# yeyupiaoling/VoiceprintRecognition-PaddlePaddle

Measured on NVIDIA H100. Metric: utterances/sec ECAPA-TDNN Fbank80 3s embed extract, higher is better.
Workload: dtype bf16x3 (split-bf16 operands, fp32 accumulate; fp32-grade)

## Files before the change

### include/ppv_b200.h

```cpp
#ifndef PPV_B200_H
#define PPV_B200_H

#include <stddef.h>
#include <stdint.h>

#ifdef __cplusplus
extern "C" {
#endif

#define PPV_OK 0
#define PPV_EINVAL (-1)
#define PPV_ECUDA (-2)
#define PPV_EUNSUPPORTED (-3)
#define PPV_ESTATE (-4)

#define PPV_PREC_BF16X3 0
#define PPV_PREC_BF16 1

#define PPV_POOL_ASP 0
#define PPV_POOL_SAP 1
#define PPV_POOL_TAP 2
#define PPV_POOL_TSP 3

typedef struct ppv_fbank ppv_fbank_t;
typedef struct ppv_model ppv_model_t;

int ppv_version(void);
int ppv_last_error(char* buf, size_t n);
int ppv_device_sm_count(void);

typedef struct {
    int sample_rate;
    int n_mels;
    float frame_length_ms;
    float frame_shift_ms;
    float preemph;
    float low_freq;
    float high_freq;
    float log_floor;
} ppv_fbank_cfg;

void ppv_fbank_default_cfg(ppv_fbank_cfg* cfg);
int ppv_fbank_create(const ppv_fbank_cfg* cfg, ppv_fbank_t** out);
int ppv_fbank_destroy(ppv_fbank_t* h);
int ppv_fbank_forward_ragged(ppv_fbank_t* h, const float* wav, const int32_t* valid_frames, int B, int L, float* out, void* stream);
int ppv_fbank_num_frames(const ppv_fbank_t* h, int L);
int ppv_fbank_feature_dim(const ppv_fbank_t* h);
int ppv_fbank_forward(ppv_fbank_t* h, const float* wav, const float* lens_ratio, int B, int L, float* out,
                      void* stream);

#define PPV_SPEC_SPECTROGRAM 1
#define PPV_SPEC_MEL 2
#define PPV_SPEC_LOGMEL 3
#define PPV_SPEC_MFCC 4
typedef struct {
    int method;
    int sample_rate;
    int n_fft;
    int hop_length;
    int win_length;
    float power;
    int center;
    int n_mels;
    float f_min;
    float f_max;
    int htk;
    int norm_slaney;
    float ref_value;
    float amin;
    int n_mfcc;
} ppv_spectral_cfg;
typedef struct ppv_spectral ppv_spectral_t;
void ppv_spectral_default_cfg(ppv_spectral_cfg* cfg, int method);
int ppv_spectral_create(const ppv_spectral_cfg* cfg, ppv_spectral_t** out);
int ppv_spectral_destroy(ppv_spectral_t* h);
int ppv_spectral_num_frames(const ppv_spectral_t* h, int L);
int ppv_spectral_feature_dim(const ppv_spectral_t* h);
int ppv_spectral_forward(ppv_spectral_t* h, const float* wav, const float* lens_ratio, int B, int L, float* out, void* stream);

#define PPV_SPECAUG_NPARAM 16
int ppv_spec_augment(float* feat, const int32_t* params, int B, int T, int F, int n_freq_masks, int n_time_masks, int fill_mode,
                     void* stream);

#define PPV_MODEL_ECAPA_TDNN 1

typedef struct {
    int input_size;
    int embd_dim;
    int channels[5];
    int kernel_sizes[5];
    int dilations[5];
    int attention_channels;
    int res2net_scale;
    int se_channels;
    int precision;
    int pooling;
    int global_context;
} ppv_ecapa_cfg;

void ppv_ecapa_default_cfg(ppv_ecapa_cfg* cfg);

#define PPV_MODEL_RESNET_SE 2
typedef struct {
    int input_size;
    int embd_dim;
    int layers[4];
    int num_filters[4];
    int attention_channels;
    int reduction;
    int precision;
} ppv_resnetse_cfg;
void ppv_resnetse_default_cfg(ppv_resnetse_cfg* cfg);

#define PPV_MODEL_ERES2NET 3
typedef struct {
    int input_size;
    int embd_dim;
    int num_blocks[4];
    int m_channels;
    int precision;
    int version;
    int base_width;
} ppv_eres2net_cfg;
void ppv_eres2net_default_cfg(ppv_eres2net_cfg* cfg);

#define PPV_MODEL_CAMPPLUS 4
typedef struct {
    int input_size;
    int embd_dim;
    int growth_rate;
    int bn_size;
    int init_channels;
    int precision;
} ppv_campplus_cfg;
void ppv_campplus_default_cfg(ppv_campplus_cfg* cfg);
int ppv_model_create(int kind, const void* cfg, ppv_model_t** out);
int ppv_model_destroy(ppv_model_t* h);
int ppv_model_load_weight(ppv_model_t* h, const char* name, const float* data, const int64_t* shape, int ndim);
int ppv_model_finalize(ppv_model_t* h);
int ppv_model_set_precision(ppv_model_t* h, int precision);
int ppv_model_embd_dim(const ppv_model_t* h);
size_t ppv_model_workspace_bytes(const ppv_model_t* h, int B, int T);
int ppv_model_forward(ppv_model_t* h, const float* feat, int B, int T, float* emb, void* ws, size_t ws_bytes,
                      void* stream);
int ppv_model_forward_lengths(ppv_model_t* h, const float* feat, const float* lengths, int B, int T, float* emb, void* ws,
                              size_t ws_bytes, void* stream);
int ppv_model_forward_wav(ppv_model_t* h, ppv_fbank_t* fb, const float* wav, const float* lens_ratio, int B, int L,
                          float* emb, void* ws, size_t ws_bytes, void* stream);
int ppv_model_read_tap(ppv_model_t* h, const char* name, float* out, size_t out_elems, void* stream);

int ppv_model_profile(ppv_model_t* h, int enable);
int ppv_model_profile_read(ppv_model_t* h, double* gemm_ms, double* other_ms, int64_t* gemm_launches,
                           int64_t* other_launches);

int ppv_set_pdl(int enabled);

typedef struct ppv_trainer ppv_trainer_t;
int ppv_trainer_create(const ppv_ecapa_cfg* cfg, int num_classes, ppv_trainer_t** out);
int ppv_trainer_destroy(ppv_trainer_t* h);
int64_t ppv_trainer_param_count(const ppv_trainer_t* h);
int64_t ppv_trainer_stat_count(const ppv_trainer_t* h);
int ppv_trainer_lookup(const ppv_trainer_t* h, const char* name, int64_t* offset, int64_t* numel, int* is_stat);
int ppv_trainer_bind(ppv_trainer_t* h, float* params, float* grads, float* stats);
int ppv_trainer_set_precision(ppv_trainer_t* h, int precision);
size_t ppv_trainer_workspace_bytes(ppv_trainer_t* h, int B, int T);
int ppv_trainer_forward_backward(ppv_trainer_t* h, const float* feat, const int64_t* labels, int B, int T, float margin, float scale,
                                 int easy_margin, float label_smoothing, float* loss, float* logits, void* ws, size_t ws_bytes, void* stream);
int ppv_trainer_read_tap(ppv_trainer_t* h, const char* name, float* out, size_t out_elems, void* stream);
int ppv_adam_step(float* params, const float* grads, float* m, float* v, int64_t n, float lr, float beta1, float beta2, float eps,
                  float weight_decay, int64_t step, float grad_scale, void* stream);

size_t ppv_cosine_workspace_bytes(int M, int N, int D);
int ppv_cosine_matrix(const float* A, const float* Bm, int M, int N, int D, float* out, void* ws, size_t ws_bytes,
                      void* stream);
int ppv_cosine_pairlist(const float* E, const int32_t* idx, int64_t P, int n, int D, float* out, void* stream);

#define PPV_PREP_NI 8
#define PPV_PREP_NF 4
size_t ppv_audio_prep_workspace_bytes(int B, int max_new_len);
int ppv_audio_prep(const float* wav, int64_t wav_ld, const int32_t* iparams, const float* fparams, const float* noise, int B,
                   int max_new_len, float target_db, int normalize, int Lout, float* out, void* ws, size_t ws_bytes, void* stream);

size_t ppv_eer_workspace_bytes(int64_t n);
int ppv_eer_mindcf(const float* scores, const int32_t* labels, int64_t n, double p_target, double c_miss, double c_fa, double* out4,
                   void* ws, size_t ws_bytes, void* stream);
int ppv_eer_mindcf_matrix(const float* scores, const int32_t* trial_labels, const int32_t* enroll_labels, int M, int N, double p_target,
                          double c_miss, double c_fa, double* out4, void* ws, size_t ws_bytes, void* stream);
int ppv_row_argmax(const float* sim, int rows, int cols, int32_t* idx, float* best, void* stream);

#define PPV_HEAD_AAM 0
#define PPV_HEAD_AAM_EASY 1
#define PPV_HEAD_AM 2
#define PPV_HEAD_ARM 3
#define PPV_HEAD_CE 4
#define PPV_HEAD_SUBCENTER 16
#define PPV_HEAD_SPHEREFACE2 8
int ppv_aam_forward(const float* emb, const float* W, const int64_t* labels, int B, int D, int S, float margin,
                    float scale, int easy_margin, float label_smoothing, float* logits, float* loss,
                    void* ws, size_t ws_bytes, void* stream);
size_t ppv_aam_workspace_bytes(int B, int D, int S);
int ppv_aam_backward(const float* emb, const float* W, const int64_t* labels, const float* logits, int B, int D,
                     int S, float margin, float scale, int easy_margin, float label_smoothing, float* d_emb,
                     float* d_W, void* ws, size_t ws_bytes, void* stream);

size_t ppv_gemm_test_workspace_bytes(int M, int N, int K);
int ppv_gemm_test(const float* A, const float* W, const float* bias, const float* bn_scale, const float* bn_shift,
                  int relu, int M, int N, int K, int block_n, int block_k, int precision, float* out, void* ws,
                  size_t ws_bytes, void* stream);

int ppv_gemm_test_planes(const float* A, const float* W, const float* bias, const float* rowgrp_bias, const float* bn_scale,
                         const float* bn_shift, int relu, int tanh_, int Tp, int P, int M, int N, int K, int block_n,
                         int precision, void* out, void* ws, size_t ws_bytes, void* stream);

size_t ppv_conv2d_test_workspace_bytes(int B, int H, int W, int Cin, int Cout, int k, int x_ld);
int ppv_conv2d_test(const float* x, const float* w, const float* bias, int relu, int B, int H, int W, int Cin, int Cout, int k,
                    int stride_h, int stride_w, int x_col0, int x_ld, int path, int precision, void* out, void* ws,
                    size_t ws_bytes, void* stream);

int ppv_gemm_bench(int M, int N, int K, int block_n, int block_k, int precision, int planes_out, int iters, void* ws,
                   size_t ws_bytes, float* ms_per_launch, void* stream);

#ifdef __cplusplus
}
#endif
#endif
```

### voiceprintrecognition-paddlepaddle_b200/csrc/capi.cu

```cuda
#include <string.h>

#include <new>

#include "common.h"
#include "image_plan.h"
#include "model_common.h"

namespace ppv {

static thread_local std::string g_last_error;

void set_error(const std::string& msg) { g_last_error = msg; }
int fail(int code, const std::string& msg) {
    g_last_error = msg;
    return code;
}

int device_sm_count() {
    int dev = 0, n = 0;
    if (cudaGetDevice(&dev) != cudaSuccess || cudaDeviceGetAttribute(&n, cudaDevAttrMultiProcessorCount, dev) != cudaSuccess || n <= 0) {
        cudaGetLastError();
        return 132;
    }
    return n;
}

static int check_device() {
    int dev = 0;
    if (cudaGetDevice(&dev) != cudaSuccess) return fail(PPV_ECUDA, "no CUDA device: libppv_b200 has no CPU fallback");
    int major = 0, minor = 0;
    cudaDeviceGetAttribute(&major, cudaDevAttrComputeCapabilityMajor, dev);
    cudaDeviceGetAttribute(&minor, cudaDevAttrComputeCapabilityMinor, dev);
    if (major != 9 || minor != 0) return fail(PPV_EUNSUPPORTED, "libppv_b200 is built for sm_90a only (found sm_" + std::to_string(major * 10 + minor) + ")");
    return PPV_OK;
}

}

using namespace ppv;

struct ppv_fbank {
    Fbank* impl;
};
struct ppv_spectral {
    Spectral* impl;
};

struct ppv_trainer {
    Trainer* impl;
};

struct ppv_model {
    int kind;
    Model* m;
};

static Model* ecapa_of(const ppv_model* h) { return h && h->kind == PPV_MODEL_ECAPA_TDNN ? h->m : nullptr; }

#define PPV_GUARD_BEGIN try {
#define PPV_GUARD_END                                                        \
    }                                                                        \
    catch (const std::bad_alloc&) { return fail(PPV_ECUDA, "host out of memory"); } \
    catch (const std::exception& e) { return fail(PPV_EINVAL, std::string("exception: ") + e.what()); } \
    catch (...) { return fail(PPV_EINVAL, "unknown exception"); }

extern "C" {

int ppv_version(void) { return 100; }

int ppv_last_error(char* buf, size_t n) {
    const std::string& e = g_last_error;
    if (buf && n > 0) {
        const size_t k = std::min(n - 1, e.size());
        memcpy(buf, e.data(), k);
        buf[k] = 0;
    }
    return int(e.size());
}

int ppv_device_sm_count(void) { return device_sm_count(); }

void ppv_fbank_default_cfg(ppv_fbank_cfg* c) {
    if (!c) return;
    c->sample_rate = 16000;
    c->n_mels = 80;
    c->frame_length_ms = 25.f;
    c->frame_shift_ms = 10.f;
    c->preemph = 0.97f;
    c->low_freq = 20.f;
    c->high_freq = 0.f;
    c->log_floor = 1.1920928955078125e-07f;
}

int ppv_fbank_create(const ppv_fbank_cfg* cfg, ppv_fbank_t** out) {
    PPV_GUARD_BEGIN
    PPV_REQUIRE(cfg && out, "ppv_fbank_create: null argument");
    int rc = check_device();
    if (rc) return rc;
    Fbank* impl = nullptr;
    rc = fbank_create(cfg, &impl);
    if (rc) return rc;
    *out = new ppv_fbank{impl};
    return PPV_OK;
    PPV_GUARD_END
}
int ppv_fbank_destroy(ppv_fbank_t* h) {
    if (!h) return PPV_OK;
    fbank_destroy(h->impl);
    delete h;
    return PPV_OK;
}
int ppv_fbank_num_frames(const ppv_fbank_t* h, int L) { return h ? fbank_num_frames(h->impl, L) : 0; }
int ppv_fbank_feature_dim(const ppv_fbank_t* h) { return h ? fbank_n_mels(h->impl) : 0; }

int ppv_fbank_forward(ppv_fbank_t* h, const float* wav, const float* lens_ratio, int B, int L, float* out, void* stream) {
    PPV_GUARD_BEGIN
    PPV_REQUIRE(h && wav && out, "ppv_fbank_forward: null argument");
    PPV_REQUIRE(B > 0 && L > 0, "ppv_fbank_forward: empty input");
    return fbank_run(h->impl, wav, lens_ratio, B, L, out, out, Planes(), 0, 0, static_cast<cudaStream_t>(stream));
    PPV_GUARD_END
}

int ppv_fbank_forward_ragged(ppv_fbank_t* h, const float* wav, const int32_t* valid_frames, int B, int L, float* out, void* stream) {
    PPV_GUARD_BEGIN
    PPV_REQUIRE(h && wav && out && valid_frames, "ppv_fbank_forward_ragged: null argument");
    PPV_REQUIRE(B > 0 && L > 0, "ppv_fbank_forward_ragged: empty input");
    return fbank_run(h->impl, wav, nullptr, B, L, out, out, Planes(), 0, 0, static_cast<cudaStream_t>(stream), valid_frames);
    PPV_GUARD_END
}

size_t ppv_audio_prep_workspace_bytes(int B, int max_new_len) { return audio_prep_workspace_bytes(B, max_new_len); }
int ppv_audio_prep(const float* wav, int64_t wav_ld, const int32_t* iparams, const float* fparams, const float* noise, int B, int max_new_len,
                   float target_db, int normalize, int Lout, float* out, void* ws, size_t ws_bytes, void* stream) {
    PPV_GUARD_BEGIN
    return audio_prep(wav, wav_ld, iparams, fparams, noise, B, max_new_len, target_db, normalize, Lout, out, ws, ws_bytes,
                      static_cast<cudaStream_t>(stream));
    PPV_GUARD_END
}

void ppv_ecapa_default_cfg(ppv_ecapa_cfg* c) {
    if (c) ppv_ecapa_default_cfg_impl(c);
}
void ppv_eres2net_default_cfg(ppv_eres2net_cfg* c) {
    if (c) ppv_eres2net_default_cfg_impl(c);
}
void ppv_campplus_default_cfg(ppv_campplus_cfg* c) {
    if (c) ppv_campplus_default_cfg_impl(c);
}
void ppv_resnetse_default_cfg(ppv_resnetse_cfg* c) {
    if (c) ppv_resnetse_default_cfg_impl(c);
}

int ppv_model_create(int kind, const void* cfg, ppv_model_t** out) {
    PPV_GUARD_BEGIN
    PPV_REQUIRE(cfg && out, "ppv_model_create: null argument");
    if (kind != PPV_MODEL_ECAPA_TDNN && kind != PPV_MODEL_RESNET_SE && kind != PPV_MODEL_ERES2NET && kind != PPV_MODEL_CAMPPLUS)
        return fail(PPV_EUNSUPPORTED,
                    "ppv_model_create: implemented kinds are PPV_MODEL_ECAPA_TDNN, PPV_MODEL_RESNET_SE, PPV_MODEL_ERES2NET, PPV_MODEL_CAMPPLUS");
    int rc = check_device();
    if (rc) return rc;
    Model* m = nullptr;
    switch (kind) {
        case PPV_MODEL_ECAPA_TDNN: rc = ecapa_create(static_cast<const ppv_ecapa_cfg*>(cfg), &m); break;
        case PPV_MODEL_RESNET_SE: rc = resnetse_create(static_cast<const ppv_resnetse_cfg*>(cfg), &m); break;
        case PPV_MODEL_ERES2NET: rc = eres2net_create(static_cast<const ppv_eres2net_cfg*>(cfg), &m); break;
        default: rc = campplus_create(static_cast<const ppv_campplus_cfg*>(cfg), &m); break;
    }
    if (rc) return rc;
    *out = new ppv_model{kind, m};
    return PPV_OK;
    PPV_GUARD_END
}
int ppv_model_destroy(ppv_model_t* h) {
    if (!h) return PPV_OK;
    delete h->m;
    delete h;
    return PPV_OK;
}
int ppv_model_load_weight(ppv_model_t* h, const char* name, const float* data, const int64_t* shape, int ndim) {
    PPV_GUARD_BEGIN
    PPV_REQUIRE(h, "ppv_model_load_weight: null model");
    return h->m->load_weight(name, data, shape, ndim);
    PPV_GUARD_END
}
int ppv_model_finalize(ppv_model_t* h) {
    PPV_GUARD_BEGIN
    PPV_REQUIRE(h, "ppv_model_finalize: null model");
    return h->m->finalize();
    PPV_GUARD_END
}
int ppv_model_set_precision(ppv_model_t* h, int precision) {
    PPV_REQUIRE(h, "ppv_model_set_precision: null model");
    return h->m->set_precision(precision);
}
int ppv_model_embd_dim(const ppv_model_t* h) { return h ? h->m->embd_dim() : 0; }
size_t ppv_model_workspace_bytes(const ppv_model_t* h, int B, int T) { return h ? h->m->workspace_bytes(B, T) : 0; }

int ppv_model_forward(ppv_model_t* h, const float* feat, int B, int T, float* emb, void* ws, size_t ws_bytes, void* stream) {
    PPV_GUARD_BEGIN
    PPV_REQUIRE(h && feat && emb, "ppv_model_forward: null argument");
    return h->m->forward(feat, B, T, emb, ws, ws_bytes, static_cast<cudaStream_t>(stream));
    PPV_GUARD_END
}
int ppv_model_forward_lengths(ppv_model_t* h, const float* feat, const float* lengths, int B, int T, float* emb, void* ws, size_t ws_bytes,
                              void* stream) {
    PPV_GUARD_BEGIN
    PPV_REQUIRE(h && feat && emb, "ppv_model_forward_lengths: null argument");
    if (!ecapa_of(h)) return fail(PPV_EUNSUPPORTED, "ppv_model_forward_lengths: only EcapaTdnn.forward takes lengths in the reference");
    return ecapa_forward(h->m, feat, nullptr, nullptr, nullptr, B, T, 0, emb, ws, ws_bytes, static_cast<cudaStream_t>(stream), lengths);
    PPV_GUARD_END
}
int ppv_model_forward_wav(ppv_model_t* h, ppv_fbank_t* fb, const float* wav, const float* lens_ratio, int B, int L, float* emb,
                          void* ws, size_t ws_bytes, void* stream) {
    PPV_GUARD_BEGIN
    PPV_REQUIRE(h && fb && wav && emb, "ppv_model_forward_wav: null argument");
    if (!ecapa_of(h)) return fail(PPV_EUNSUPPORTED, "ppv_model_forward_wav: the fused waveform path exists for ECAPA-TDNN only; call ppv_fbank_forward + ppv_model_forward");
    const int T = fbank_num_frames(fb->impl, L);
    PPV_REQUIRE(T > 0, "ppv_model_forward_wav: waveform shorter than one frame");
    return ecapa_forward(h->m, nullptr, fb->impl, wav, lens_ratio, B, T, L, emb, ws, ws_bytes, static_cast<cudaStream_t>(stream));
    PPV_GUARD_END
}
int ppv_model_read_tap(ppv_model_t* h, const char* name, float* out, size_t out_elems, void* stream) {
    PPV_GUARD_BEGIN
    PPV_REQUIRE(h, "ppv_model_read_tap: null model");
    return h->m->read_tap(name, out, out_elems, static_cast<cudaStream_t>(stream));
    PPV_GUARD_END
}

size_t ppv_eer_workspace_bytes(int64_t n) { return eer_workspace_bytes(n); }
int ppv_eer_mindcf(const float* scores, const int32_t* labels, int64_t n, double p_target, double c_miss, double c_fa, double* out4, void* ws,
                   size_t ws_bytes, void* stream) {
    PPV_GUARD_BEGIN
    PPV_REQUIRE(labels, "ppv_eer_mindcf: null labels");
    return eer_mindcf(scores, labels, nullptr, nullptr, 0, n, p_target, c_miss, c_fa, out4, ws, ws_bytes, static_cast<cudaStream_t>(stream));
    PPV_GUARD_END
}
int ppv_eer_mindcf_matrix(const float* scores, const int32_t* trial_labels, const int32_t* enroll_labels, int M, int N, double p_target,
                          double c_miss, double c_fa, double* out4, void* ws, size_t ws_bytes, void* stream) {
    PPV_GUARD_BEGIN
    PPV_REQUIRE(trial_labels && enroll_labels && M > 0 && N > 0, "ppv_eer_mindcf_matrix: bad argument");
    return eer_mindcf(scores, nullptr, trial_labels, enroll_labels, N, int64_t(M) * N, p_target, c_miss, c_fa, out4, ws, ws_bytes,
                      static_cast<cudaStream_t>(stream));
    PPV_GUARD_END
}
int ppv_row_argmax(const float* sim, int rows, int cols, int32_t* idx, float* best, void* stream) {
    PPV_GUARD_BEGIN
    return row_argmax(sim, rows, cols, idx, best, static_cast<cudaStream_t>(stream));
    PPV_GUARD_END
}

int ppv_model_profile(ppv_model_t* h, int enable) {
    PPV_REQUIRE(ecapa_of(h), "ppv_model_profile: ECAPA-TDNN model required");
    return ecapa_profile(h->m, enable);
}
int ppv_model_profile_read(ppv_model_t* h, double* gemm_ms, double* other_ms, int64_t* gemm_launches, int64_t* other_launches) {
    PPV_GUARD_BEGIN
    PPV_REQUIRE(ecapa_of(h), "ppv_model_profile_read: ECAPA-TDNN model required");
    return ecapa_profile_read(h->m, gemm_ms, other_ms, gemm_launches, other_launches);
    PPV_GUARD_END
}

void ppv_spectral_default_cfg(ppv_spectral_cfg* c, int method) {
    if (c) spectral_default_cfg(c, method);
}
int ppv_spectral_create(const ppv_spectral_cfg* cfg, ppv_spectral_t** out) {
    PPV_GUARD_BEGIN
    PPV_REQUIRE(cfg && out, "ppv_spectral_create: null argument");
    int rc = check_device();
    if (rc) return rc;
    Spectral* impl = nullptr;
    rc = spectral_create(cfg, &impl);
    if (rc) return rc;
    *out = new ppv_spectral{impl};
    return PPV_OK;
    PPV_GUARD_END
}
int ppv_spectral_destroy(ppv_spectral_t* h) {
    if (!h) return PPV_OK;
    spectral_destroy(h->impl);
    delete h;
    return PPV_OK;
}
int ppv_spectral_num_frames(const ppv_spectral_t* h, int L) { return h ? spectral_num_frames(h->impl, L) : 0; }
int ppv_spectral_feature_dim(const ppv_spectral_t* h) { return h ? spectral_feature_dim(h->impl) : 0; }
int ppv_spectral_forward(ppv_spectral_t* h, const float* wav, const float* lens_ratio, int B, int L, float* out, void* stream) {
    PPV_GUARD_BEGIN
    PPV_REQUIRE(h && wav && out, "ppv_spectral_forward: null argument");
    PPV_REQUIRE(B > 0 && L > 0, "ppv_spectral_forward: empty input");
    return spectral_run(h->impl, wav, lens_ratio, B, L, out, static_cast<cudaStream_t>(stream));
    PPV_GUARD_END
}
int ppv_spec_augment(float* feat, const int32_t* params, int B, int T, int F, int n_freq_masks, int n_time_masks, int fill_mode, void* stream) {
    PPV_GUARD_BEGIN
    return spec_augment_run(feat, params, B, T, F, n_freq_masks, n_time_masks, fill_mode, static_cast<cudaStream_t>(stream));
    PPV_GUARD_END
}

int ppv_trainer_create(const ppv_ecapa_cfg* cfg, int num_classes, ppv_trainer_t** out) {
    PPV_GUARD_BEGIN
    PPV_REQUIRE(cfg && out, "ppv_trainer_create: null argument");
    int rc = check_device();
    if (rc) return rc;
    Trainer* impl = nullptr;
    rc = trainer_create(cfg, num_classes, &impl);
    if (rc) return rc;
    *out = new ppv_trainer{impl};
    return PPV_OK;
    PPV_GUARD_END
}
int ppv_trainer_destroy(ppv_trainer_t* h) {
    if (!h) return PPV_OK;
    trainer_destroy(h->impl);
    delete h;
    return PPV_OK;
}
int64_t ppv_trainer_param_count(const ppv_trainer_t* h) { return h ? trainer_param_count(h->impl) : 0; }
int64_t ppv_trainer_stat_count(const ppv_trainer_t* h) { return h ? trainer_stat_count(h->impl) : 0; }
int ppv_trainer_lookup(const ppv_trainer_t* h, const char* name, int64_t* offset, int64_t* numel, int* is_stat) {
    PPV_GUARD_BEGIN
    PPV_REQUIRE(h, "ppv_trainer_lookup: null handle");
    return trainer_lookup(h->impl, name, offset, numel, is_stat);
    PPV_GUARD_END
}
int ppv_set_pdl(int enabled) {
    const int prev = ppv::pdl_enabled();
    ppv::pdl_enabled() = enabled ? 1 : 0;
    return prev;
}
int ppv_trainer_set_precision(ppv_trainer_t* h, int precision) {
    PPV_GUARD_BEGIN
    PPV_REQUIRE(h, "ppv_trainer_set_precision: null handle");
    return trainer_set_precision(h->impl, precision);
    PPV_GUARD_END
}
int ppv_trainer_bind(ppv_trainer_t* h, float* params, float* grads, float* stats) {
    PPV_GUARD_BEGIN
    PPV_REQUIRE(h, "ppv_trainer_bind: null handle");
    return trainer_bind(h->impl, params, grads, stats);
    PPV_GUARD_END
}
size_t ppv_trainer_workspace_bytes(ppv_trainer_t* h, int B, int T) {
    try {
        return h ? trainer_workspace_bytes(h->impl, B, T) : 0;
    } catch (...) {
        return 0;
    }
}
int ppv_trainer_forward_backward(ppv_trainer_t* h, const float* feat, const int64_t* labels, int B, int T, float margin, float scale,
                                 int easy_margin, float label_smoothing, float* loss, float* logits, void* ws, size_t ws_bytes, void* stream) {
    PPV_GUARD_BEGIN
    PPV_REQUIRE(h, "ppv_trainer_forward_backward: null handle");
    return trainer_forward_backward(h->impl, feat, labels, B, T, margin, scale, easy_margin, label_smoothing, loss, logits, ws, ws_bytes,
                                    static_cast<cudaStream_t>(stream));
    PPV_GUARD_END
}
int ppv_trainer_read_tap(ppv_trainer_t* h, const char* name, float* out, size_t out_elems, void* stream) {
    PPV_GUARD_BEGIN
    PPV_REQUIRE(h, "ppv_trainer_read_tap: null handle");
    return trainer_read_tap(h->impl, name, out, out_elems, static_cast<cudaStream_t>(stream));
    PPV_GUARD_END
}
int ppv_adam_step(float* params, const float* grads, float* m, float* v, int64_t n, float lr, float beta1, float beta2, float eps,
                  float weight_decay, int64_t step, float grad_scale, void* stream) {
    PPV_GUARD_BEGIN
    return adam_step(params, grads, m, v, n, lr, beta1, beta2, eps, weight_decay, step, grad_scale, static_cast<cudaStream_t>(stream));
    PPV_GUARD_END
}

size_t ppv_cosine_workspace_bytes(int M, int N, int D) { return cosine_workspace_bytes(M, N, D); }
int ppv_cosine_matrix(const float* A, const float* Bm, int M, int N, int D, float* out, void* ws, size_t ws_bytes, void* stream) {
    PPV_GUARD_BEGIN
    int rc = check_device();
    if (rc) return rc;
    return cosine_matrix(A, Bm, M, N, D, out, ws, ws_bytes, PPV_PREC_BF16X3, static_cast<cudaStream_t>(stream));
    PPV_GUARD_END
}
int ppv_cosine_pairlist(const float* E, const int32_t* idx, int64_t P, int n, int D, float* out, void* stream) {
    PPV_GUARD_BEGIN
    return cosine_pairlist(E, idx, P, n, D, out, static_cast<cudaStream_t>(stream));
    PPV_GUARD_END
}

size_t ppv_aam_workspace_bytes(int B, int D, int S) { return aam_workspace_bytes(B, D, S); }
int ppv_aam_forward(const float* emb, const float* W, const int64_t* labels, int B, int D, int S, float margin, float scale,
                    int easy_margin, float label_smoothing, float* logits, float* loss, void* ws, size_t ws_bytes, void* stream) {
    PPV_GUARD_BEGIN
    return aam_forward(emb, W, labels, B, D, S, margin, scale, easy_margin, label_smoothing, logits, loss, ws, ws_bytes,
                       static_cast<cudaStream_t>(stream));
    PPV_GUARD_END
}
int ppv_aam_backward(const float* emb, const float* W, const int64_t* labels, const float* logits, int B, int D, int S, float margin,
                     float scale, int easy_margin, float label_smoothing, float* d_emb, float* d_W, void* ws, size_t ws_bytes,
                     void* stream) {
    PPV_GUARD_BEGIN
    return aam_backward(emb, W, labels, logits, B, D, S, margin, scale, easy_margin, label_smoothing, d_emb, d_W, ws, ws_bytes,
                        static_cast<cudaStream_t>(stream));
    PPV_GUARD_END
}

static inline size_t au(size_t x, size_t a) { return (x + a - 1) / a * a; }
size_t ppv_gemm_test_workspace_bytes(int M, int N, int K) {
    const size_t Kp = au(size_t(K), 64);
    return au(au(size_t(M), 128) * Kp * 4, 256) + au(au(size_t(N), 256) * Kp * 4, 256) + 256;
}
int ppv_gemm_test(const float* A, const float* W, const float* bias, const float* bn_scale, const float* bn_shift, int relu, int M,
                  int N, int K, int block_n, int block_k, int precision, float* out, void* ws, size_t ws_bytes, void* stream) {
    PPV_GUARD_BEGIN
    PPV_REQUIRE(A && W && out && ws, "ppv_gemm_test: null argument");
    PPV_REQUIRE(ws_bytes >= ppv_gemm_test_workspace_bytes(M, N, K), "ppv_gemm_test: workspace too small");
    int rc = check_device();
    if (rc) return rc;
    cudaStream_t st = static_cast<cudaStream_t>(stream);
    const int Kp = int(au(size_t(K), 64));
    Planes pa, pw;
    pa.rows = int64_t(au(size_t(M), 128));
    pa.ld = Kp;
    pa.plane_stride = pa.rows * Kp;
    pa.base = static_cast<__nv_bfloat16*>(ws);
    pw.rows = int64_t(au(size_t(N), 256));
    pw.ld = Kp;
    pw.plane_stride = pw.rows * Kp;
    pw.base = reinterpret_cast<__nv_bfloat16*>(static_cast<uint8_t*>(ws) + au(size_t(pa.plane_stride) * 4, 256));
    PPV_CUDA_OK(cudaMemsetAsync(ws, 0, ppv_gemm_test_workspace_bytes(M, N, K), st));
    rc = launch_f32_to_planes(A, M, K, pa, st);
    if (rc) return rc;
    rc = launch_f32_to_planes(W, N, K, pw, st);
    if (rc) return rc;
    GemmSource src{pa, 0, Kp, 0};
    Epilogue ep;
    ep.bias = bias;
    ep.relu = relu;
    ep.bn_scale = bn_scale;
    ep.bn_shift = bn_shift;
    ep.out_mode = OUT_F32;
    ep.out = out;
    ep.out_ld = N;
    GemmParams gp;
    rc = gemm_build(&gp, &src, 1, pw, M, N, ep, block_n, block_k);
    if (rc) return rc;
    return gemm_launch(gp, precision, device_sm_count(), st);
    PPV_GUARD_END
}

int ppv_gemm_test_planes(const float* A, const float* W, const float* bias, const float* rowgrp_bias, const float* bn_scale,
                         const float* bn_shift, int relu, int tanh_, int Tp, int P, int M, int N, int K, int block_n, int precision,
                         void* out, void* ws, size_t ws_bytes, void* stream) {
    PPV_GUARD_BEGIN
    PPV_REQUIRE(A && W && out && ws, "ppv_gemm_test_planes: null argument");
    PPV_REQUIRE(ws_bytes >= ppv_gemm_test_workspace_bytes(M, N, K), "ppv_gemm_test_planes: workspace too small");
    PPV_REQUIRE(N % 32 == 0 && (Tp == 0 || (M % Tp == 0 && Tp > 2 * P)), "ppv_gemm_test_planes: bad shape");
    int rc = check_device();
    if (rc) return rc;
    cudaStream_t st = static_cast<cudaStream_t>(stream);
    const int Kp = int(au(size_t(K), 64));
    Planes pa, pw;
    pa.rows = int64_t(au(size_t(M), 128));
    pa.ld = Kp;
    pa.plane_stride = pa.rows * Kp;
    pa.base = static_cast<__nv_bfloat16*>(ws);
    pw.rows = int64_t(au(size_t(N), 256));
    pw.ld = Kp;
    pw.plane_stride = pw.rows * Kp;
    pw.base = reinterpret_cast<__nv_bfloat16*>(static_cast<uint8_t*>(ws) + au(size_t(pa.plane_stride) * 4, 256));
    PPV_CUDA_OK(cudaMemsetAsync(ws, 0, ppv_gemm_test_workspace_bytes(M, N, K), st));
    rc = launch_f32_to_planes(A, M, K, pa, st);
    if (rc) return rc;
    rc = launch_f32_to_planes(W, N, K, pw, st);
    if (rc) return rc;
    GemmSource src{pa, 0, Kp, 0};
    Epilogue ep;
    ep.bias = bias;
    ep.rowgrp_bias = rowgrp_bias;
    ep.relu = relu;
    ep.tanh_ = tanh_;
    ep.bn_scale = bn_scale;
    ep.bn_shift = bn_shift;
    ep.out_mode = OUT_PLANES;
    ep.out = out;
    ep.out_ld = N;
    ep.out_plane_stride = int64_t(M) * N;
    if (Tp > 0) {
        ep.Tp = Tp;
        ep.P = P;
        ep.T = Tp - 2 * P;
    }
    GemmParams gp;
    rc = gemm_build(&gp, &src, 1, pw, M, N, ep, block_n, 64);
    if (rc) return rc;
    return gemm_launch(gp, precision, device_sm_count(), st);
    PPV_GUARD_END
}

static size_t conv2d_test_x_bytes(int B, int H, int W, int x_ld) {
    return au(au(size_t(B) * (H + 2) * (W + 2), 128) * size_t(x_ld) * 4, 256);
}
size_t ppv_conv2d_test_workspace_bytes(int B, int H, int W, int Cin, int Cout, int k, int x_ld) {
    if (x_ld <= 0) x_ld = Cin;
    return conv2d_test_x_bytes(B, H, W, x_ld) + au(au(size_t(Cout), 256) * k * k * Cin * 4, 256) + 256;
}
int ppv_conv2d_test(const float* x, const float* w, const float* bias, int relu, int B, int H, int W, int Cin, int Cout, int k,
                    int stride_h, int stride_w, int x_col0, int x_ld, int path, int precision, void* out, void* ws, size_t ws_bytes,
                    void* stream) {
    PPV_GUARD_BEGIN
    PPV_REQUIRE(x && w && out && ws, "ppv_conv2d_test: null argument");
    if (x_ld <= 0) x_ld = Cin;
    PPV_REQUIRE(B > 0 && H > 0 && W > 0 && Cin > 0 && Cout > 0 && (k == 1 || k == 3) && stride_h >= 1 && stride_w >= 1,
                "ppv_conv2d_test: bad shape");
    PPV_REQUIRE(x_col0 >= 0 && x_col0 + Cin <= x_ld, "ppv_conv2d_test: the input columns exceed x_ld");
    PPV_REQUIRE(path >= 0 && path <= 2, "ppv_conv2d_test: path must be 0 (3x3 patch kernel), 1 (pointwise kernel) or 2 (gather-GEMM)");
    PPV_REQUIRE(precision == PPV_PREC_BF16X3 || precision == PPV_PREC_BF16, "ppv_conv2d_test: bad precision");
    PPV_REQUIRE(ws_bytes >= ppv_conv2d_test_workspace_bytes(B, H, W, Cin, Cout, k, x_ld), "ppv_conv2d_test: workspace too small");
    const int Hp = H + 2, Wp = W + 2, Ho = (H - 1) / stride_h + 1, Wo = (W - 1) / stride_w + 1;
    const int64_t M = int64_t(B) * Hp * Wp;
    PPV_REQUIRE(M < (int64_t(1) << 31) && Wp + 1 < 32768, "ppv_conv2d_test: grid too large for 32-bit rows / 16-bit tap offsets");
    int rc = check_device();
    if (rc) return rc;
    cudaStream_t st = static_cast<cudaStream_t>(stream);
    Planes xp;
    xp.rows = int64_t(au(size_t(M), 128));
    xp.ld = x_ld;
    xp.plane_stride = xp.rows * x_ld;
    xp.base = static_cast<__nv_bfloat16*>(ws);
    const size_t x_bytes = conv2d_test_x_bytes(B, H, W, x_ld);
    PPV_CUDA_OK(cudaMemsetAsync(ws, 0, x_bytes, st));
    const size_t pitch = size_t(x_ld) * sizeof(__nv_bfloat16), rows2 = size_t(2 * xp.rows);
    if (x_col0 > 0) PPV_CUDA_OK(cudaMemset2DAsync(xp.base, pitch, 0x3f, size_t(x_col0) * sizeof(__nv_bfloat16), rows2, st));
    if (x_col0 + Cin < x_ld)
        PPV_CUDA_OK(cudaMemset2DAsync(xp.base + x_col0 + Cin, pitch, 0x3f, size_t(x_ld - x_col0 - Cin) * sizeof(__nv_bfloat16), rows2, st));
    for (int b = 0; b < B; ++b)
        for (int h = 0; h < H; ++h) {
            Planes row = xp;
            row.base = xp.base + ((int64_t(b) * Hp + h + 1) * Wp + 1) * x_ld + x_col0;
            rc = launch_f32_to_planes(x + (int64_t(b) * H + h) * W * Cin, W, Cin, row, st);
            if (rc) return rc;
        }
    const int K = k * k * Cin;
    std::vector<float> wh(size_t(Cout) * K);
    PPV_CUDA_OK(cudaMemcpyAsync(wh.data(), w, wh.size() * sizeof(float), cudaMemcpyDeviceToHost, st));
    PPV_CUDA_OK(cudaStreamSynchronize(st));
    ArenaBuilder ab;
    GemmWeights gw;
    ab.put_matrix(&gw, conv_weight_matrix(wh.data(), Cout, Cin, k * k, Cout, {{k * k, Cin, 0, Cin, 0}}), Cout, K);
    uint8_t* wdev = static_cast<uint8_t*>(ws) + x_bytes;
    PPV_CUDA_OK(cudaMemcpyAsync(wdev, ab.host.data(), ab.host.size(), cudaMemcpyHostToDevice, st));
    PPV_CUDA_OK(cudaStreamSynchronize(st));
    gw.W.base = reinterpret_cast<__nv_bfloat16*>(wdev + ab.patches[0].off);
    const int64_t out_plane = int64_t(B) * (Ho + 2) * (Wo + 2) * Cout;
    PPV_CUDA_OK(cudaMemsetAsync(out, 0, size_t(2 * out_plane) * sizeof(__nv_bfloat16), st));
    Planes outp;
    outp.base = static_cast<__nv_bfloat16*>(out);
    outp.ld = Cout;
    outp.plane_stride = out_plane;
    const ImageGeo gin{H, W, Hp, Wp}, gout{Ho, Wo, Ho + 2, Wo + 2};
    Epilogue ep = image_epilogue(outp, gin, gout, stride_h, stride_w);
    ep.bias = bias;
    ep.relu = relu ? 1 : 0;
    const int sms = device_sm_count();
    if (path == 0) {
        PPV_REQUIRE(k == 3 && conv3x3_c32_supported(Cin, Cout, H, W), "ppv_conv2d_test: the patch kernel takes 3x3 convs with 32 -> 32 channels only");
        Conv3x3Params cp;
        rc = conv3x3_build(&cp, xp, x_col0, gw.W, B, H, W, Hp, Wp, ep);
        if (rc) return rc;
        return conv3x3_launch(cp, precision, sms, st);
    }
    if (path == 1) {
        PPV_REQUIRE(k == 1, "ppv_conv2d_test: the pointwise kernel takes 1x1 convs only");
        const GemmSource src{xp, x_col0, Cin, 0};
        PwStep s;
        if (!pointwise_step_build(&s, &src, 1, gw.W, Cout, M, ep))
            return fail(PPV_EINVAL, "ppv_conv2d_test: the pointwise kernel does not take this conv (or PPV_POINTWISE=0)");
        return pointwise_launch(s, sms, st);
    }
    std::vector<GemmSource> srcs;
    if (k == 3)
        image_taps(&srcs, xp, x_col0, Cin, gin);
    else
        srcs.push_back(GemmSource{xp, x_col0, Cin, 0});
    GemmParams gp;
    rc = gemm_build(&gp, srcs.data(), int(srcs.size()), gw.W, int(M), Cout, ep, gemm_pick_bn(Cout));
    if (rc) return rc;
    return gemm_launch(gp, precision, sms, st);
    PPV_GUARD_END
}

int ppv_gemm_bench(int M, int N, int K, int block_n, int block_k, int precision, int planes_out, int iters, void* ws, size_t ws_bytes,
                   float* ms_per_launch, void* stream) {
    PPV_GUARD_BEGIN
    PPV_REQUIRE(ws && ms_per_launch && iters > 0, "ppv_gemm_bench: bad argument");
    PPV_REQUIRE(planes_out >= 0 && planes_out <= 3, "ppv_gemm_bench: planes_out must be 0-3");
    constexpr int kTp = 306, kP = 4;
    PPV_REQUIRE(planes_out < 2 || M % kTp == 0, "ppv_gemm_bench: model epilogues need M % 306 == 0");
    cudaStream_t st = static_cast<cudaStream_t>(stream);
    const size_t Kp = au(size_t(K), 64);
    const size_t a_bytes = au(au(size_t(M), 128) * Kp * 4, 256), w_bytes = au(au(size_t(N), 256) * Kp * 4, 256);
    const size_t o_bytes = au(au(size_t(M), 128) * size_t(N) * 4, 256);
    const size_t v_bytes = au((3 + size_t(M / kTp)) * size_t(N) * 4, 256);
    PPV_REQUIRE(ws_bytes >= a_bytes + w_bytes + o_bytes + v_bytes, "ppv_gemm_bench: workspace too small");
    Planes pa, pw, po;
    pa.rows = int64_t(au(size_t(M), 128)); pa.ld = int(Kp); pa.plane_stride = pa.rows * pa.ld; pa.base = static_cast<__nv_bfloat16*>(ws);
    pw.rows = int64_t(au(size_t(N), 256)); pw.ld = int(Kp); pw.plane_stride = pw.rows * pw.ld;
    pw.base = reinterpret_cast<__nv_bfloat16*>(static_cast<uint8_t*>(ws) + a_bytes);
    po.rows = pa.rows; po.ld = N; po.plane_stride = po.rows * po.ld;
    po.base = reinterpret_cast<__nv_bfloat16*>(static_cast<uint8_t*>(ws) + a_bytes + w_bytes);
    PPV_CUDA_OK(cudaMemsetAsync(ws, 0x11, a_bytes + w_bytes, st));
    float* vec = reinterpret_cast<float*>(static_cast<uint8_t*>(ws) + a_bytes + w_bytes + o_bytes);
    PPV_CUDA_OK(cudaMemsetAsync(vec, 0x3c, v_bytes, st));
    GemmSource src{pa, 0, int(Kp), 0};
    Epilogue ep;
    ep.relu = 1;
    if (planes_out) {
        ep.out_mode = OUT_PLANES; ep.out = po.base; ep.out_ld = po.ld; ep.out_plane_stride = po.plane_stride;
        if (planes_out >= 2) {
            ep.Tp = kTp; ep.P = kP; ep.T = kTp - 2 * kP;
            ep.bias = vec; ep.bn_scale = vec + N; ep.bn_shift = vec + 2 * N;
            if (planes_out == 3) { ep.rowgrp_bias = vec + 3 * N; ep.tanh_ = 1; }
        }
    } else {
        ep.out_mode = OUT_F32; ep.out = po.base; ep.out_ld = N;
    }
    GemmParams gp;
    int rc = gemm_build(&gp, &src, 1, pw, M, N, ep, block_n, block_k);
    if (rc) return rc;
    const int sms = device_sm_count();
    for (int i = 0; i < 3; ++i) { rc = gemm_launch(gp, precision, sms, st); if (rc) return rc; }
    cudaEvent_t e0, e1;
    PPV_CUDA_OK(cudaEventCreate(&e0));
    PPV_CUDA_OK(cudaEventCreate(&e1));
    PPV_CUDA_OK(cudaEventRecord(e0, st));
    for (int i = 0; i < iters; ++i) { rc = gemm_launch(gp, precision, sms, st); if (rc) return rc; }
    PPV_CUDA_OK(cudaEventRecord(e1, st));
    PPV_CUDA_OK(cudaEventSynchronize(e1));
    float ms = 0.f;
    PPV_CUDA_OK(cudaEventElapsedTime(&ms, e0, e1));
    cudaEventDestroy(e0);
    cudaEventDestroy(e1);
    gemm_trace_dump(gp);
    *ms_per_launch = ms / float(iters);
    return PPV_OK;
    PPV_GUARD_END
}

}
```

### voiceprintrecognition-paddlepaddle_b200/csrc/common.h

```cpp
#pragma once
#include <cuda.h>
#include <cuda_bf16.h>
#include <cuda_runtime.h>
#include <stdint.h>
#include <stdlib.h>

#include <algorithm>
#include <string>
#include <utility>

#include "../../include/ppv_b200.h"

namespace ppv {

void set_error(const std::string& msg);
int fail(int code, const std::string& msg);

#define PPV_CUDA_OK(expr)                                                                             \
    do {                                                                                              \
        cudaError_t _e = (expr);                                                                      \
        if (_e != cudaSuccess)                                                                        \
            return ::ppv::fail(PPV_ECUDA, std::string(#expr) + ": " + cudaGetErrorString(_e));        \
    } while (0)
#define PPV_LAUNCH_OK(what)                                                                           \
    do {                                                                                              \
        cudaError_t _e = cudaGetLastError();                                                          \
        if (_e != cudaSuccess) return ::ppv::fail(PPV_ECUDA, std::string(what) + ": " + cudaGetErrorString(_e)); \
    } while (0)
#define PPV_REQUIRE(cond, msg)                                     \
    do {                                                           \
        if (!(cond)) return ::ppv::fail(PPV_EINVAL, std::string(msg)); \
    } while (0)

#define PPV_ONCE_PER_DEVICE(stmt)                                    \
    do {                                                             \
        static unsigned long long _ppv_done = 0ull;                  \
        int _ppv_dev = 0;                                            \
        cudaGetDevice(&_ppv_dev);                                    \
        if (!((_ppv_done >> (_ppv_dev & 63)) & 1ull)) {              \
            stmt;                                                    \
            _ppv_done |= 1ull << (_ppv_dev & 63);                    \
        }                                                            \
    } while (0)

inline int& pdl_enabled() {
    static int v = 1;
    return v;
}

template <typename... KArgs, typename... Args>
inline cudaError_t launch_pdl(void (*kernel)(KArgs...), dim3 grid, dim3 block, size_t smem, cudaStream_t st, Args&&... args) {
    cudaLaunchConfig_t cfg = {};
    cfg.gridDim = grid;
    cfg.blockDim = block;
    cfg.dynamicSmemBytes = smem;
    cfg.stream = st;
    cudaLaunchAttribute attr[1];
    attr[0].id = cudaLaunchAttributeProgrammaticStreamSerialization;
    attr[0].val.programmaticStreamSerializationAllowed = pdl_enabled() ? 1 : 0;
    cfg.attrs = attr;
    cfg.numAttrs = 1;
    return cudaLaunchKernelEx(&cfg, kernel, std::forward<Args>(args)...);
}
#define PPV_PDL_OK(call, what)                                                                                     \
    do {                                                                                                           \
        cudaError_t _e = (call);                                                                                   \
        if (_e != cudaSuccess) return ::ppv::fail(PPV_ECUDA, std::string(what) + ": " + cudaGetErrorString(_e));   \
    } while (0)

struct Planes {
    __nv_bfloat16* base = nullptr;
    int64_t rows = 0;
    int ld = 0;
    int64_t plane_stride = 0;
    __host__ __device__ __nv_bfloat16* hi() const { return base; }
    __host__ __device__ __nv_bfloat16* lo() const { return base + plane_stride; }
};

struct TimeLayout {
    int B = 0, T = 0, P = 0, Tp = 0;
    int64_t rows() const { return int64_t(B) * Tp; }
};

constexpr int GEMM_BM = 128;
constexpr int GEMM_BK = 64;
constexpr int GEMM_MAX_KSTEPS = 192;
constexpr int GEMM_MAX_MAPS = 4;
constexpr int GEMM_WS_STAGES = 4;

struct KStep {
    int16_t map;
    int16_t row_off;
    int32_t a_col;
};

enum OutMode : int { OUT_PLANES = 0, OUT_F32 = 1 };

struct Epilogue {
    const float* bias = nullptr;
    const float* rowgrp_bias = nullptr;
    const float* bn_scale = nullptr;
    const float* bn_shift = nullptr;
    int relu = 0;
    int tanh_ = 0;
    int sigmoid_ = 0;
    int silu_ = 0;
    float relu_max = 0.f;
    int out_mode = OUT_PLANES;
    void* out = nullptr;
    int64_t out_ld = 0;
    int64_t out_plane_stride = 0;
    int out_col0 = 0;
    int Tp = 0, P = 0, T = 0;
    int halo = 0;
    int img_Hp = 0, img_Wp = 0, img_H = 0, img_W = 0, img_stride = 1, out_Hp = 0, out_Wp = 0;
    int img_stride_w = 0;
    const float* seg_scale = nullptr;
    int seg_len = 0, nseg = 0;
    int zero_invalid = 0;
    int f32_vec_ok = 0;
    int debug_nostore = 0;
    int lean = 0;
};

constexpr int GEMM_TRACE_TILES = 16;

struct GemmParams {
    CUtensorMap mapA[GEMM_MAX_MAPS];
    CUtensorMap mapB;
    KStep ksteps[GEMM_MAX_KSTEPS];
    int num_ksteps;
    int bk;
    int l2_prefetch;
    int ws;
    int lin_splits;
    int lin_b_row0, lin_b_col0;
    int64_t lin_split_rows;
    int M, N;
    int m_tiles, n_tiles;
    Epilogue epi;
    unsigned long long* trace;
    int bn;
};
void gemm_trace_dump(const GemmParams& gp);

struct GemmSource {
    Planes t;
    int col0;
    int ncols;
    int row_off;
};

int gemm_build(GemmParams* gp, const GemmSource* srcs, int nsrc, const Planes& W, int M, int N, const Epilogue& epi,
               int BN, int BK = 0);
int gemm_build_wgrad(GemmParams* gp, const Planes& At, const Planes& Bt, int M, int N, int b_row0, int b_col0, int splits, float* out,
                     int64_t out_ld, int out_col0, int64_t split_rows, int BN);
int gemm_launch(const GemmParams& gp, int precision, int num_sms, cudaStream_t stream);
inline int gemm_pick_bn(int N, int max_bn = 256) {
    for (int bn = max_bn; bn > 64; bn /= 2)
        if (N % bn == 0) return bn;
    return 64;
}

int encode_planes_map(CUtensorMap* m, const Planes& t, int box_rows);
int encode_planes_map_ex(CUtensorMap* m, const Planes& t, int box_cols, int box_rows, int swizzle_bytes);

struct Res2Params {
    CUtensorMap mapA[2];
    CUtensorMap mapW;
    int a_col[2];
    int nsrc, dil;
    int l2_prefetch;
    int M, m_tiles;
    Epilogue epi;
};
int res2conv_build(Res2Params* rp, const GemmSource* srcs, int nsrc, const Planes& W, int M, int dil, const Epilogue& epi);
int res2conv_launch(const Res2Params& rp, int precision, int num_sms, cudaStream_t st);

struct Conv3x3Params {
    CUtensorMap mapX;
    CUtensorMap mapW;
    int x_col0;
    int B, H, W, Hp, Wp;
    int nph, npw, patches;
    Epilogue epi;
};
bool conv3x3_c32_supported(int Cin, int Cout, int H, int W);
int conv3x3_build(Conv3x3Params* cp, const Planes& x, int x_col0, const Planes& Wt, int B, int H, int W, int Hp, int Wp, const Epilogue& epi);
int conv3x3_launch(const Conv3x3Params& cp, int precision, int num_sms, cudaStream_t st);

constexpr int RES2CHAIN_MAX = 7;
struct Res2ChainParams {
    CUtensorMap mapX;
    CUtensorMap mapXt, mapY, mapYtail;
    CUtensorMap mapW[RES2CHAIN_MAX];
    const float* bias[RES2CHAIN_MAX];
    const float* bn_scale[RES2CHAIN_MAX];
    const float* bn_shift[RES2CHAIN_MAX];
    Planes x;
    Planes y;
    int nconv, width, B, T, P, Tp, dil, ntiles;
    int paired;
    unsigned long long* trace;
};
int res2chain_build(Res2ChainParams* cp, const Planes& x, const Planes& y, const Planes* W, const float* const* bias, const float* const* bn_scale,
                    const float* const* bn_shift, int nconv, int B, int T, int P, int Tp, int dil, bool paired);
int res2chain_launch(const Res2ChainParams& cp, int precision, int num_sms, cudaStream_t st);
bool res2chain_fits(int T, int P);
bool res2chain_pair_fits(int T, int P);
void res2chain_trace_dump(const Res2ChainParams& cp);

int pointwise_launch(const GemmSource* srcs, int nsrc, const Planes& W, int64_t M, int N, const Epilogue& ep, int num_sms, cudaStream_t st);
struct PwStep {
    GemmSource srcs[2];
    int nsrc = 0, N = 0;
    int64_t M = 0;
    Planes W;
    Epilogue ep;
};
inline int pointwise_launch(const PwStep& s, int num_sms, cudaStream_t st) { return pointwise_launch(s.srcs, s.nsrc, s.W, s.M, s.N, s.ep, num_sms, st); }
bool pointwise_step_build(PwStep* s, const GemmSource* srcs, int nsrc, const Planes& W, int N, int64_t M, const Epilogue& ep);

bool skinny_linear_supported(int M, int N, int K, const Epilogue& ep);
int skinny_linear_launch(const Planes& x, int x_col0, const Planes& W, int M, int N, int K, const Epilogue& ep, cudaStream_t st);

struct AspFusedParams {
    CUtensorMap mapW;
    CUtensorMap mapAtt;
    CUtensorMap mapX;
    Planes x;
    Planes gstat;
    const float* bn_scale;
    const float* bn_shift;
    Planes out;
    float* out_raw;
    int B, T, P, Tp, C, K;
    float eps;
    const int* nvalid;
};

int asp_fused_build(AspFusedParams* p, const Planes& W, const Planes& att, const Planes& x, const Planes& gstat, const float* bn_scale,
                    const float* bn_shift, const Planes& out, float* out_raw, int B, int T, int P, int Tp, int C, int K, float eps);
int asp_fused_launch(const AspFusedParams& p, int precision, int num_sms, cudaStream_t st);

int launch_pack_features(const float* feat, int B, int T, int F, const Planes& out, int P, int Tp, cudaStream_t st);
int launch_colstats(const Planes& x, int col0, int C, int B, int T, int P, int Tp, int mode, float eps, float* out_f32,
                    const Planes& out_pl, cudaStream_t st, float inv_count = 0.f, const int* nvalid = nullptr);
int launch_lengths_to_counts(const float* lengths, int B, int T, int* nvalid, cudaStream_t st);
int launch_se_scale_res(const Planes& z, const float* scale, const Planes& res, int rc0, const Planes& out, int oc0, int C,
                        int Tp, int64_t rows, int num_sms, cudaStream_t st, int relu = 0, float relu_max = 0.f);
int launch_asp_pool(const float* logits, int64_t lg_ld, const Planes& x, int C, int B, int T, int P, int Tp, float eps,
                    const float* bn_scale, const float* bn_shift, const Planes& out_pl, float* out_raw, cudaStream_t st);
int launch_planes_to_f32(const Planes& x, int col0, int C, int B, int T, int P, int Tp, float* out, cudaStream_t st);
int launch_f32_to_planes(const float* src, int64_t rows, int cols, const Planes& out, cudaStream_t st);

struct Fbank;
int fbank_create(const ppv_fbank_cfg* cfg, Fbank** out);
void fbank_destroy(Fbank* h);
int fbank_num_frames(const Fbank* h, int L);
int fbank_n_mels(const Fbank* h);
int fbank_run(Fbank* h, const float* wav, const float* lens_ratio, int B, int L, float* raw, float* out_f32,
              const Planes& out_pl, int P, int Tp, cudaStream_t st, const int* valid_frames = nullptr);

size_t audio_prep_workspace_bytes(int B, int max_new_len);
int audio_prep(const float* wav, int64_t wav_ld, const int32_t* iparams, const float* fparams, const float* noise, int B, int max_new_len,
               float target_db, int normalize, int Lout, float* out, void* ws, size_t ws_bytes, cudaStream_t st);

struct Spectral;
void spectral_default_cfg(ppv_spectral_cfg* c, int method);
int spectral_create(const ppv_spectral_cfg* cfg, Spectral** out);
void spectral_destroy(Spectral* h);
int spectral_num_frames(const Spectral* h, int L);
int spectral_feature_dim(const Spectral* h);
int spectral_run(Spectral* h, const float* wav, const float* lens_ratio, int B, int L, float* out, cudaStream_t st);
int spec_augment_run(float* feat, const int32_t* params, int B, int T, int F, int n_freq_masks, int n_time_masks, int fill_mode, cudaStream_t st);

struct Model;
void ppv_ecapa_default_cfg_impl(ppv_ecapa_cfg* c);
int ecapa_create(const ppv_ecapa_cfg* cfg, Model** out);
int ecapa_forward(Model* m, const float* feat, Fbank* fb, const float* wav, const float* lens_ratio, int B, int T, int L, float* emb,
                  void* ws, size_t ws_bytes, cudaStream_t st, const float* lengths = nullptr);
int ecapa_profile(Model* m, int enable);
int ecapa_profile_read(Model* m, double* gemm_ms, double* other_ms, int64_t* gemm_launches, int64_t* other_launches);
void ppv_resnetse_default_cfg_impl(ppv_resnetse_cfg* c);
int resnetse_create(const ppv_resnetse_cfg* cfg, Model** out);
void ppv_eres2net_default_cfg_impl(ppv_eres2net_cfg* c);
int eres2net_create(const ppv_eres2net_cfg* cfg, Model** out);
void ppv_campplus_default_cfg_impl(ppv_campplus_cfg* c);
int campplus_create(const ppv_campplus_cfg* cfg, Model** out);

struct ImageGeo {
    int H = 0, W = 0, Hp = 0, Wp = 0;
    int64_t rows(int B) const { return int64_t(B) * Hp * Wp; }
};
int launch_stem_conv(const float* feat, int B, int T, int F, const float* w9, const float* bias, int C0, const Planes& out, int Hp, int Wp,
                     cudaStream_t st);
int launch_flatten_image(const Planes& in, int B, int H, int W, int Hp, int Wp, int C, const Planes& out, int num_sms, cudaStream_t st);
int launch_image_to_f32(const Planes& in, int B, int H, int W, int Hp, int Wp, int C, float* out, cudaStream_t st);
int launch_aff_combine(const Planes& x, int xc0, const Planes& y, int yc0, const Planes& t, const Planes& out, int C, int64_t rows, int num_sms,
                       cudaStream_t st);

struct Trainer;
int trainer_create(const ppv_ecapa_cfg* cfg, int num_classes, Trainer** out);
void trainer_destroy(Trainer* t);
int64_t trainer_param_count(const Trainer* t);
int64_t trainer_stat_count(const Trainer* t);
int trainer_lookup(const Trainer* t, const char* name, int64_t* off, int64_t* numel, int* is_stat);
int trainer_bind(Trainer* t, float* params, float* grads, float* stats);
int trainer_set_precision(Trainer* t, int precision);
size_t trainer_workspace_bytes(Trainer* t, int B, int T);
int trainer_forward_backward(Trainer* t, const float* feat, const int64_t* labels, int B, int T, float margin, float scale, int easy_margin,
                             float label_smoothing, float* loss_out, float* logits_out, void* ws, size_t ws_bytes, cudaStream_t st);
int trainer_read_tap(Trainer* t, const char* name, float* out, size_t out_elems, cudaStream_t st);
int adam_step(float* params, const float* grads, float* m, float* v, int64_t n, float lr, float beta1, float beta2, float eps, float weight_decay,
              int64_t step, float grad_scale, cudaStream_t st);

size_t cosine_workspace_bytes(int M, int N, int D);
int cosine_matrix(const float* A, const float* Bm, int M, int N, int D, float* out, void* ws, size_t ws_bytes, int precision,
                  cudaStream_t st);
int cosine_pairlist(const float* E, const int32_t* idx, int64_t P, int n, int D, float* out, cudaStream_t st);
size_t aam_workspace_bytes(int B, int D, int S);
int aam_forward(const float* emb, const float* W, const int64_t* labels, int B, int D, int S, float margin, float scale,
                int easy_margin, float label_smoothing, float* logits, float* loss, void* ws, size_t ws_bytes, cudaStream_t st);
int aam_backward(const float* emb, const float* W, const int64_t* labels, const float* logits, int B, int D, int S, float margin,
                 float scale, int easy_margin, float label_smoothing, float* d_emb, float* d_W, void* ws, size_t ws_bytes,
                 cudaStream_t st);

size_t eer_workspace_bytes(int64_t n);
int eer_mindcf(const float* scores, const int32_t* labels, const int32_t* row_labels, const int32_t* col_labels, int ncols, int64_t n,
               double p_target, double c_miss, double c_fa, double* out, void* ws, size_t ws_bytes, cudaStream_t st);
int row_argmax(const float* sim, int rows, int cols, int32_t* idx, float* best, cudaStream_t st);

int device_sm_count();

}
```

### voiceprintrecognition-paddlepaddle_b200/csrc/ecapa.cu

```cuda
#include <stdlib.h>
#include <string.h>

#include "common.h"
#include "model_common.h"

namespace ppv {

namespace {

struct ConvW : GemmWeights {
    float* bn_scale = nullptr;
    float* bn_shift = nullptr;
};

struct KSpec {
    int src;
    int col0, ncols, row_off;
    int w_cin0, w_cnt, w_tap;
};

enum Buf { B_FEAT, B_X0, B_H, B_Y, B_Z, B_CAT, B_MFA, B_ATT, B_GSTAT, B_POOL, B_SEM, B_SEH, B_COUNT };

struct Step {
    enum Kind { GEMM, SKINNY, RES2, RES2CHAIN, SE_SQUEEZE, SE_SCALE, ASP_GLOBAL, ASP_FUSED, POOL_STATS } kind;
    Planes sk_x, sk_w;
    int sk_col0 = 0, sk_M = 0, sk_N = 0, sk_K = 0;
    Epilogue sk_ep;
    GemmParams gp;
    AspFusedParams ap;
    Res2Params rp;
    Res2ChainParams cp;
    int blk = 0;
};

struct EcBuffers {
    Planes bufs[B_COUNT];
    float *se_mean = nullptr, *se_scale = nullptr, *fold_out = nullptr, *pooled_raw = nullptr, *raw_logmel = nullptr;
    int* nvalid = nullptr;
};

}

struct EcapaModel : Model {
    ppv_ecapa_cfg cfg;
    int C = 0, C3 = 0, width = 0, scale = 0, Fp = 0, P = 0, att = 0, se = 0;
    ConvW conv0, tdnn1[3], res2[3][8], tdnn2[3], se1[3], se2[3], mfa, fold, att1, att2, fc;
    float *aspbn_scale = nullptr, *aspbn_shift = nullptr;
    std::vector<Step> steps;
    EcBuffers buf;
    int Tp = 0;
    bool prof_on = false;
    std::vector<cudaEvent_t> prof_ev;
    std::vector<int> prof_kind;
    size_t prof_used = 0;
    int64_t launches_gemm = 0, launches_other = 0;

    explicit EcapaModel(const ppv_ecapa_cfg& c) : Model("ecapa", c.precision), cfg(c) {}
    ~EcapaModel() override {
        for (cudaEvent_t e : prof_ev) cudaEventDestroy(e);
    }
    int embd_dim() const override { return cfg.embd_dim; }
    size_t workspace_bytes(int B, int T) const override;
    int forward_ex(const float* feat, Fbank* fb, const float* wav, const float* lens_ratio, int B, int T, int L, float* emb, void* ws,
                   size_t ws_bytes, cudaStream_t st, const float* lengths);

  protected:
    bool prepare_weights(ArenaBuilder& ab) override;
    int build_plan(int B, int T, void* ws, size_t ws_bytes, cudaStream_t st) override;
    int run_steps(const float* feat, cudaStream_t st) override { return run(feat, nullptr, nullptr, nullptr, 0, nullptr, st); }
    int tap(const std::string& n, float* out, size_t out_elems, cudaStream_t st) override;
    int run(const float* feat, Fbank* fb, const float* wav, const float* lens_ratio, int L, const float* lengths, cudaStream_t st);
};

void ppv_ecapa_default_cfg_impl(ppv_ecapa_cfg* c) {
    c->input_size = 80;
    c->embd_dim = 192;
    const int ch[5] = {512, 512, 512, 512, 1536}, ks[5] = {5, 3, 3, 3, 1}, dl[5] = {1, 2, 3, 4, 1};
    for (int i = 0; i < 5; ++i) {
        c->channels[i] = ch[i];
        c->kernel_sizes[i] = ks[i];
        c->dilations[i] = dl[i];
    }
    c->attention_channels = 128;
    c->res2net_scale = 8;
    c->se_channels = 128;
    c->precision = PPV_PREC_BF16X3;
    c->pooling = PPV_POOL_ASP;
    c->global_context = 1;
}

int ecapa_create(const ppv_ecapa_cfg* cfg, Model** out) {
    PPV_REQUIRE(cfg && out, "ecapa_create: null argument");
    const int C = cfg->channels[0];
    if (cfg->channels[1] != C || cfg->channels[2] != C || cfg->channels[3] != C)
        return fail(PPV_EUNSUPPORTED, "ecapa: channels[0..3] must be equal (no shortcut conv path)");
    if (cfg->channels[4] != 3 * C) return fail(PPV_EUNSUPPORTED, "ecapa: channels[4] must equal 3 * channels[0] (MFA concat)");
    if (cfg->res2net_scale < 2 || cfg->res2net_scale > 8 || C % cfg->res2net_scale)
        return fail(PPV_EUNSUPPORTED, "ecapa: res2net_scale must divide channels and be in [2,8]");
    const int width = C / cfg->res2net_scale;
    if (width % 64) return fail(PPV_EUNSUPPORTED, "ecapa: channels / res2net_scale must be a multiple of 64");
    if (cfg->kernel_sizes[1] != 3 || cfg->kernel_sizes[2] != 3 || cfg->kernel_sizes[3] != 3 || cfg->kernel_sizes[4] != 1 ||
        (cfg->kernel_sizes[0] % 2) == 0 || cfg->dilations[4] != 1)
        return fail(PPV_EUNSUPPORTED, "ecapa: kernel sizes must be [odd,3,3,3,1]");
    if (cfg->attention_channels % 64 || cfg->embd_dim % 32 || cfg->se_channels <= 0 || cfg->se_channels % 64)
        return fail(PPV_EUNSUPPORTED, "ecapa: attention_channels % 64, se_channels % 64, embd_dim % 32 required");
    if (cfg->pooling < PPV_POOL_ASP || cfg->pooling > PPV_POOL_TSP) return fail(PPV_EUNSUPPORTED, "ecapa: pooling must be PPV_POOL_ASP / SAP / TAP / TSP");
    EcapaModel* m = new EcapaModel(*cfg);
    m->C = C;
    m->C3 = 3 * C;
    m->width = width;
    m->scale = cfg->res2net_scale;
    m->Fp = int(mc_align_up(cfg->input_size, 64));
    m->att = cfg->attention_channels;
    m->se = cfg->se_channels;
    int P = (cfg->kernel_sizes[0] - 1) / 2 * cfg->dilations[0];
    for (int i = 1; i <= 3; ++i) P = std::max(P, cfg->dilations[i]);
    m->P = P;
    *out = m;
    return PPV_OK;
}

namespace {

void put_conv(ArenaBuilder& ab, ConvW* cw, const std::vector<float>& w, int N, int Cin, int k, const std::vector<KSpec>& ks) {
    int Ktot = 0;
    for (const KSpec& s : ks) Ktot += s.ncols;
    std::vector<double> mtx(size_t(N) * Ktot, 0.0);
    for (int n = 0; n < N; ++n) {
        int kpos = 0;
        for (const KSpec& s : ks) {
            for (int c = 0; c < s.w_cnt; ++c) mtx[size_t(n) * Ktot + kpos + c] = w[(size_t(n) * Cin + s.w_cin0 + c) * k + s.w_tap];
            kpos += s.ncols;
        }
    }
    ab.put_matrix(cw, mtx, N, Ktot, 128);
}

bool bn_affine_f32(ArenaBuilder& ab, const std::string& prefix, int C, std::vector<float>* scale, std::vector<float>* shift) {
    std::vector<double> sc, sh;
    if (!ab.bn_affine(prefix, C, &sc, &sh)) return false;
    scale->assign(sc.begin(), sc.end());
    shift->assign(sh.begin(), sh.end());
    return true;
}

std::vector<KSpec> spec_conv0(const EcapaModel* m) {
    std::vector<KSpec> ks;
    const int k = m->cfg.kernel_sizes[0], d = m->cfg.dilations[0];
    for (int j = 0; j < k; ++j) ks.push_back({B_FEAT, 0, m->Fp, (j - (k - 1) / 2) * d, 0, m->cfg.input_size, j});
    return ks;
}
std::vector<KSpec> spec_res2(const EcapaModel* m, int blk, int j) {
    std::vector<KSpec> ks;
    const int d = m->cfg.dilations[blk], w = m->width;
    for (int tap = 0; tap < 3; ++tap) ks.push_back({B_H, j * w, w, (tap - 1) * d, 0, w, tap});
    if (j >= 2)
        for (int tap = 0; tap < 3; ++tap) ks.push_back({B_Y, (j - 1) * w, w, (tap - 1) * d, 0, w, tap});
    return ks;
}

}

bool EcapaModel::prepare_weights(ArenaBuilder& ab) {
    EcapaModel* const m = this;
    const int C = m->C, C3 = m->C3, w = m->width, F = m->cfg.input_size, A = m->att, S = m->se, E = m->cfg.embd_dim;
    const int k0 = m->cfg.kernel_sizes[0];
    auto conv_layer = [&](ConvW* cw, const std::string& wname, int N, int Cin, int k, const std::vector<KSpec>& ks,
                          const std::string& bn_prefix, bool has_bias) -> bool {
        const HostWeight* hw = ab.get(wname + ".weight", {N, Cin, k});
        if (!hw) return false;
        put_conv(ab, cw, hw->v, N, Cin, k, ks);
        if (has_bias) {
            const HostWeight* hb = ab.get(wname + ".bias", {N});
            if (!hb) return false;
            ab.put_f32(&cw->bias, hb->v);
        }
        if (!bn_prefix.empty()) {
            std::vector<float> sc, sh;
            if (!bn_affine_f32(ab, bn_prefix, N, &sc, &sh)) return false;
            ab.put_f32(&cw->bn_scale, sc);
            ab.put_f32(&cw->bn_shift, sh);
        }
        return true;
    };
    bool ok = conv_layer(&m->conv0, "blocks.0.conv.conv", C, F, k0, spec_conv0(m), "blocks.0.norm.norm", true);
    for (int b = 1; b <= 3 && ok; ++b) {
        const std::string p = "blocks." + std::to_string(b);
        ok = ok && conv_layer(&m->tdnn1[b - 1], p + ".tdnn1.conv.conv", C, C, 1, {{-1, 0, C, 0, 0, C, 0}}, p + ".tdnn1.norm.norm", true);
        for (int j = 1; j < m->scale && ok; ++j) {
            const std::string q = p + ".res2net_block.blocks." + std::to_string(j - 1);
            ok = ok && conv_layer(&m->res2[b - 1][j], q + ".conv.conv", w, w, 3, spec_res2(m, b, j), q + ".norm.norm", true);
        }
        ok = ok && conv_layer(&m->tdnn2[b - 1], p + ".tdnn2.conv.conv", C, C, 1, {{B_H, 0, w, 0, 0, w, 0}, {B_Y, w, C - w, 0, w, C - w, 0}},
                              p + ".tdnn2.norm.norm", true);
        ok = ok && conv_layer(&m->se1[b - 1], p + ".se_block.conv1.conv", S, C, 1, {{B_SEM, 0, C, 0, 0, C, 0}}, "", true);
        ok = ok && conv_layer(&m->se2[b - 1], p + ".se_block.conv2.conv", C, S, 1, {{B_SEH, 0, S, 0, 0, S, 0}}, "", true);
    }
    ok = ok && conv_layer(&m->mfa, "mfa.conv.conv", C3, C3, 1, {{B_CAT, 0, C3, 0, 0, C3, 0}}, "mfa.norm.norm", true);
    const int pooling = m->cfg.pooling;
    auto folded_fc = [&](int Kp) -> bool {
        const HostWeight* w = ab.get("fc.conv.weight", {E, Kp, 1});
        const HostWeight* b = ab.get("fc.conv.bias", {E});
        std::vector<float> sc, sh;
        if (!w || !b || !bn_affine_f32(ab, "asp_bn", Kp, &sc, &sh)) return false;
        std::vector<float> wf(size_t(E) * Kp), bf(E);
        for (int n = 0; n < E; ++n) {
            double acc = b->v[n];
            for (int k = 0; k < Kp; ++k) {
                wf[size_t(n) * Kp + k] = w->v[size_t(n) * Kp + k] * sc[k];
                acc += double(w->v[size_t(n) * Kp + k]) * sh[k];
            }
            bf[n] = float(acc);
        }
        put_conv(ab, &m->fc, wf, E, Kp, 1, {{B_POOL, 0, Kp, 0, 0, Kp, 0}});
        ab.put_f32(&m->fc.bias, bf);
        return true;
    };
    if (pooling == PPV_POOL_ASP) {
    const int ctx = m->cfg.global_context ? 3 : 1;
    ok = ok && conv_layer(&m->att1, "asp.tdnn.conv.conv", A, ctx * C3, 1, {{B_MFA, 0, C3, 0, 0, C3, 0}}, "asp.tdnn.norm.norm", true);
    if (ok && m->cfg.global_context) {
        const HostWeight* hw = ab.get("asp.tdnn.conv.conv.weight", {A, 3 * C3, 1});
        put_conv(ab, &m->fold, hw->v, A, 3 * C3, 1, {{B_GSTAT, 0, 2 * C3, 0, C3, 2 * C3, 0}});
    }
    ok = ok && conv_layer(&m->att2, "asp.conv.conv", C3, A, 1, {{B_ATT, 0, A, 0, 0, A, 0}}, "", true);
    ok = ok && conv_layer(&m->fc, "fc.conv", E, 2 * C3, 1, {{B_POOL, 0, 2 * C3, 0, 0, 2 * C3, 0}}, "", true);
    if (ok) {
        std::vector<float> sc, sh;
        ok = bn_affine_f32(ab, "asp_bn.norm", 2 * C3, &sc, &sh);
        if (ok) {
            ab.put_f32(&m->aspbn_scale, sc);
            ab.put_f32(&m->aspbn_shift, sh);
        }
    }
    } else if (pooling == PPV_POOL_SAP) {
        if (A != 128) {
            ab.err = "SAP pooling uses a 128-channel bottleneck (ecapa_tdnn.py:222): attention_channels must be 128";
            ok = false;
        }
        ok = ok && conv_layer(&m->att1, "asp.linear1", A, C3, 1, {{B_MFA, 0, C3, 0, 0, C3, 0}}, "", true);
        ok = ok && conv_layer(&m->att2, "asp.linear2", C3, A, 1, {{B_ATT, 0, A, 0, 0, A, 0}}, "", true);
        ok = ok && folded_fc(C3);
        if (ok) {
            ab.put_f32(&m->aspbn_scale, std::vector<float>(2 * C3, 1.f));
            ab.put_f32(&m->aspbn_shift, std::vector<float>(2 * C3, 0.f));
        }
    } else {
        ok = ok && folded_fc(pooling == PPV_POOL_TAP ? C3 : 2 * C3);
    }
    return ok;
}

namespace {

void carve(const EcapaModel* m, WsCarver& cv, int B, int T, EcBuffers* eb, float** emb_out) {
    const int64_t R = int64_t(B) * (T + 2 * m->P);
    const int C = m->C, C3 = m->C3;
    eb->bufs[B_FEAT] = cv.planes(R, m->Fp);
    eb->bufs[B_X0] = cv.planes(R, C);
    eb->bufs[B_H] = cv.planes(R, C);
    eb->bufs[B_Y] = cv.planes(R, C);
    eb->bufs[B_Z] = cv.planes(R, C);
    eb->bufs[B_CAT] = cv.planes(R, C3);
    eb->bufs[B_MFA] = cv.planes(R, C3);
    eb->bufs[B_ATT] = cv.planes(R, m->att);
    eb->bufs[B_GSTAT] = cv.planes(B, 2 * C3);
    eb->bufs[B_POOL] = cv.planes(B, 2 * C3);
    eb->bufs[B_SEM] = cv.planes(B, C);
    eb->bufs[B_SEH] = cv.planes(B, m->se);
    eb->se_mean = static_cast<float*>(cv.take(size_t(B) * C * 4));
    eb->se_scale = static_cast<float*>(cv.take(size_t(B) * C * 4));
    eb->fold_out = static_cast<float*>(cv.take(mc_align_up(B, 128) * m->att * 4));
    eb->pooled_raw = static_cast<float*>(cv.take(size_t(B) * 2 * C3 * 4));
    eb->raw_logmel = static_cast<float*>(cv.take(size_t(B) * T * m->cfg.input_size * 4));
    *emb_out = static_cast<float*>(cv.take(mc_align_up(B, 128) * m->cfg.embd_dim * 4));
    eb->nvalid = static_cast<int*>(cv.take(size_t(B) * sizeof(int)));
}

constexpr int ECAPA_MAX_BN = 128;

}

size_t EcapaModel::workspace_bytes(int B, int T) const {
    if (B <= 0 || T <= 0) return 0;
    WsCarver cv;
    EcBuffers eb;
    float* emb;
    carve(this, cv, B, T, &eb, &emb);
    return mc_align_up(cv.off, 256);
}

int EcapaModel::build_plan(int B, int T, void* ws, size_t ws_bytes, cudaStream_t st) {
    EcapaModel* const m = this;
    PPV_REQUIRE(T > m->P, "ecapa: too few frames for the reflect padding");
    const size_t need = workspace_bytes(B, T);
    PPV_REQUIRE(ws && ws_bytes >= need, "ecapa: workspace too small (see ppv_model_workspace_bytes)");
    PPV_REQUIRE((reinterpret_cast<uintptr_t>(ws) & 255) == 0, "ecapa: workspace must be 256-byte aligned");
    WsCarver cv;
    cv.base = static_cast<uint8_t*>(ws);
    carve(m, cv, B, T, &m->buf, &m->emb_out);
    m->Tp = T + 2 * m->P;
    PPV_CUDA_OK(cudaMemsetAsync(ws, 0, need, st));
    m->steps.clear();
    const int Tp = m->Tp, P = m->P, C = m->C, C3 = m->C3, w = m->width;
    const int64_t R = int64_t(B) * Tp;
    const char* r2env = getenv("PPV_RES2_GEMM");
    const bool use_res2_kernel = (w == 64) && !(r2env && r2env[0] == '1');
    const char* rcenv = getenv("PPV_RES2_CHAIN");
    const bool use_res2_chain = use_res2_kernel && m->scale == 8 && res2chain_fits(T, P) && !(rcenv && rcenv[0] == '0');
    const bool res2_paired = use_res2_chain && res2chain_pair_fits(T, P) && !(rcenv && strcmp(rcenv, "single") == 0);
    const char* skenv = getenv("PPV_SKINNY");
    const bool use_skinny = !(skenv && skenv[0] == '0');

    auto add_gemm = [&](const ConvW& cw, const std::vector<KSpec>& ks, const Planes* src_override, int override_col0, int M,
                        Epilogue ep) -> int {
        std::vector<GemmSource> srcs;
        for (const KSpec& s : ks) {
            GemmSource g;
            if (s.src < 0) {
                g.t = *src_override;
                g.col0 = override_col0 + s.col0;
            } else {
                g.t = m->buf.bufs[s.src];
                g.col0 = s.col0;
            }
            g.ncols = s.ncols;
            g.row_off = s.row_off;
            srcs.push_back(g);
        }
        ep.bias = cw.bias;
        if (ep.relu) {
            ep.bn_scale = cw.bn_scale;
            ep.bn_shift = cw.bn_shift;
        }
        if (use_skinny && M == B && srcs.size() == 1 && srcs[0].row_off == 0 && skinny_linear_supported(M, cw.N, srcs[0].ncols, ep) &&
            cw.Ktot == srcs[0].ncols) {
            Step sk;
            sk.kind = Step::SKINNY;
            sk.sk_x = srcs[0].t;
            sk.sk_col0 = srcs[0].col0;
            sk.sk_w = cw.W;
            sk.sk_M = M;
            sk.sk_N = cw.N;
            sk.sk_K = srcs[0].ncols;
            sk.sk_ep = ep;
            m->steps.push_back(sk);
            return PPV_OK;
        }
        Step stp;
        stp.kind = Step::GEMM;
        int rc = gemm_build(&stp.gp, srcs.data(), int(srcs.size()), cw.W, M, cw.N, ep, gemm_pick_bn(cw.N, ECAPA_MAX_BN));
        if (rc) return rc;
        m->steps.push_back(stp);
        return PPV_OK;
    };
    auto planes_out = [&](const Planes& p, int col0, bool halo) {
        Epilogue ep;
        ep.out_mode = OUT_PLANES;
        ep.out = p.base;
        ep.out_ld = p.ld;
        ep.out_plane_stride = p.plane_stride;
        ep.out_col0 = col0;
        ep.Tp = Tp;
        ep.P = P;
        ep.T = T;
        ep.halo = halo ? 1 : 0;
        ep.relu = 1;
        return ep;
    };
    int rc = add_gemm(m->conv0, spec_conv0(m), nullptr, 0, int(R), planes_out(m->buf.bufs[B_X0], 0, false));
    if (rc) return rc;
    for (int b = 1; b <= 3; ++b) {
        const Planes& X = (b == 1) ? m->buf.bufs[B_X0] : m->buf.bufs[B_CAT];
        const int xcol = (b == 1) ? 0 : (b - 2) * C;
        rc = add_gemm(m->tdnn1[b - 1], {{-1, 0, C, 0, 0, C, 0}}, &X, xcol, int(R), planes_out(m->buf.bufs[B_H], 0, !use_res2_chain));
        if (rc) return rc;
        if (use_res2_chain) {
            Planes Wj[RES2CHAIN_MAX];
            const float *bj[RES2CHAIN_MAX], *sj[RES2CHAIN_MAX], *hj[RES2CHAIN_MAX];
            for (int j = 1; j < m->scale; ++j) {
                const ConvW& cw = m->res2[b - 1][j];
                Wj[j - 1] = cw.W;
                bj[j - 1] = cw.bias;
                sj[j - 1] = cw.bn_scale;
                hj[j - 1] = cw.bn_shift;
            }
            Step stp;
            stp.kind = Step::RES2CHAIN;
            rc = res2chain_build(&stp.cp, m->buf.bufs[B_H], m->buf.bufs[B_Y], Wj, bj, sj, hj, m->scale - 1, B, T, P, Tp, m->cfg.dilations[b],
                                 res2_paired);
            if (rc) return rc;
            m->steps.push_back(stp);
        }
        for (int j = 1; j < m->scale && !use_res2_chain; ++j) {
            if (use_res2_kernel) {
                GemmSource srcs[2];
                srcs[0] = GemmSource{m->buf.bufs[B_H], j * w, w, 0};
                srcs[1] = GemmSource{m->buf.bufs[B_Y], (j - 1) * w, w, 0};
                Epilogue ep = planes_out(m->buf.bufs[B_Y], j * w, true);
                const ConvW& cw = m->res2[b - 1][j];
                ep.bias = cw.bias;
                ep.bn_scale = cw.bn_scale;
                ep.bn_shift = cw.bn_shift;
                Step stp;
                stp.kind = Step::RES2;
                rc = res2conv_build(&stp.rp, srcs, j >= 2 ? 2 : 1, cw.W, int(R), m->cfg.dilations[b], ep);
                if (rc) return rc;
                m->steps.push_back(stp);
            } else {
                rc = add_gemm(m->res2[b - 1][j], spec_res2(m, b, j), nullptr, 0, int(R), planes_out(m->buf.bufs[B_Y], j * w, true));
                if (rc) return rc;
            }
        }
        rc = add_gemm(m->tdnn2[b - 1], {{B_H, 0, w, 0, 0, w, 0}, {B_Y, w, C - w, 0, w, C - w, 0}}, nullptr, 0, int(R),
                      planes_out(m->buf.bufs[B_Z], 0, false));
        if (rc) return rc;
        Step s;
        s.blk = b;
        s.kind = Step::SE_SQUEEZE;
        m->steps.push_back(s);
        {
            Epilogue e1;
            e1.out_mode = OUT_PLANES;
            e1.out = m->buf.bufs[B_SEH].base;
            e1.out_ld = m->buf.bufs[B_SEH].ld;
            e1.out_plane_stride = m->buf.bufs[B_SEH].plane_stride;
            e1.relu = 1;
            rc = add_gemm(m->se1[b - 1], {{B_SEM, 0, C, 0, 0, 0, 0}}, nullptr, 0, B, e1);
            if (rc) return rc;
            Epilogue e2;
            e2.out_mode = OUT_F32;
            e2.out = m->buf.se_scale;
            e2.out_ld = C;
            e2.sigmoid_ = 1;
            rc = add_gemm(m->se2[b - 1], {{B_SEH, 0, m->se, 0, 0, 0, 0}}, nullptr, 0, B, e2);
            if (rc) return rc;
        }
        s.kind = Step::SE_SCALE;
        m->steps.push_back(s);
    }
    rc = add_gemm(m->mfa, {{B_CAT, 0, C3, 0, 0, C3, 0}}, nullptr, 0, int(R), planes_out(m->buf.bufs[B_MFA], 0, false));
    if (rc) return rc;
    const int pooling = m->cfg.pooling;
    if (pooling == PPV_POOL_TAP || pooling == PPV_POOL_TSP) {
        Step s;
        s.kind = Step::POOL_STATS;
        m->steps.push_back(s);
    } else {
        Step s;
        s.kind = Step::ASP_GLOBAL;
        m->steps.push_back(s);
    }
    if (pooling == PPV_POOL_ASP && m->cfg.global_context) {
        Epilogue ep;
        ep.out_mode = OUT_F32;
        ep.out = m->buf.fold_out;
        ep.out_ld = m->att;
        ConvW cw = m->fold;
        cw.bias = nullptr;
        rc = add_gemm(cw, {{B_GSTAT, 0, 2 * C3, 0, 0, 0, 0}}, nullptr, 0, B, ep);
        if (rc) return rc;
    }
    if (pooling == PPV_POOL_ASP || pooling == PPV_POOL_SAP) {
        {
            Epilogue ep = planes_out(m->buf.bufs[B_ATT], 0, false);
            if (pooling == PPV_POOL_ASP) {
                if (m->cfg.global_context) ep.rowgrp_bias = m->buf.fold_out;
            } else {
                ep.relu = 0;
            }
            ep.tanh_ = 1;
            rc = add_gemm(m->att1, {{B_MFA, 0, C3, 0, 0, 0, 0}}, nullptr, 0, int(R), ep);
            if (rc) return rc;
        }
        {
            Step s;
            s.kind = Step::ASP_FUSED;
            rc = asp_fused_build(&s.ap, m->att2.W, m->buf.bufs[B_ATT], m->buf.bufs[B_MFA], m->buf.bufs[B_GSTAT], m->aspbn_scale, m->aspbn_shift,
                                 m->buf.bufs[B_POOL], m->buf.pooled_raw, B, T, P, Tp, C3, m->att, 1e-12f);
            if (rc) return rc;
            m->steps.push_back(s);
        }
    }
    {
        Epilogue ep;
        ep.out_mode = OUT_F32;
        ep.out = m->emb_out;
        ep.out_ld = m->cfg.embd_dim;
        const int Kp = (pooling == PPV_POOL_ASP || pooling == PPV_POOL_TSP) ? 2 * C3 : C3;
        rc = add_gemm(m->fc, {{B_POOL, 0, Kp, 0, 0, 0, 0}}, nullptr, 0, B, ep);
        if (rc) return rc;
    }
    return PPV_OK;
}

int EcapaModel::forward_ex(const float* feat, Fbank* fb, const float* wav, const float* lens_ratio, int B, int T, int L, float* emb, void* ws,
                           size_t ws_bytes, cudaStream_t st, const float* lengths) {
    int rc = forward_begin(emb, B, T);
    if (rc) return rc;
    PPV_REQUIRE((feat != nullptr) != (wav != nullptr), "ecapa_forward: exactly one of feat / wav");
    if (wav) {
        PPV_REQUIRE(fb, "ecapa_forward: wav input needs a fbank handle");
        PPV_REQUIRE(fbank_n_mels(fb) == cfg.input_size, "ecapa_forward: fbank n_mels != model input_size");
        PPV_REQUIRE(fbank_num_frames(fb, L) == T, "ecapa_forward: frame count mismatch");
    }
    rc = update_plan(B, T, ws, ws_bytes, st);
    if (!rc) rc = run(feat, fb, wav, lens_ratio, L, lengths, st);
    return rc ? rc : copy_embeddings(emb, st);
}

int ecapa_forward(Model* m, const float* feat, Fbank* fb, const float* wav, const float* lens_ratio, int B, int T, int L, float* emb, void* ws,
                  size_t ws_bytes, cudaStream_t st, const float* lengths) {
    return static_cast<EcapaModel*>(m)->forward_ex(feat, fb, wav, lens_ratio, B, T, L, emb, ws, ws_bytes, st, lengths);
}

int EcapaModel::run(const float* feat, Fbank* fb, const float* wav, const float* lens_ratio, int L, const float* lengths, cudaStream_t st) {
    EcapaModel* const m = this;
    const int B = m->plan_B, T = m->plan_T;
    const int Tp = m->Tp, P = m->P, C = m->C, C3 = m->C3;
    const int64_t R = int64_t(B) * Tp;
    int rc;
    auto prof_mark = [&](int kind, bool begin) {
        if (!m->prof_on) return;
        if (begin) {
            if (m->prof_used + 2 > m->prof_ev.size()) {
                cudaEvent_t a, b;
                cudaEventCreate(&a);
                cudaEventCreate(&b);
                m->prof_ev.push_back(a);
                m->prof_ev.push_back(b);
                m->prof_kind.push_back(kind);
            }
            m->prof_kind[m->prof_used / 2] = kind;
            cudaEventRecord(m->prof_ev[m->prof_used], st);
        } else {
            cudaEventRecord(m->prof_ev[m->prof_used + 1], st);
            m->prof_used += 2;
        }
    };
    const int* nv = nullptr;
    if (lengths) {
        PPV_REQUIRE(m->cfg.pooling == PPV_POOL_ASP, "ecapa_forward: lengths is implemented for ASP pooling (the other heads ignore it in the reference)");
        rc = launch_lengths_to_counts(lengths, B, T, m->buf.nvalid, st);
        if (rc) return rc;
        nv = m->buf.nvalid;
    }
    prof_mark(1, true);
    if (wav) {
        rc = fbank_run(fb, wav, lens_ratio, B, L, m->buf.raw_logmel, nullptr, m->buf.bufs[B_FEAT], P, Tp, st);
        m->launches_other += 3;
    } else {
        rc = launch_pack_features(feat, B, T, m->cfg.input_size, m->buf.bufs[B_FEAT], P, Tp, st);
        m->launches_other += 1;
    }
    prof_mark(1, false);
    if (rc) return rc;
    for (const Step& s : m->steps) {
        const bool tensor_step = (s.kind == Step::GEMM || s.kind == Step::ASP_FUSED || s.kind == Step::RES2 || s.kind == Step::RES2CHAIN);
        prof_mark(tensor_step ? 0 : 1, true);
        if (tensor_step) m->launches_gemm += 1; else m->launches_other += 1;
        switch (s.kind) {
            case Step::GEMM: rc = gemm_launch(s.gp, m->precision, m->num_sms, st); break;
            case Step::SKINNY: rc = skinny_linear_launch(s.sk_x, s.sk_col0, s.sk_w, s.sk_M, s.sk_N, s.sk_K, s.sk_ep, st); break;
            case Step::RES2: rc = res2conv_launch(s.rp, m->precision, m->num_sms, st); break;
            case Step::RES2CHAIN:
                rc = res2chain_launch(s.cp, m->precision, m->num_sms, st);
                if (s.cp.trace) {
                    static int dumps = 0;
                    if (++dumps == 10) res2chain_trace_dump(s.cp);
                }
                break;
            case Step::SE_SQUEEZE:
                rc = launch_colstats(m->buf.bufs[B_Z], 0, C, B, T, P, Tp, 0, 0.f, nullptr, m->buf.bufs[B_SEM], st, 0.f, nv);
                break;
            case Step::SE_SCALE: {
                const Planes& X = (s.blk == 1) ? m->buf.bufs[B_X0] : m->buf.bufs[B_CAT];
                const int xcol = (s.blk == 1) ? 0 : (s.blk - 2) * C;
                rc = launch_se_scale_res(m->buf.bufs[B_Z], m->buf.se_scale, X, xcol, m->buf.bufs[B_CAT], (s.blk - 1) * C, C, Tp, R, m->num_sms, st);
                break;
            }
            case Step::ASP_GLOBAL:
                rc = launch_colstats(m->buf.bufs[B_MFA], 0, C3, B, T, P, Tp, 1, 1e-12f, nullptr, m->buf.bufs[B_GSTAT], st, 0.f, nv);
                break;
            case Step::ASP_FUSED: {
                AspFusedParams ap = s.ap;
                ap.nvalid = nv;
                rc = asp_fused_launch(ap, m->precision, m->num_sms, st);
                break;
            }
            case Step::POOL_STATS:
                rc = launch_colstats(m->buf.bufs[B_MFA], 0, C3, B, T, P, Tp, m->cfg.pooling == PPV_POOL_TAP ? 0 : 3, 0.f, nullptr, m->buf.bufs[B_POOL], st);
                break;
        }
        prof_mark(0, false);
        if (rc) return rc;
    }
    return PPV_OK;
}

int ecapa_profile(Model* model, int enable) {
    EcapaModel* m = static_cast<EcapaModel*>(model);
    m->prof_on = enable != 0;
    m->prof_used = 0;
    m->launches_gemm = m->launches_other = 0;
    return PPV_OK;
}

int ecapa_profile_read(Model* model, double* gemm_ms, double* other_ms, int64_t* gemm_launches, int64_t* other_launches) {
    EcapaModel* m = static_cast<EcapaModel*>(model);
    PPV_REQUIRE(gemm_ms && other_ms && gemm_launches && other_launches, "ecapa_profile_read: null argument");
    double g = 0, o = 0;
    if (m->prof_used >= 2) PPV_CUDA_OK(cudaEventSynchronize(m->prof_ev[m->prof_used - 1]));
    for (size_t i = 0; i + 1 < m->prof_used; i += 2) {
        float ms = 0.f;
        PPV_CUDA_OK(cudaEventElapsedTime(&ms, m->prof_ev[i], m->prof_ev[i + 1]));
        (m->prof_kind[i / 2] == 0 ? g : o) += ms;
    }
    *gemm_ms = g;
    *other_ms = o;
    *gemm_launches = m->launches_gemm;
    *other_launches = m->launches_other;
    m->prof_used = 0;
    m->launches_gemm = m->launches_other = 0;
    return PPV_OK;
}

int EcapaModel::tap(const std::string& n, float* out, size_t out_elems, cudaStream_t st) {
    EcapaModel* const m = this;
    const int B = m->plan_B, T = m->plan_T, P = m->P, Tp = m->Tp, C = m->C, C3 = m->C3;
    const Planes* src = nullptr;
    int col0 = 0, cols = 0;
    if (n == "feat") {
        src = &m->buf.bufs[B_FEAT];
        cols = m->cfg.input_size;
    } else if (n == "blocks.0") {
        src = &m->buf.bufs[B_X0];
        cols = C;
    } else if (n == "blocks.1" || n == "blocks.2" || n == "blocks.3") {
        src = &m->buf.bufs[B_CAT];
        col0 = (n.back() - '1') * C;
        cols = C;
    } else if (n == "mfa") {
        src = &m->buf.bufs[B_MFA];
        cols = C3;
    } else if (n == "asp") {
        PPV_REQUIRE(out_elems >= size_t(B) * 2 * C3, "ecapa_read_tap: output too small");
        PPV_CUDA_OK(cudaMemcpyAsync(out, m->buf.pooled_raw, size_t(B) * 2 * C3 * 4, cudaMemcpyDeviceToDevice, st));
        return PPV_OK;
    } else {
        return fail(PPV_EINVAL, "ecapa_read_tap: unknown tap " + n);
    }
    PPV_REQUIRE(out_elems >= size_t(B) * T * cols, "ecapa_read_tap: output too small");
    return launch_planes_to_f32(*src, col0, cols, B, T, P, Tp, out, st);
}

}
```

### voiceprintrecognition-paddlepaddle_b200/csrc/elementwise.cu

```cuda
#include "common.h"
#include "ptx.cuh"

namespace ppv {

__device__ __forceinline__ float2 ld_split2(const __nv_bfloat16* hi, const __nv_bfloat16* lo, int64_t off) {
    const __nv_bfloat162 h = *reinterpret_cast<const __nv_bfloat162*>(hi + off);
    const __nv_bfloat162 l = *reinterpret_cast<const __nv_bfloat162*>(lo + off);
    const float2 hf = __bfloat1622float2(h);
    const float2 lf = __bfloat1622float2(l);
    return make_float2(hf.x + lf.x, hf.y + lf.y);
}
__device__ __forceinline__ void st_split2(__nv_bfloat16* hi, __nv_bfloat16* lo, int64_t off, float a, float b) {
    __nv_bfloat16 h0, l0, h1, l1;
    split_bf16(a, h0, l0);
    split_bf16(b, h1, l1);
    *reinterpret_cast<uint32_t*>(hi + off) = pack_bf16x2(h0, h1);
    *reinterpret_cast<uint32_t*>(lo + off) = pack_bf16x2(l0, l1);
}

__global__ void pack_features_kernel(const float* __restrict__ feat, int B, int T, int F, Planes out, int P, int Tp) {
    griddep_launch_dependents();
    griddep_wait();
    const int warps_per_block = blockDim.x >> 5;
    const int64_t frame = int64_t(blockIdx.x) * warps_per_block + (threadIdx.x >> 5);
    const int lane = threadIdx.x & 31;
    if (frame >= int64_t(B) * T) return;
    const int b = int(frame / T);
    const int t = int(frame - int64_t(b) * T);
    const float* src = feat + frame * F;
    const int64_t row = int64_t(b) * Tp + P + t;
    int64_t rows[3] = {row, -1, -1};
    if (t >= 1 && t <= P) rows[1] = row - 2 * t;
    const int u = T - 1 - t;
    if (u >= 1 && u <= P) rows[2] = row + 2 * u;
    for (int c = 2 * lane; c < out.ld; c += 64) {
        const float a = (c < F) ? src[c] : 0.f;
        const float bb = (c + 1 < F) ? src[c + 1] : 0.f;
#pragma unroll
        for (int k = 0; k < 3; ++k)
            if (rows[k] >= 0) st_split2(out.hi(), out.lo(), rows[k] * out.ld + c, a, bb);
    }
}

int launch_pack_features(const float* feat, int B, int T, int F, const Planes& out, int P, int Tp, cudaStream_t st) {
    const int64_t frames = int64_t(B) * T;
    const int wpb = 8;
    PPV_PDL_OK(launch_pdl(pack_features_kernel, dim3(unsigned((frames + wpb - 1) / wpb)), dim3(wpb * 32), 0, st, feat, B, T, F, out, P, Tp),
               "pack_features_kernel");
    return PPV_OK;
}

constexpr int STAT_WARPS = 8;

__device__ __forceinline__ float2 block_colsum(float2 v, float2 (*s_part)[32], int warp, int lane) {
    s_part[warp][lane] = v;
    __syncthreads();
    float2 r = make_float2(0.f, 0.f);
#pragma unroll
    for (int w = 0; w < STAT_WARPS; ++w) {
        r.x += s_part[w][lane].x;
        r.y += s_part[w][lane].y;
    }
    __syncthreads();
    return r;
}

__global__ void __launch_bounds__(STAT_WARPS * 32)
    colstats_kernel(Planes x, int col0, int C, int T_all, int P, int Tp, int mode, float eps, float inv_count, float* __restrict__ out_f32,
                    Planes out_pl, const int* __restrict__ nvalid) {
    __shared__ float s_s[STAT_WARPS][64];
    __shared__ float s_q[STAT_WARPS][64];
    griddep_launch_dependents();
    griddep_wait();
    const int b = blockIdx.y;
    const int T = nvalid ? max(1, min(T_all, nvalid[b])) : T_all;
    const int warp = threadIdx.x >> 5, lane = threadIdx.x & 31;
    const int cg = lane & 7, rsub = lane >> 3;
    const int c = col0 + blockIdx.x * 64 + cg * 8;
    const int64_t row0 = int64_t(b) * Tp + P;
    auto load8 = [&](int64_t row, float (&v)[8]) {
        const uint4 h = *reinterpret_cast<const uint4*>(x.hi() + row * x.ld + c);
        const uint4 l = *reinterpret_cast<const uint4*>(x.lo() + row * x.ld + c);
        const uint32_t hw[4] = {h.x, h.y, h.z, h.w}, lw[4] = {l.x, l.y, l.z, l.w};
#pragma unroll
        for (int i = 0; i < 4; ++i) {
            const float2 hf = __bfloat1622float2(*reinterpret_cast<const __nv_bfloat162*>(&hw[i]));
            const float2 lf = __bfloat1622float2(*reinterpret_cast<const __nv_bfloat162*>(&lw[i]));
            v[2 * i] = hf.x + lf.x;
            v[2 * i + 1] = hf.y + lf.y;
        }
    };
    float k[8], s[8], q[8];
    load8(row0, k);
#pragma unroll
    for (int i = 0; i < 8; ++i) s[i] = q[i] = 0.f;
#pragma unroll 4
    for (int t = warp * 4 + rsub; t < T; t += STAT_WARPS * 4) {
        float v[8];
        load8(row0 + t, v);
#pragma unroll
        for (int i = 0; i < 8; ++i) {
            const float d = v[i] - k[i];
            s[i] += d;
            q[i] = fmaf(d, d, q[i]);
        }
    }
#pragma unroll
    for (int i = 0; i < 8; ++i) {
        s[i] += __shfl_xor_sync(0xffffffffu, s[i], 8);
        s[i] += __shfl_xor_sync(0xffffffffu, s[i], 16);
        q[i] += __shfl_xor_sync(0xffffffffu, q[i], 8);
        q[i] += __shfl_xor_sync(0xffffffffu, q[i], 16);
    }
    if (rsub == 0) {
#pragma unroll
        for (int i = 0; i < 8; ++i) {
            s_s[warp][cg * 8 + i] = s[i];
            s_q[warp][cg * 8 + i] = q[i];
        }
    }
    __syncthreads();
    if (threadIdx.x < 64) {
        const int ch = threadIdx.x;
        float S = 0.f, Q = 0.f;
#pragma unroll
        for (int w = 0; w < STAT_WARPS; ++w) {
            S += s_s[w][ch];
            Q += s_q[w][ch];
        }
        const int64_t off0 = row0 * x.ld + col0 + blockIdx.x * 64 + ch;
        const float K = __bfloat162float(x.hi()[off0]) + __bfloat162float(x.lo()[off0]);
        const float inv = inv_count > 0.f ? inv_count : 1.f / float(T);
        const float mean = (inv_count > 0.f ? K * float(T) * inv : K) + S * inv;
        const int cc = blockIdx.x * 64 + ch;
        if (mode == 0) {
            if (out_f32) out_f32[int64_t(b) * C + cc] = mean;
            if (out_pl.base) {
                __nv_bfloat16 h, l;
                split_bf16(mean, h, l);
                out_pl.hi()[int64_t(b) * out_pl.ld + cc] = h;
                out_pl.lo()[int64_t(b) * out_pl.ld + cc] = l;
            }
        } else {
            const float ssq = Q - S * S * inv;
            const float sd = (mode == 2)   ? sqrtf(fmaxf(ssq, 0.f) / float(T > 1 ? T - 1 : 1) + eps)
                             : (mode == 3) ? fmaxf(ssq, 0.f) / float(T > 1 ? T - 1 : 1)
                                           : sqrtf(fmaxf(ssq * inv, eps));
            __nv_bfloat16 h, l;
            split_bf16(mean, h, l);
            out_pl.hi()[int64_t(b) * out_pl.ld + cc] = h;
            out_pl.lo()[int64_t(b) * out_pl.ld + cc] = l;
            split_bf16(sd, h, l);
            out_pl.hi()[int64_t(b) * out_pl.ld + C + cc] = h;
            out_pl.lo()[int64_t(b) * out_pl.ld + C + cc] = l;
        }
    }
}

__global__ void lengths_to_counts_kernel(const float* __restrict__ lengths, int B, int T, int* __restrict__ nvalid) {
    griddep_launch_dependents();
    griddep_wait();
    const int b = blockIdx.x * blockDim.x + threadIdx.x;
    if (b >= B) return;
    const float lim = lengths[b] * float(T);
    int n = 0;
    for (int t = 0; t < T; ++t) n += (float(t) < lim) ? 1 : 0;
    nvalid[b] = n;
}
int launch_lengths_to_counts(const float* lengths, int B, int T, int* nvalid, cudaStream_t st) {
    PPV_PDL_OK(launch_pdl(lengths_to_counts_kernel, dim3((B + 127) / 128), dim3(128), 0, st, lengths, B, T, nvalid), "lengths_to_counts_kernel");
    return PPV_OK;
}

int launch_colstats(const Planes& x, int col0, int C, int B, int T, int P, int Tp, int mode, float eps, float* out_f32,
                    const Planes& out_pl, cudaStream_t st, float inv_count, const int* nvalid) {
    PPV_REQUIRE(C % 64 == 0 && col0 % 8 == 0 && x.ld % 8 == 0, "colstats: C % 64, col0 % 8, ld % 8 required");
    dim3 grid(C / 64, B);
    PPV_PDL_OK(launch_pdl(colstats_kernel, grid, dim3(STAT_WARPS * 32), 0, st, x, col0, C, T, P, Tp, mode, eps, inv_count, out_f32, out_pl, nvalid),
               "colstats_kernel");
    return PPV_OK;
}

__device__ __forceinline__ void unpack8(const uint4& h, const uint4& l, float (&v)[8]) {
    const uint32_t hw[4] = {h.x, h.y, h.z, h.w}, lw[4] = {l.x, l.y, l.z, l.w};
#pragma unroll
    for (int i = 0; i < 4; ++i) {
        const float2 hf = __bfloat1622float2(*reinterpret_cast<const __nv_bfloat162*>(&hw[i]));
        const float2 lf = __bfloat1622float2(*reinterpret_cast<const __nv_bfloat162*>(&lw[i]));
        v[2 * i] = hf.x + lf.x;
        v[2 * i + 1] = hf.y + lf.y;
    }
}
__global__ void __launch_bounds__(256)
    se_scale_res_kernel(Planes z, const float* __restrict__ scale, Planes res, int rc0, Planes out, int oc0, int C, int Tp,
                        int64_t rows, int relu, float relu_max) {
    griddep_launch_dependents();
    griddep_wait();
    const int groups = C >> 3;
    const int64_t total = rows * groups;
    for (int64_t i = int64_t(blockIdx.x) * blockDim.x + threadIdx.x; i < total; i += int64_t(gridDim.x) * blockDim.x) {
        const int64_t r = i / groups;
        const int c = int(i - r * groups) * 8;
        const int b = int(r / Tp);
        float zv[8], rv[8];
        unpack8(*reinterpret_cast<const uint4*>(z.hi() + r * z.ld + c), *reinterpret_cast<const uint4*>(z.lo() + r * z.ld + c), zv);
        unpack8(*reinterpret_cast<const uint4*>(res.hi() + r * res.ld + rc0 + c),
                *reinterpret_cast<const uint4*>(res.lo() + r * res.ld + rc0 + c), rv);
        float4 s0 = make_float4(1.f, 1.f, 1.f, 1.f), s1 = s0;
        if (scale) {
            s0 = *reinterpret_cast<const float4*>(scale + int64_t(b) * C + c);
            s1 = *reinterpret_cast<const float4*>(scale + int64_t(b) * C + c + 4);
        }
        const float sv[8] = {s0.x, s0.y, s0.z, s0.w, s1.x, s1.y, s1.z, s1.w};
        uint32_t h[4], l[4];
#pragma unroll
        for (int k = 0; k < 4; ++k) {
            __nv_bfloat16 h0, l0, h1, l1;
            float y0 = fmaf(sv[2 * k], zv[2 * k], rv[2 * k]), y1 = fmaf(sv[2 * k + 1], zv[2 * k + 1], rv[2 * k + 1]);
            if (relu) {
                y0 = fmaxf(y0, 0.f);
                y1 = fmaxf(y1, 0.f);
                if (relu_max > 0.f) {
                    y0 = fminf(y0, relu_max);
                    y1 = fminf(y1, relu_max);
                }
            }
            split_bf16(y0, h0, l0);
            split_bf16(y1, h1, l1);
            h[k] = pack_bf16x2(h0, h1);
            l[k] = pack_bf16x2(l0, l1);
        }
        *reinterpret_cast<uint4*>(out.hi() + r * out.ld + oc0 + c) = make_uint4(h[0], h[1], h[2], h[3]);
        *reinterpret_cast<uint4*>(out.lo() + r * out.ld + oc0 + c) = make_uint4(l[0], l[1], l[2], l[3]);
    }
}

int launch_se_scale_res(const Planes& z, const float* scale, const Planes& res, int rc0, const Planes& out, int oc0, int C,
                        int Tp, int64_t rows, int num_sms, cudaStream_t st, int relu, float relu_max) {
    PPV_REQUIRE(C % 8 == 0 && rc0 % 8 == 0 && oc0 % 8 == 0, "se_scale_res: 8-channel alignment required");
    const int64_t total = rows * (C / 8);
    const int64_t want = (total + 255) / 256;
    const int grid = int(std::min<int64_t>(want, int64_t(num_sms) * 16));
    PPV_PDL_OK(launch_pdl(se_scale_res_kernel, dim3(grid), dim3(256), 0, st, z, scale, res, rc0, out, oc0, C, Tp, rows, relu, relu_max), "se_scale_res_kernel");
    return PPV_OK;
}

__global__ void __launch_bounds__(STAT_WARPS * 32)
    asp_pool_kernel(const float* __restrict__ logits, int64_t lg_ld, Planes x, int C, int T, int P, int Tp, float eps,
                    const float* __restrict__ bn_scale, const float* __restrict__ bn_shift, Planes out_pl,
                    float* __restrict__ out_raw) {
    __shared__ float2 s_part[STAT_WARPS][32];
    const int b = blockIdx.y;
    const int warp = threadIdx.x >> 5, lane = threadIdx.x & 31;
    const int c = blockIdx.x * 64 + 2 * lane;
    const int64_t row0 = int64_t(b) * Tp + P;
    float2 mx = make_float2(-INFINITY, -INFINITY);
    for (int t = warp; t < T; t += STAT_WARPS) {
        const float2 l = *reinterpret_cast<const float2*>(logits + (row0 + t) * lg_ld + c);
        mx.x = fmaxf(mx.x, l.x);
        mx.y = fmaxf(mx.y, l.y);
    }
    s_part[warp][lane] = mx;
    __syncthreads();
#pragma unroll
    for (int w = 0; w < STAT_WARPS; ++w) {
        mx.x = fmaxf(mx.x, s_part[w][lane].x);
        mx.y = fmaxf(mx.y, s_part[w][lane].y);
    }
    __syncthreads();
    float2 se = make_float2(0.f, 0.f), sx = make_float2(0.f, 0.f);
    for (int t = warp; t < T; t += STAT_WARPS) {
        const float2 l = *reinterpret_cast<const float2*>(logits + (row0 + t) * lg_ld + c);
        const float2 v = ld_split2(x.hi(), x.lo(), (row0 + t) * x.ld + c);
        const float ex = expf(l.x - mx.x), ey = expf(l.y - mx.y);
        se.x += ex;
        se.y += ey;
        sx.x = fmaf(ex, v.x, sx.x);
        sx.y = fmaf(ey, v.y, sx.y);
    }
    se = block_colsum(se, s_part, warp, lane);
    sx = block_colsum(sx, s_part, warp, lane);
    const float2 inv = make_float2(1.f / se.x, 1.f / se.y);
    const float2 mean = make_float2(sx.x * inv.x, sx.y * inv.y);
    float2 sv = make_float2(0.f, 0.f);
    for (int t = warp; t < T; t += STAT_WARPS) {
        const float2 l = *reinterpret_cast<const float2*>(logits + (row0 + t) * lg_ld + c);
        const float2 v = ld_split2(x.hi(), x.lo(), (row0 + t) * x.ld + c);
        const float ax = expf(l.x - mx.x) * inv.x, ay = expf(l.y - mx.y) * inv.y;
        const float dx = v.x - mean.x, dy = v.y - mean.y;
        sv.x = fmaf(ax, dx * dx, sv.x);
        sv.y = fmaf(ay, dy * dy, sv.y);
    }
    sv = block_colsum(sv, s_part, warp, lane);
    if (warp == 0) {
        const float stdx = sqrtf(fmaxf(sv.x, eps)), stdy = sqrtf(fmaxf(sv.y, eps));
        if (out_raw) {
            *reinterpret_cast<float2*>(out_raw + int64_t(b) * 2 * C + c) = mean;
            *reinterpret_cast<float2*>(out_raw + int64_t(b) * 2 * C + C + c) = make_float2(stdx, stdy);
        }
        if (!bn_scale || !out_pl.base) return;
        const float2 s0 = *reinterpret_cast<const float2*>(bn_scale + c), h0 = *reinterpret_cast<const float2*>(bn_shift + c);
        const float2 s1 = *reinterpret_cast<const float2*>(bn_scale + C + c),
                     h1 = *reinterpret_cast<const float2*>(bn_shift + C + c);
        st_split2(out_pl.hi(), out_pl.lo(), int64_t(b) * out_pl.ld + c, fmaf(mean.x, s0.x, h0.x), fmaf(mean.y, s0.y, h0.y));
        st_split2(out_pl.hi(), out_pl.lo(), int64_t(b) * out_pl.ld + C + c, fmaf(stdx, s1.x, h1.x), fmaf(stdy, s1.y, h1.y));
    }
}

int launch_asp_pool(const float* logits, int64_t lg_ld, const Planes& x, int C, int B, int T, int P, int Tp, float eps,
                    const float* bn_scale, const float* bn_shift, const Planes& out_pl, float* out_raw, cudaStream_t st) {
    PPV_REQUIRE(C % 64 == 0, "asp_pool: C must be a multiple of 64");
    dim3 grid(C / 64, B);
    asp_pool_kernel<<<grid, STAT_WARPS * 32, 0, st>>>(logits, lg_ld, x, C, T, P, Tp, eps, bn_scale, bn_shift, out_pl, out_raw);
    PPV_LAUNCH_OK("asp_pool_kernel");
    return PPV_OK;
}

__global__ void __launch_bounds__(256)
    aff_combine_kernel(Planes x, int xc0, Planes y, int yc0, Planes t, Planes out, int C, int64_t rows) {
    griddep_launch_dependents();
    griddep_wait();
    const int groups = C >> 3;
    const int64_t total = rows * groups;
    for (int64_t i = int64_t(blockIdx.x) * blockDim.x + threadIdx.x; i < total; i += int64_t(gridDim.x) * blockDim.x) {
        const int64_t r = i / groups;
        const int c = int(i - r * groups) * 8;
        float xv[8], yv[8], tv[8];
        unpack8(*reinterpret_cast<const uint4*>(x.hi() + r * x.ld + xc0 + c), *reinterpret_cast<const uint4*>(x.lo() + r * x.ld + xc0 + c), xv);
        unpack8(*reinterpret_cast<const uint4*>(y.hi() + r * y.ld + yc0 + c), *reinterpret_cast<const uint4*>(y.lo() + r * y.ld + yc0 + c), yv);
        unpack8(*reinterpret_cast<const uint4*>(t.hi() + r * t.ld + c), *reinterpret_cast<const uint4*>(t.lo() + r * t.ld + c), tv);
        uint32_t h[4], l[4];
#pragma unroll
        for (int k = 0; k < 4; ++k) {
            __nv_bfloat16 h0, l0, h1, l1;
            split_bf16(fmaf(xv[2 * k], 1.f + tv[2 * k], yv[2 * k] * (1.f - tv[2 * k])), h0, l0);
            split_bf16(fmaf(xv[2 * k + 1], 1.f + tv[2 * k + 1], yv[2 * k + 1] * (1.f - tv[2 * k + 1])), h1, l1);
            h[k] = pack_bf16x2(h0, h1);
            l[k] = pack_bf16x2(l0, l1);
        }
        *reinterpret_cast<uint4*>(out.hi() + r * out.ld + c) = make_uint4(h[0], h[1], h[2], h[3]);
        *reinterpret_cast<uint4*>(out.lo() + r * out.ld + c) = make_uint4(l[0], l[1], l[2], l[3]);
    }
}

int launch_aff_combine(const Planes& x, int xc0, const Planes& y, int yc0, const Planes& t, const Planes& out, int C, int64_t rows, int num_sms,
                       cudaStream_t st) {
    PPV_REQUIRE(C % 8 == 0 && xc0 % 8 == 0 && yc0 % 8 == 0, "aff_combine: 8-channel alignment required");
    const int64_t total = rows * (C / 8);
    const int grid = int(std::min<int64_t>((total + 255) / 256, int64_t(num_sms) * 16));
    PPV_PDL_OK(launch_pdl(aff_combine_kernel, dim3(grid), dim3(256), 0, st, x, xc0, y, yc0, t, out, C, rows), "aff_combine_kernel");
    return PPV_OK;
}

__global__ void planes_to_f32_kernel(Planes x, int col0, int C, int B, int T, int P, int Tp, float* __restrict__ out) {
    const int64_t total = int64_t(B) * T * C;
    for (int64_t i = int64_t(blockIdx.x) * blockDim.x + threadIdx.x; i < total; i += int64_t(gridDim.x) * blockDim.x) {
        const int c = int(i % C);
        const int64_t f = i / C;
        const int b = int(f / T), t = int(f % T);
        const int64_t off = (int64_t(b) * Tp + P + t) * x.ld + col0 + c;
        out[i] = __bfloat162float(x.hi()[off]) + __bfloat162float(x.lo()[off]);
    }
}

int launch_planes_to_f32(const Planes& x, int col0, int C, int B, int T, int P, int Tp, float* out, cudaStream_t st) {
    const int64_t total = int64_t(B) * T * C;
    const int grid = int(std::min<int64_t>((total + 255) / 256, 132 * 32));
    planes_to_f32_kernel<<<grid, 256, 0, st>>>(x, col0, C, B, T, P, Tp, out);
    PPV_LAUNCH_OK("planes_to_f32_kernel");
    return PPV_OK;
}

__global__ void f32_to_planes_kernel(const float* __restrict__ src, int64_t rows, int cols, Planes out) {
    const int64_t total = rows * cols;
    for (int64_t i = int64_t(blockIdx.x) * blockDim.x + threadIdx.x; i < total; i += int64_t(gridDim.x) * blockDim.x) {
        const int64_t r = i / cols;
        const int c = int(i - r * cols);
        __nv_bfloat16 h, l;
        split_bf16(src[i], h, l);
        out.hi()[r * out.ld + c] = h;
        out.lo()[r * out.ld + c] = l;
    }
}

int launch_f32_to_planes(const float* src, int64_t rows, int cols, const Planes& out, cudaStream_t st) {
    const int64_t total = rows * cols;
    const int grid = int(std::min<int64_t>((total + 255) / 256, 132 * 32));
    f32_to_planes_kernel<<<grid, 256, 0, st>>>(src, rows, cols, out);
    PPV_LAUNCH_OK("f32_to_planes_kernel");
    return PPV_OK;
}

}
```

### voiceprintrecognition-paddlepaddle_b200/csrc/gemm_epilogue.cuh

```cuda
#pragma once
#include "common.h"
#include "ptx.cuh"

namespace ppv {

constexpr int GEMM_MMA_THREADS = 256;
constexpr int GEMM_THREADS = 128 + GEMM_MMA_THREADS;

__device__ __forceinline__ float epilogue_math1(const Epilogue& ep, int N, int col, int64_t grp, int64_t sgrp, float x) {
    if (ep.bias) x += __ldg(ep.bias + col);
    if (ep.rowgrp_bias) x += __ldg(ep.rowgrp_bias + grp * N + col);
    if (ep.seg_scale) x *= __ldg(ep.seg_scale + sgrp * N + col);
    if (ep.relu) {
        x = fmaxf(x, 0.f);
        if (ep.relu_max > 0.f) x = fminf(x, ep.relu_max);
    }
    if (ep.silu_) x = x / (1.f + expf(-x));
    if (ep.bn_scale) x = fmaf(x, __ldg(ep.bn_scale + col), __ldg(ep.bn_shift + col));
    if (ep.tanh_) x = tanhf(x);
    if (ep.sigmoid_) x = 1.f / (1.f + expf(-x));
    return x;
}

struct EpiRow {
    bool valid = false;
    int64_t out_row = 0, mirror_a = -1, mirror_b = -1, grp = 0, sgrp = 0;
    int64_t zero_row = -1;
};
__device__ __forceinline__ EpiRow epilogue_row(const Epilogue& ep, int64_t row, int64_t out_row_shift) {
    EpiRow r;
    r.valid = row >= 0;
    const int64_t row_in = row;
    if (row < 0) row = 0;
    r.out_row = row + out_row_shift;
    if (ep.img_Wp > 0) {
        const int64_t img = int64_t(ep.img_Hp) * ep.img_Wp;
        r.grp = row / img;
        const int rem = int(row - r.grp * img);
        const int h = rem / ep.img_Wp - 1, w = rem % ep.img_Wp - 1;
        r.valid = r.valid && h >= 0 && h < ep.img_H && w >= 0 && w < ep.img_W;
        const int sw = ep.img_stride_w ? ep.img_stride_w : ep.img_stride;
        r.valid = r.valid && (h % ep.img_stride) == 0 && (w % sw) == 0;
        r.out_row = (r.grp * ep.out_Hp + h / ep.img_stride + 1) * ep.out_Wp + w / sw + 1;
    } else if (ep.Tp > 0) {
        r.grp = row / ep.Tp;
        const int t = int(row - r.grp * ep.Tp) - ep.P;
        r.valid = r.valid && t >= 0 && t < ep.T;
        if (ep.seg_scale && r.valid) r.sgrp = r.grp * ep.nseg + t / ep.seg_len;
        if (ep.halo && r.valid) {
            if (t >= 1 && t <= ep.P) r.mirror_a = row - 2 * t;
            const int u = ep.T - 1 - t;
            if (u >= 1 && u <= ep.P) r.mirror_b = row + 2 * u;
        }
    }
    const bool same_grid = ep.img_Wp == 0 || (ep.img_stride == 1 && ep.img_stride_w <= 1 && ep.out_Hp == ep.img_Hp && ep.out_Wp == ep.img_Wp);
    if (!r.valid && row_in >= 0 && ep.zero_invalid && ep.out_mode == OUT_PLANES && !ep.halo && same_grid) r.zero_row = row_in + out_row_shift;
    return r;
}

__device__ __forceinline__ void epilogue_pair(const Epilogue& ep, int N, int col, const EpiRow& r, float a, float b) {
    if (col >= N) return;
    if (!r.valid) {
        if (r.zero_row >= 0) {
            __nv_bfloat16* ph = static_cast<__nv_bfloat16*>(ep.out) + r.zero_row * ep.out_ld + ep.out_col0 + col;
            *reinterpret_cast<uint32_t*>(ph) = 0u;
            *reinterpret_cast<uint32_t*>(ph + ep.out_plane_stride) = 0u;
        }
        return;
    }
    const bool two = col + 1 < N;
    a = epilogue_math1(ep, N, col, r.grp, r.sgrp, a);
    if (two) b = epilogue_math1(ep, N, col + 1, r.grp, r.sgrp, b);
    if (ep.out_mode == OUT_F32) {
        float* dst = static_cast<float*>(ep.out) + r.out_row * ep.out_ld + ep.out_col0 + col;
        if (two && ep.f32_vec_ok) {
            *reinterpret_cast<float2*>(dst) = make_float2(a, b);
        } else {
            dst[0] = a;
            if (two) dst[1] = b;
        }
        return;
    }
    uint32_t h, l;
    split_pack_bf16x2(a, b, h, l);
    __nv_bfloat16* obase = static_cast<__nv_bfloat16*>(ep.out) + ep.out_col0 + col;
    auto store_row = [&](int64_t row) {
        uint32_t* ph = reinterpret_cast<uint32_t*>(obase + row * ep.out_ld);
        ph[0] = h;
        *reinterpret_cast<uint32_t*>(reinterpret_cast<__nv_bfloat16*>(ph) + ep.out_plane_stride) = l;
    };
    store_row(r.out_row);
    if (r.mirror_a >= 0) store_row(r.mirror_a);
    if (r.mirror_b >= 0) store_row(r.mirror_b);
}

template <int BN, typename RowOf>
__device__ __forceinline__ void epilogue_frag(const Epilogue& ep, int N, int n0, float (&acc)[BN / 2], RowOf&& row_of, int t,
                                              int64_t out_row_shift = 0) {
    if (ep.debug_nostore) return;
    const int w = t >> 5, l = t & 31;
    const int r0 = 16 * w + (l >> 2);
    const EpiRow ra = epilogue_row(ep, row_of(r0), out_row_shift);
    const EpiRow rb = epilogue_row(ep, row_of(r0 + 8), out_row_shift);
    constexpr int EPI_GROUPS = BN / 8 < 4 ? BN / 8 : 4;
#pragma unroll 1
    for (int c = 0; c < BN / 8; c += EPI_GROUPS) {
#pragma unroll
        for (int i = 0; i < EPI_GROUPS; ++i) {
            const int col = n0 + 8 * (c + i) + 2 * (l & 3);
            epilogue_pair(ep, N, col, ra, acc[4 * i + 0], acc[4 * i + 1]);
            epilogue_pair(ep, N, col, rb, acc[4 * i + 2], acc[4 * i + 3]);
        }
#pragma unroll
        for (int j = 0; j + 4 * EPI_GROUPS < BN / 2; ++j) acc[j] = acc[j + 4 * EPI_GROUPS];
    }
}

__device__ __forceinline__ void quad_transpose_pairs(float (&a)[8], float (&b)[8], int q) {
    const bool q2 = (q & 2) != 0, q1 = (q & 1) != 0;
#pragma unroll
    for (int e = 0; e < 4; ++e) {
        const float sa = q2 ? a[e] : a[e + 4], sb = q2 ? b[e] : b[e + 4];
        const float ra_ = __shfl_xor_sync(0xffffffffu, sa, 2), rb_ = __shfl_xor_sync(0xffffffffu, sb, 2);
        if (q2) a[e] = ra_, b[e] = rb_;
        else a[e + 4] = ra_, b[e + 4] = rb_;
    }
#pragma unroll
    for (int e = 0; e < 8; e += 4) {
#pragma unroll
        for (int f = 0; f < 2; ++f) {
            const float sa = q1 ? a[e + f] : a[e + 2 + f], sb = q1 ? b[e + f] : b[e + 2 + f];
            const float ra_ = __shfl_xor_sync(0xffffffffu, sa, 1), rb_ = __shfl_xor_sync(0xffffffffu, sb, 1);
            if (q1) a[e + f] = ra_, b[e + f] = rb_;
            else a[e + 2 + f] = ra_, b[e + 2 + f] = rb_;
        }
    }
}

template <int BN, typename RowOf>
__device__ __forceinline__ void epilogue_frag_lean(const Epilogue& ep, int N, int n0, float (&acc)[BN / 2], RowOf&& row_of, int t) {
    static_assert(BN % 32 == 0, "lean epilogue: whole 32-column trips");
    const int w = t >> 5, l = t & 31, q = l & 3;
    const int r0 = 16 * w + (l >> 2);
    const EpiRow ra = epilogue_row(ep, row_of(r0), 0);
    const EpiRow rb = epilogue_row(ep, row_of(r0 + 8), 0);
    const int cq = n0 + 8 * q;
    __nv_bfloat16* const obase = static_cast<__nv_bfloat16*>(ep.out) + ep.out_col0 + cq;
    __nv_bfloat16* const pa = obase + ra.out_row * ep.out_ld;
    __nv_bfloat16* const pb = obase + rb.out_row * ep.out_ld;
    const int64_t lo_off = ep.out_plane_stride;
    const float* const ga = ep.rowgrp_bias ? ep.rowgrp_bias + ra.grp * N + cq : nullptr;
    const float* const gb = ep.rowgrp_bias ? ep.rowgrp_bias + rb.grp * N + cq : nullptr;
#pragma unroll 1
    for (int c = 0; c < BN / 8; c += 4) {
        float a[8], b[8];
#pragma unroll
        for (int i = 0; i < 4; ++i) a[2 * i] = acc[4 * i], a[2 * i + 1] = acc[4 * i + 1], b[2 * i] = acc[4 * i + 2], b[2 * i + 1] = acc[4 * i + 3];
#pragma unroll
        for (int j = 0; j + 16 < BN / 2; ++j) acc[j] = acc[j + 16];
        quad_transpose_pairs(a, b, q);
        const int j0 = 8 * c;
        if (n0 + j0 >= N) continue;
#pragma unroll
        for (int k = 0; k < 8; ++k) {
            const int col = cq + j0 + k;
            if (ep.bias) {
                const float bb = __ldg(ep.bias + col);
                a[k] += bb, b[k] += bb;
            }
            if (ga) a[k] += __ldg(ga + j0 + k), b[k] += __ldg(gb + j0 + k);
            if (ep.relu) a[k] = fmaxf(a[k], 0.f), b[k] = fmaxf(b[k], 0.f);
            if (ep.bn_scale) {
                const float sc = __ldg(ep.bn_scale + col), sh = __ldg(ep.bn_shift + col);
                a[k] = fmaf(a[k], sc, sh), b[k] = fmaf(b[k], sc, sh);
            }
            if (ep.tanh_) a[k] = tanhf(a[k]), b[k] = tanhf(b[k]);
        }
        uint4 ha, la, hb, lb;
        split_pack_bf16x2(a[0], a[1], ha.x, la.x), split_pack_bf16x2(a[2], a[3], ha.y, la.y);
        split_pack_bf16x2(a[4], a[5], ha.z, la.z), split_pack_bf16x2(a[6], a[7], ha.w, la.w);
        split_pack_bf16x2(b[0], b[1], hb.x, lb.x), split_pack_bf16x2(b[2], b[3], hb.y, lb.y);
        split_pack_bf16x2(b[4], b[5], hb.z, lb.z), split_pack_bf16x2(b[6], b[7], hb.w, lb.w);
        if (ra.valid) {
            *reinterpret_cast<uint4*>(pa + j0) = ha;
            *reinterpret_cast<uint4*>(pa + j0 + lo_off) = la;
        }
        if (rb.valid) {
            *reinterpret_cast<uint4*>(pb + j0) = hb;
            *reinterpret_cast<uint4*>(pb + j0 + lo_off) = lb;
        }
    }
}

template <int BN, typename RowOf>
__device__ __forceinline__ void gemm_epilogue(const Epilogue& ep, int N, int n0, float (&acc)[BN / 2], RowOf&& row_of, int t,
                                              int64_t out_row_shift) {
    if (ep.lean) epilogue_frag_lean<BN>(ep, N, n0, acc, row_of, t);
    else epilogue_frag<BN>(ep, N, n0, acc, row_of, t, out_row_shift);
}

}
```

### voiceprintrecognition-paddlepaddle_b200/csrc/gemm_wgmma.cu

```cuda
#include <stdio.h>
#include <stdlib.h>
#include <string.h>

#include <algorithm>
#include <mutex>

#include "common.h"
#include "gemm_epilogue.cuh"
#include "ptx.cuh"

namespace ppv {

template <int BN, int NSPLIT, int BK>
struct GemmCfg {
    static constexpr int NA = (NSPLIT == 3) ? 2 : 1;
    static constexpr int NB = NA;
    static constexpr int A_BYTES = GEMM_BM * BK * 2;
    static constexpr int B_BYTES = BN * BK * 2;
    static constexpr int STAGE_BYTES = NA * A_BYTES + NB * B_BYTES;
    static constexpr int BAR_BYTES = 256;
    static constexpr int MAX_SMEM = 232448;
    static constexpr int STAGES_RAW = (MAX_SMEM - 1024 - BAR_BYTES) / STAGE_BYTES;
    static constexpr int MAX_STAGES = 8;
    static constexpr int STAGES = STAGES_RAW > MAX_STAGES ? MAX_STAGES : STAGES_RAW;
    static constexpr int SMEM_BYTES = 1024 + STAGES * STAGE_BYTES + BAR_BYTES;
    static constexpr bool PINGPONG = BN <= 128;
    static constexpr int EMPTY_ARRIVALS = PINGPONG ? 1 : GEMM_MMA_THREADS / 128;
    static_assert(STAGES >= 2, "need at least a double buffer");
    static_assert(BN == 64 || BN == 128 || BN == 256, "BN");
    static_assert(BK == 64 || BK == 32, "BK");
};

template <int BK>
__device__ __forceinline__ uint64_t make_kmajor_desc(uint32_t smem_addr) {
    return BK == 64 ? make_sw128_kmajor_desc(smem_addr) : make_sw64_kmajor_desc(smem_addr);
}

template <int BN, int NSPLIT, int BK>
__global__ void __launch_bounds__(GEMM_THREADS, 1) gemm_wgmma_kernel(const __grid_constant__ GemmParams gp) {
    using Cfg = GemmCfg<BN, NSPLIT, BK>;
    constexpr int STAGES = Cfg::STAGES;
    extern __shared__ uint8_t smem_raw[];
    const uint32_t smem_base = (smem_u32(smem_raw) + 1023u) & ~1023u;
    const uint32_t tiles_base = smem_base;
    const uint32_t bar_base = smem_base + STAGES * Cfg::STAGE_BYTES;
    constexpr int MAXST = Cfg::MAX_STAGES;
    auto full_bar = [&](int s) { return bar_base + 8u * s; };
    auto empty_bar = [&](int s) { return bar_base + 8u * (MAXST + s); };
    const uint32_t w_full = bar_base + 8u * (2 * MAXST);

    const int warp = threadIdx.x >> 5;
    const int lane = threadIdx.x & 31;
    const int nst = gp.ws ? GEMM_WS_STAGES : STAGES;
    const uint32_t w_res = tiles_base + GEMM_WS_STAGES * Cfg::STAGE_BYTES;

    if (warp == 0 && lane == 0) {
        for (int i = 0; i < GEMM_MAX_MAPS; ++i) prefetch_tmap(&gp.mapA[i]);
        prefetch_tmap(&gp.mapB);
    }
    if (warp == 1 && lane == 0) {
        for (int s = 0; s < MAXST; ++s) {
            mbar_init(full_bar(s), 1);
            mbar_init(empty_bar(s), Cfg::EMPTY_ARRIVALS);
        }
        mbar_init(w_full, 1);
        fence_mbar_init();
    }
    __syncthreads();
    griddep_launch_dependents();
    griddep_wait();

    const int mn_tiles = gp.m_tiles * gp.n_tiles;
    const int num_tiles = mn_tiles * (gp.lin_splits > 0 ? gp.lin_splits : 1);
    const int nk = gp.num_ksteps;
    auto tile_m = [&](int t) { return (t % mn_tiles) / gp.n_tiles; };
    auto tile_n = [&](int t) { return (t % mn_tiles) % gp.n_tiles; };
    const bool trace_cta = gp.trace != nullptr && blockIdx.x == 0;
    auto stamp = [&](bool on, int role, int local, int ev) {
        if (on) gp.trace[(role * GEMM_TRACE_TILES + local) * 8 + ev] = clock64();
    };
    stamp(trace_cta && threadIdx.x == 0, 0, 0, 7);

    if (warp < 4) {
        setmaxnreg_dec<40>();
        if (warp == 0) {
            int stage = 0;
            uint32_t phase = 0;
            if (gp.ws && lane == 0) {
                mbar_arrive_expect_tx(w_full, nk * Cfg::NB * Cfg::B_BYTES);
                for (int s = 0; s < nk; ++s)
                    for (int p = 0; p < Cfg::NB; ++p) tma_load_3d(w_res + (s * Cfg::NB + p) * Cfg::B_BYTES, &gp.mapB, w_full, s * BK, 0, p);
            }
            __syncwarp();
            int local = 0;
            for (int tile = blockIdx.x; tile < num_tiles; tile += gridDim.x, ++local) {
                const bool tr = trace_cta && lane == 0 && local < GEMM_TRACE_TILES;
                const int zsplit = tile / mn_tiles;
                const int m0 = tile_m(tile) * GEMM_BM;
                const int n0 = tile_n(tile) * BN;
                const int ntile = tile + gridDim.x;
                if (gp.l2_prefetch && ntile < num_tiles && tile_n(ntile) == 0 && lane < nk && gp.lin_splits == 0) {
                    const int nm0 = tile_m(ntile) * GEMM_BM;
                    for (int s = lane; s < nk; s += 32) {
                        const KStep ks = gp.ksteps[s];
#pragma unroll
                        for (int p = 0; p < Cfg::NA; ++p) tma_prefetch_l2_3d(&gp.mapA[ks.map], ks.a_col, nm0 + ks.row_off, p);
                    }
                }
                __syncwarp();
                for (int s = 0; s < nk; ++s) {
                    mbar_wait(empty_bar(stage), phase ^ 1u);
                    stamp(tr && s == 0, 0, local, 0);
                    stamp(tr && s == nk - 1, 0, local, 1);
                    if (lane == 0) {
                        const uint32_t sa = tiles_base + stage * Cfg::STAGE_BYTES;
                        const uint32_t sb = sa + Cfg::NA * Cfg::A_BYTES;
                        const uint32_t fb = full_bar(stage);
                        mbar_arrive_expect_tx(fb, gp.ws ? Cfg::NA * Cfg::A_BYTES : Cfg::STAGE_BYTES);
                        if (gp.ws) {
                            const KStep ks = gp.ksteps[s];
#pragma unroll
                            for (int p = 0; p < Cfg::NA; ++p) tma_load_3d(sa + p * Cfg::A_BYTES, &gp.mapA[ks.map], fb, ks.a_col, m0 + ks.row_off, p);
                        } else if (gp.lin_splits > 0) {
                            const int kcol = (zsplit * nk + s) * BK;
#pragma unroll
                            for (int p = 0; p < Cfg::NA; ++p) tma_load_3d(sa + p * Cfg::A_BYTES, &gp.mapA[0], fb, kcol, m0, p);
#pragma unroll
                            for (int p = 0; p < Cfg::NB; ++p)
                                tma_load_3d(sb + p * Cfg::B_BYTES, &gp.mapB, fb, kcol + gp.lin_b_col0, gp.lin_b_row0 + n0, p);
                        } else {
                            const KStep ks = gp.ksteps[s];
                            const CUtensorMap* ma = &gp.mapA[ks.map];
#pragma unroll
                            for (int p = 0; p < Cfg::NA; ++p) tma_load_3d(sa + p * Cfg::A_BYTES, ma, fb, ks.a_col, m0 + ks.row_off, p);
#pragma unroll
                            for (int p = 0; p < Cfg::NB; ++p) tma_load_3d(sb + p * Cfg::B_BYTES, &gp.mapB, fb, s * BK, n0, p);
                        }
                    }
                    __syncwarp();
                    if (++stage == nst) {
                        stage = 0;
                        phase ^= 1u;
                    }
                }
            }
        }
    } else if constexpr (Cfg::PINGPONG) {
        setmaxnreg_inc<232>();
        const int g = (warp - 4) >> 2;
        const int t = threadIdx.x & 127;
        constexpr uint32_t A_HALF = 64 * BK * 2;
        const int my_tiles = blockIdx.x < num_tiles ? (num_tiles - 1 - int(blockIdx.x)) / int(gridDim.x) + 1 : 0;
        int stage = 0;
        uint32_t phase = 0;
        float acc0[BN / 2], acc1[BN / 2];
#pragma unroll
        for (int i = 0; i < BN / 2; ++i) acc0[i] = acc1[i] = 0.f;
        if (gp.ws) mbar_wait(w_full, 0);
        int local = 0;
        for (int tile = blockIdx.x; tile < num_tiles; tile += gridDim.x, ++local) {
            if ((local & 1) != g) {
                const int adv = stage + nk;
                phase ^= uint32_t((adv / nst) & 1);
                stage = adv % nst;
                continue;
            }
            const int m0 = tile_m(tile) * GEMM_BM;
            const int n0 = tile_n(tile) * BN;
            const bool tr = trace_cta && t == 0 && local < GEMM_TRACE_TILES;
            named_bar_sync_if(local > 0, 1 + g, 2 * 128);
            stamp(tr, 1 + g, local, 0);
            int prev = -1;
            wgmma_fence_acc(acc0);
            wgmma_fence_acc(acc1);
            for (int s = 0; s < nk; ++s) {
                mbar_wait(full_bar(stage), phase);
                stamp(tr && s == 0, 1 + g, local, 1);
                const uint32_t sa = tiles_base + stage * Cfg::STAGE_BYTES;
                const uint32_t sb = gp.ws ? w_res + s * Cfg::NB * Cfg::B_BYTES : sa + Cfg::NA * Cfg::A_BYTES;
                const uint64_t a0_hi = make_kmajor_desc<BK>(sa), a1_hi = make_kmajor_desc<BK>(sa + A_HALF);
                const uint64_t b_hi = make_kmajor_desc<BK>(sb);
                wgmma_fence();
#pragma unroll
                for (int k = 0; k < BK / 16; ++k) {
                    wgmma_bf16<BN>(acc0, a0_hi + 2 * k, b_hi + 2 * k, (s > 0 || k > 0) ? 1u : 0u);
                    wgmma_bf16<BN>(acc1, a1_hi + 2 * k, b_hi + 2 * k, (s > 0 || k > 0) ? 1u : 0u);
                }
                if (NSPLIT == 3) {
                    const uint64_t a0_lo = make_kmajor_desc<BK>(sa + Cfg::A_BYTES), a1_lo = make_kmajor_desc<BK>(sa + Cfg::A_BYTES + A_HALF);
                    const uint64_t b_lo = make_kmajor_desc<BK>(sb + Cfg::B_BYTES);
#pragma unroll
                    for (int k = 0; k < BK / 16; ++k) {
                        wgmma_bf16<BN>(acc0, a0_lo + 2 * k, b_hi + 2 * k, 1u);
                        wgmma_bf16<BN>(acc1, a1_lo + 2 * k, b_hi + 2 * k, 1u);
                    }
#pragma unroll
                    for (int k = 0; k < BK / 16; ++k) {
                        wgmma_bf16<BN>(acc0, a0_hi + 2 * k, b_lo + 2 * k, 1u);
                        wgmma_bf16<BN>(acc1, a1_hi + 2 * k, b_lo + 2 * k, 1u);
                    }
                }
                wgmma_commit();
                stamp(tr && s == nk - 1, 1 + g, local, 2);
                wgmma_wait<1>();
                if (prev >= 0 && t == 0) mbar_arrive(empty_bar(prev));
                prev = stage;
                if (++stage == nst) {
                    stage = 0;
                    phase ^= 1u;
                }
            }
            wgmma_wait<0>();
            stamp(tr, 1 + g, local, 3);
            named_bar_arrive_if(local + 1 < my_tiles, 1 + (g ^ 1), 2 * 128);
            wgmma_fence_acc(acc0);
            wgmma_fence_acc(acc1);
            if (t == 0) mbar_arrive(empty_bar(prev));
            stamp(tr, 1 + g, local, 4);
            const int64_t shift = int64_t(tile / mn_tiles) * gp.lin_split_rows;
#pragma unroll 1
            for (int h = 0; h < 2; ++h) {
                const int rbase = m0 + 64 * h;
                gemm_epilogue<BN>(gp.epi, gp.N, n0, acc0, [&](int r) -> int64_t { return rbase + r < gp.M ? int64_t(rbase + r) : -1; }, t, shift);
#pragma unroll
                for (int i = 0; i < BN / 2; ++i) acc0[i] = acc1[i];
            }
            stamp(tr, 1 + g, local, 5);
        }
    } else {
        setmaxnreg_inc<232>();
        const int g = (warp - 4) >> 2;
        const int t = threadIdx.x & 127;
        constexpr uint32_t A_WG_OFF = 64 * BK * 2;
        int stage = 0;
        uint32_t phase = 0;
        float acc[BN / 2];
#pragma unroll
        for (int i = 0; i < BN / 2; ++i) acc[i] = 0.f;
        if (gp.ws) mbar_wait(w_full, 0);
        int local = 0;
        for (int tile = blockIdx.x; tile < num_tiles; tile += gridDim.x, ++local) {
            const int m0 = tile_m(tile) * GEMM_BM;
            const int n0 = tile_n(tile) * BN;
            const bool tr = trace_cta && t == 0 && local < GEMM_TRACE_TILES;
            stamp(tr, 1 + g, local, 0);
            int prev = -1;
            wgmma_fence_acc(acc);
            for (int s = 0; s < nk; ++s) {
                mbar_wait(full_bar(stage), phase);
                stamp(tr && s == 0, 1 + g, local, 1);
                const uint32_t sa = tiles_base + stage * Cfg::STAGE_BYTES;
                const uint32_t sb = gp.ws ? w_res + s * Cfg::NB * Cfg::B_BYTES : sa + Cfg::NA * Cfg::A_BYTES;
                const uint64_t a_hi = make_kmajor_desc<BK>(sa + g * A_WG_OFF);
                const uint64_t b_hi = make_kmajor_desc<BK>(sb);
                wgmma_fence();
#pragma unroll
                for (int k = 0; k < BK / 16; ++k) wgmma_bf16<BN>(acc, a_hi + 2 * k, b_hi + 2 * k, (s > 0 || k > 0) ? 1u : 0u);
                if (NSPLIT == 3) {
                    const uint64_t a_lo = make_kmajor_desc<BK>(sa + Cfg::A_BYTES + g * A_WG_OFF);
                    const uint64_t b_lo = make_kmajor_desc<BK>(sb + Cfg::B_BYTES);
#pragma unroll
                    for (int k = 0; k < BK / 16; ++k) wgmma_bf16<BN>(acc, a_lo + 2 * k, b_hi + 2 * k, 1u);
#pragma unroll
                    for (int k = 0; k < BK / 16; ++k) wgmma_bf16<BN>(acc, a_hi + 2 * k, b_lo + 2 * k, 1u);
                }
                wgmma_commit();
                stamp(tr && s == nk - 1, 1 + g, local, 2);
                wgmma_wait<1>();
                if (prev >= 0 && t == 0) mbar_arrive(empty_bar(prev));
                prev = stage;
                if (++stage == nst) {
                    stage = 0;
                    phase ^= 1u;
                }
            }
            wgmma_wait<0>();
            stamp(tr, 1 + g, local, 3);
            wgmma_fence_acc(acc);
            if (t == 0) mbar_arrive(empty_bar(prev));
            stamp(tr, 1 + g, local, 4);
            const int64_t shift = int64_t(tile / mn_tiles) * gp.lin_split_rows;
            const int rbase = m0 + 64 * g;
            gemm_epilogue<BN>(gp.epi, gp.N, n0, acc, [&](int r) -> int64_t { return rbase + r < gp.M ? int64_t(rbase + r) : -1; }, t, shift);
            stamp(tr, 1 + g, local, 5);
        }
    }
}

typedef CUresult (*EncodeTiledFn)(CUtensorMap*, CUtensorMapDataType, cuuint32_t, void*, const cuuint64_t*,
                                  const cuuint64_t*, const cuuint32_t*, const cuuint32_t*, CUtensorMapInterleave,
                                  CUtensorMapSwizzle, CUtensorMapL2promotion, CUtensorMapFloatOOBfill);

static EncodeTiledFn get_encode_fn() {
    static EncodeTiledFn fn = nullptr;
    static std::once_flag once;
    std::call_once(once, [] {
        void* p = nullptr;
        cudaDriverEntryPointQueryResult q;
        if (cudaGetDriverEntryPoint("cuTensorMapEncodeTiled", &p, cudaEnableDefault, &q) == cudaSuccess &&
            q == cudaDriverEntryPointSuccess)
            fn = reinterpret_cast<EncodeTiledFn>(p);
    });
    return fn;
}

int encode_planes_map_ex(CUtensorMap* m, const Planes& t, int box_cols, int box_rows, int swizzle_bytes) {
    EncodeTiledFn enc = get_encode_fn();
    if (!enc) return fail(PPV_ECUDA, "cuTensorMapEncodeTiled entry point not available");
    if ((reinterpret_cast<uintptr_t>(t.base) & 15) || (t.ld % 8) || (t.plane_stride % 8))
        return fail(PPV_EINVAL, "planes tensor not 16-byte aligned");
    cuuint64_t dims[3] = {cuuint64_t(t.ld), cuuint64_t(t.rows), 2};
    cuuint64_t strides[2] = {cuuint64_t(t.ld) * 2, cuuint64_t(t.plane_stride) * 2};
    cuuint32_t box[3] = {cuuint32_t(box_cols), cuuint32_t(box_rows), 1};
    cuuint32_t estr[3] = {1, 1, 1};
    CUresult r = enc(m, CU_TENSOR_MAP_DATA_TYPE_BFLOAT16, 3, t.base, dims, strides, box, estr, CU_TENSOR_MAP_INTERLEAVE_NONE,
                     swizzle_bytes == 128 ? CU_TENSOR_MAP_SWIZZLE_128B : swizzle_bytes == 64 ? CU_TENSOR_MAP_SWIZZLE_64B : CU_TENSOR_MAP_SWIZZLE_NONE,
                     CU_TENSOR_MAP_L2_PROMOTION_L2_256B,
                     CU_TENSOR_MAP_FLOAT_OOB_FILL_NONE);
    if (r != CUDA_SUCCESS) return fail(PPV_ECUDA, "cuTensorMapEncodeTiled failed, CUresult " + std::to_string(int(r)));
    return PPV_OK;
}

int encode_planes_map(CUtensorMap* m, const Planes& t, int box_rows) { return encode_planes_map_ex(m, t, GEMM_BK, box_rows, 128); }

int gemm_build(GemmParams* gp, const GemmSource* srcs, int nsrc, const Planes& W, int M, int N, const Epilogue& epi,
               int BN, int BK) {
    if (BK == 0) {
        BK = 64;
        for (int i = 0; i < nsrc; ++i)
            if (srcs[i].ncols % 64) BK = 32;
    }
    PPV_REQUIRE(BK == 64 || BK == 32, "gemm_build: BK must be 64 or 32");
    PPV_REQUIRE(BN == 64 || BN == 128 || BN == 256, "gemm_build: BN must be 64/128/256");
    PPV_REQUIRE(epi.out_mode == OUT_F32 || N % 32 == 0, "gemm_build: planes output needs N % 32 == 0");
    PPV_REQUIRE(!epi.rowgrp_bias || N % 32 == 0, "gemm_build: row-group bias needs N % 32 == 0");
    memset(gp, 0, sizeof(*gp));
    const __nv_bfloat16* bases[GEMM_MAX_MAPS];
    int nmaps = 0;
    int ks = 0;
    for (int i = 0; i < nsrc; ++i) {
        const GemmSource& s = srcs[i];
        PPV_REQUIRE(s.ncols % BK == 0 && s.col0 % 8 == 0, "gemm_build: source K slice must be a multiple of the k-step");
        PPV_REQUIRE(s.col0 + s.ncols <= s.t.ld, "gemm_build: source K slice exceeds the row");
        int mi = -1;
        for (int j = 0; j < nmaps; ++j)
            if (bases[j] == s.t.base) mi = j;
        if (mi < 0) {
            PPV_REQUIRE(nmaps < GEMM_MAX_MAPS, "gemm_build: too many distinct A tensors");
            mi = nmaps++;
            bases[mi] = s.t.base;
            int rc = encode_planes_map_ex(&gp->mapA[mi], s.t, BK, GEMM_BM, BK * 2);
            if (rc) return rc;
        }
        for (int c = 0; c < s.ncols; c += BK) {
            PPV_REQUIRE(ks < GEMM_MAX_KSTEPS, "gemm_build: too many k-steps");
            gp->ksteps[ks].map = int16_t(mi);
            gp->ksteps[ks].row_off = int16_t(s.row_off);
            gp->ksteps[ks].a_col = s.col0 + c;
            ++ks;
        }
    }
    for (int j = nmaps; j < GEMM_MAX_MAPS; ++j) gp->mapA[j] = gp->mapA[0];
    PPV_REQUIRE(ks > 0, "gemm_build: empty K");
    PPV_REQUIRE(W.ld == ks * BK, "gemm_build: weight K does not match the k-steps");
    PPV_REQUIRE(W.rows >= N, "gemm_build: weight rows < N");
    int rc = encode_planes_map_ex(&gp->mapB, W, BK, BN, BK * 2);
    if (rc) return rc;
    gp->num_ksteps = ks;
    gp->bk = BK;
    gp->M = M;
    gp->N = N;
    gp->m_tiles = (M + GEMM_BM - 1) / GEMM_BM;
    gp->n_tiles = (N + BN - 1) / BN;
    gp->bn = BN;
    gp->epi = epi;
    {
        const size_t stage_bytes = size_t(2) * GEMM_BM * BK * 2 + size_t(2) * BN * BK * 2;
        const size_t stages_full = std::min<size_t>(8, (232448 - 1024 - 256) / stage_bytes);
        const size_t w_bytes = size_t(ks) * 2 * BN * BK * 2;
        const char* wsenv = getenv("PPV_GEMM_WS");
        gp->ws = (gp->n_tiles == 1 && stages_full > GEMM_WS_STAGES && w_bytes <= (stages_full - GEMM_WS_STAGES) * stage_bytes && gp->m_tiles >= 264 &&
                  !(wsenv && wsenv[0] == '0'))
                     ? 1
                     : 0;
    }
    {
        const char* ns = getenv("PPV_GEMM_NOSTORE");
        gp->epi.debug_nostore = (ns && ns[0] == '1') ? 1 : 0;
        const char* pf = getenv("PPV_GEMM_NO_L2PREFETCH");
        gp->l2_prefetch = (pf && pf[0] == '1') ? 0 : 1;
    }
    if (getenv("PPV_GEMM_TRACE")) {
        static unsigned long long* buf = nullptr;
        if (!buf) {
            PPV_CUDA_OK(cudaMalloc(reinterpret_cast<void**>(&buf), 3 * GEMM_TRACE_TILES * 8 * sizeof(unsigned long long)));
            PPV_CUDA_OK(cudaMemset(buf, 0, 3 * GEMM_TRACE_TILES * 8 * sizeof(unsigned long long)));
        }
        gp->trace = buf;
    }
    if (epi.out_mode == OUT_PLANES) {
        PPV_REQUIRE((epi.out_ld % 16) == 0 && (epi.out_col0 % 16) == 0 && (epi.out_plane_stride % 16) == 0 &&
                        (reinterpret_cast<uintptr_t>(epi.out) & 15) == 0,
                    "gemm_build: planes output must be 16-byte aligned");
        gp->epi.lean = (!epi.halo && !epi.zero_invalid && epi.img_Wp == 0 && !epi.seg_scale && !epi.silu_ && !epi.sigmoid_ &&
                        !(epi.relu && epi.relu_max > 0.f) && !gp->epi.debug_nostore)
                           ? 1
                           : 0;
    } else {
        gp->epi.f32_vec_ok = ((epi.out_ld % 2) == 0 && (epi.out_col0 % 2) == 0 && (reinterpret_cast<uintptr_t>(epi.out) & 7) == 0) ? 1 : 0;
    }
    return PPV_OK;
}

int gemm_build_wgrad(GemmParams* gp, const Planes& At, const Planes& Bt, int M, int N, int b_row0, int b_col0, int splits, float* out,
                     int64_t out_ld, int out_col0, int64_t split_rows, int BN) {
    PPV_REQUIRE(BN == 64 || BN == 128 || BN == 256, "gemm_build_wgrad: BN must be 64/128/256");
    PPV_REQUIRE(At.ld == Bt.ld && splits >= 1, "gemm_build_wgrad: operands must share the contraction length");
    memset(gp, 0, sizeof(*gp));
    int rc = encode_planes_map_ex(&gp->mapA[0], At, GEMM_BK, GEMM_BM, 128);
    if (rc) return rc;
    for (int j = 1; j < GEMM_MAX_MAPS; ++j) gp->mapA[j] = gp->mapA[0];
    rc = encode_planes_map_ex(&gp->mapB, Bt, GEMM_BK, BN, 128);
    if (rc) return rc;
    const int nk_total = (At.ld + GEMM_BK - 1) / GEMM_BK;
    gp->lin_splits = std::min(splits, nk_total);
    gp->num_ksteps = (nk_total + gp->lin_splits - 1) / gp->lin_splits;
    gp->lin_b_row0 = b_row0;
    gp->lin_b_col0 = b_col0;
    gp->lin_split_rows = split_rows;
    gp->bk = GEMM_BK;
    gp->M = M;
    gp->N = N;
    gp->m_tiles = (M + GEMM_BM - 1) / GEMM_BM;
    gp->n_tiles = (N + BN - 1) / BN;
    gp->bn = BN;
    Epilogue ep;
    ep.out_mode = OUT_F32;
    ep.out = out;
    ep.out_ld = out_ld;
    ep.out_col0 = out_col0;
    gp->epi = ep;
    gp->epi.f32_vec_ok = ((out_ld % 2) == 0 && (out_col0 % 2) == 0 && (reinterpret_cast<uintptr_t>(out) & 7) == 0) ? 1 : 0;
    PPV_REQUIRE(N % 32 == 0, "gemm_build_wgrad: N % 32 == 0 required");
    return PPV_OK;
}

template <int BN, int NSPLIT, int BK>
static int launch_one(const GemmParams& gp, int num_sms, cudaStream_t stream) {
    using Cfg = GemmCfg<BN, NSPLIT, BK>;
    PPV_ONCE_PER_DEVICE(PPV_CUDA_OK(cudaFuncSetAttribute(gemm_wgmma_kernel<BN, NSPLIT, BK>, cudaFuncAttributeMaxDynamicSharedMemorySize,
                                         Cfg::SMEM_BYTES)));
    const int tiles = gp.m_tiles * gp.n_tiles * (gp.lin_splits > 0 ? gp.lin_splits : 1);
    const int grid = std::min(tiles, num_sms);
    PPV_PDL_OK(launch_pdl(gemm_wgmma_kernel<BN, NSPLIT, BK>, dim3(grid), dim3(GEMM_THREADS), Cfg::SMEM_BYTES, stream, gp),
               "gemm_wgmma_kernel");
    return PPV_OK;
}

template <int BN>
static int launch_bn(const GemmParams& gp, bool x3, int num_sms, cudaStream_t stream) {
    if (gp.bk == 32) return x3 ? launch_one<BN, 3, 32>(gp, num_sms, stream) : launch_one<BN, 1, 32>(gp, num_sms, stream);
    return x3 ? launch_one<BN, 3, 64>(gp, num_sms, stream) : launch_one<BN, 1, 64>(gp, num_sms, stream);
}

void gemm_trace_dump(const GemmParams& gp) {
    if (!gp.trace) return;
    unsigned long long h[3 * GEMM_TRACE_TILES * 8];
    cudaDeviceSynchronize();
    cudaMemcpy(h, gp.trace, sizeof(h), cudaMemcpyDeviceToHost);
    const unsigned long long t0 = h[7];
    auto at = [&](int r, int i, int e) -> long long { const unsigned long long v = h[(r * GEMM_TRACE_TILES + i) * 8 + e]; return v ? (long long)(v - t0) : -1ll; };
    printf("gemm trace M=%d N=%d nk=%d BN=%d (cycles from kernel start)\n", gp.M, gp.N, gp.num_ksteps, gp.bn);
    for (int i = 0; i < GEMM_TRACE_TILES; ++i)
        if (at(0, i, 0) >= 0) printf("gemm trace tma  tile %2d: first slot %8lld  last slot %8lld\n", i, at(0, i, 0), at(0, i, 1));
    for (int r = 1; r < 3; ++r) {
        long long prev_end = -1;
        for (int i = 0; i < GEMM_TRACE_TILES; ++i) {
            if (at(r, i, 0) < 0) continue;
            printf("gemm trace wg%d  tile %2d:", r - 1, i);
            for (int e = 0; e < 6; ++e) printf(" %8lld", at(r, i, e));
            printf("   wait %6lld  kloop %6lld  epi %6lld  period %6lld\n", at(r, i, 1) - at(r, i, 0), at(r, i, 3) - at(r, i, 1),
                   at(r, i, 5) - at(r, i, 4), prev_end >= 0 ? at(r, i, 5) - prev_end : -1ll);
            prev_end = at(r, i, 5);
        }
    }
    fflush(stdout);
}

int gemm_launch(const GemmParams& gp, int precision, int num_sms, cudaStream_t stream) {
    const bool x3 = (precision == PPV_PREC_BF16X3);
    switch (gp.bn) {
        case 64: return launch_bn<64>(gp, x3, num_sms, stream);
        case 128: return launch_bn<128>(gp, x3, num_sms, stream);
        case 256: return launch_bn<256>(gp, x3, num_sms, stream);
    }
    return fail(PPV_EINVAL, "gemm_launch: bad BN");
}

}
```

### voiceprintrecognition-paddlepaddle_b200/csrc/skinny.cu

```cuda
#include "common.h"
#include "ptx.cuh"

namespace ppv {

namespace {

constexpr int SK_R = 16, SK_C = 16;
constexpr int SK_KC = 512;
constexpr int SK_LD = SK_KC + 4;
constexpr int SK_ITERS = (SK_R + SK_C) * (SK_KC / 8) / 256;
constexpr int SK_SMEM = (SK_R + SK_C) * SK_LD * 4;

__global__ void __launch_bounds__(256) skinny_linear_kernel(Planes x, int x_col0, Planes W, int M, int N, int K, Epilogue ep) {
    extern __shared__ __align__(16) float sk_smem[];
    float(*sx)[SK_LD] = reinterpret_cast<float(*)[SK_LD]>(sk_smem);
    float(*sw)[SK_LD] = reinterpret_cast<float(*)[SK_LD]>(sk_smem + SK_R * SK_LD);
    griddep_launch_dependents();
    griddep_wait();
    const int r0 = blockIdx.y * SK_R, c0 = blockIdx.x * SK_C;
    const int tid = threadIdx.x;
    const int lr = tid & 15, lc = tid >> 4;
    uint4 rh[SK_ITERS], rl[SK_ITERS];
    auto fetch = [&](int k0) {
        const int kc = min(SK_KC, K - k0);
#pragma unroll
        for (int it = 0; it < SK_ITERS; ++it) {
            const int i = tid + it * 256;
            const int row = i / (SK_KC / 8), seg = i - row * (SK_KC / 8);
            const bool is_x = row < SK_R;
            const int gr = is_x ? r0 + row : c0 + (row - SK_R);
            rh[it] = rl[it] = make_uint4(0u, 0u, 0u, 0u);
            if (seg * 8 < kc && gr < (is_x ? M : N)) {
                const Planes& p = is_x ? x : W;
                const int64_t off = int64_t(gr) * p.ld + (is_x ? x_col0 : 0) + k0 + seg * 8;
                rh[it] = *reinterpret_cast<const uint4*>(p.hi() + off);
                rl[it] = *reinterpret_cast<const uint4*>(p.lo() + off);
            }
        }
    };
    auto stash = [&]() {
#pragma unroll
        for (int it = 0; it < SK_ITERS; ++it) {
            const int i = tid + it * 256;
            const int row = i / (SK_KC / 8), seg = i - row * (SK_KC / 8);
            const uint32_t hw[4] = {rh[it].x, rh[it].y, rh[it].z, rh[it].w}, lw[4] = {rl[it].x, rl[it].y, rl[it].z, rl[it].w};
            float v[8];
#pragma unroll
            for (int j = 0; j < 4; ++j) {
                const float2 a = unpack_bf16x2(hw[j]), b = unpack_bf16x2(lw[j]);
                v[2 * j] = a.x + b.x;
                v[2 * j + 1] = a.y + b.y;
            }
            float* dst = row < SK_R ? &sx[row][seg * 8] : &sw[row - SK_R][seg * 8];
            *reinterpret_cast<float4*>(dst) = make_float4(v[0], v[1], v[2], v[3]);
            *reinterpret_cast<float4*>(dst + 4) = make_float4(v[4], v[5], v[6], v[7]);
        }
    };
    float acc0 = 0.f, acc1 = 0.f, acc2 = 0.f, acc3 = 0.f;
    fetch(0);
    for (int k0 = 0; k0 < K; k0 += SK_KC) {
        const int kc = min(SK_KC, K - k0);
        stash();
        __syncthreads();
        if (k0 + SK_KC < K) fetch(k0 + SK_KC);
        const float* px = sx[lr];
        const float* pw = sw[lc];
#pragma unroll 4
        for (int k = 0; k < kc; k += 4) {
            const float4 a = *reinterpret_cast<const float4*>(px + k);
            const float4 b = *reinterpret_cast<const float4*>(pw + k);
            acc0 = fmaf(a.x, b.x, acc0);
            acc1 = fmaf(a.y, b.y, acc1);
            acc2 = fmaf(a.z, b.z, acc2);
            acc3 = fmaf(a.w, b.w, acc3);
        }
        __syncthreads();
    }
    const int r = r0 + lr, c = c0 + lc;
    if (r >= M || c >= N) return;
    float y = (acc0 + acc1) + (acc2 + acc3);
    if (ep.bias) y += ep.bias[c];
    if (ep.relu) y = fmaxf(y, 0.f);
    if (ep.sigmoid_) y = 1.f / (1.f + expf(-y));
    if (ep.out_mode == OUT_F32) {
        static_cast<float*>(ep.out)[int64_t(r) * ep.out_ld + ep.out_col0 + c] = y;
    } else {
        __nv_bfloat16 h, l;
        split_bf16(y, h, l);
        __nv_bfloat16* o = static_cast<__nv_bfloat16*>(ep.out) + int64_t(r) * ep.out_ld + ep.out_col0 + c;
        o[0] = h;
        o[ep.out_plane_stride] = l;
    }
}

}

bool skinny_linear_supported(int M, int N, int K, const Epilogue& ep) {
    return M <= 4096 && K % 8 == 0 && K <= 1024 && !ep.rowgrp_bias && !ep.seg_scale && !ep.bn_scale && !ep.tanh_ && !ep.silu_ && ep.Tp == 0 && ep.img_Wp == 0 &&
           ep.relu_max == 0.f;
}

int skinny_linear_launch(const Planes& x, int x_col0, const Planes& W, int M, int N, int K, const Epilogue& ep, cudaStream_t st) {
    PPV_REQUIRE(skinny_linear_supported(M, N, K, ep), "skinny_linear: unsupported shape / epilogue");
    PPV_REQUIRE(x.ld % 8 == 0 && x_col0 % 8 == 0 && W.ld == K, "skinny_linear: operand layout");
    dim3 grid((N + SK_C - 1) / SK_C, (M + SK_R - 1) / SK_R);
    PPV_ONCE_PER_DEVICE(PPV_CUDA_OK(cudaFuncSetAttribute(skinny_linear_kernel, cudaFuncAttributeMaxDynamicSharedMemorySize, SK_SMEM)));
    PPV_PDL_OK(launch_pdl(skinny_linear_kernel, grid, dim3(256), size_t(SK_SMEM), st, x, x_col0, W, M, N, K, ep), "skinny_linear_kernel");
    return PPV_OK;
}

}
```

### voiceprintrecognition-paddlepaddle_b200/ppvector/_lib.py

```python
import ctypes as C
import os

_HERE = os.path.dirname(os.path.abspath(__file__))
LIB_PATH = os.path.normpath(os.path.join(_HERE, "..", "lib", "libppv_b200.so"))

PPV_PREC_BF16X3 = 0
PPV_PREC_BF16 = 1
PPV_MODEL_ECAPA_TDNN = 1
PPV_POOL_ASP, PPV_POOL_SAP, PPV_POOL_TAP, PPV_POOL_TSP = 0, 1, 2, 3


class PPVError(RuntimeError):
    pass


class FbankCfg(C.Structure):
    _fields_ = [("sample_rate", C.c_int), ("n_mels", C.c_int), ("frame_length_ms", C.c_float),
                ("frame_shift_ms", C.c_float), ("preemph", C.c_float), ("low_freq", C.c_float),
                ("high_freq", C.c_float), ("log_floor", C.c_float)]


class EcapaCfg(C.Structure):
    _fields_ = [("input_size", C.c_int), ("embd_dim", C.c_int), ("channels", C.c_int * 5),
                ("kernel_sizes", C.c_int * 5), ("dilations", C.c_int * 5), ("attention_channels", C.c_int),
                ("res2net_scale", C.c_int), ("se_channels", C.c_int), ("precision", C.c_int), ("pooling", C.c_int),
                ("global_context", C.c_int)]


class ResNetSECfg(C.Structure):
    _fields_ = [("input_size", C.c_int), ("embd_dim", C.c_int), ("layers", C.c_int * 4), ("num_filters", C.c_int * 4),
                ("attention_channels", C.c_int), ("reduction", C.c_int), ("precision", C.c_int)]


PPV_MODEL_RESNET_SE = 2
PPV_MODEL_ERES2NET = 3


class ERes2NetCfg(C.Structure):
    _fields_ = [("input_size", C.c_int), ("embd_dim", C.c_int), ("num_blocks", C.c_int * 4), ("m_channels", C.c_int),
                ("precision", C.c_int), ("version", C.c_int), ("base_width", C.c_int)]


PPV_MODEL_CAMPPLUS = 4
PPV_SPEC_SPECTROGRAM, PPV_SPEC_MEL, PPV_SPEC_LOGMEL, PPV_SPEC_MFCC = 1, 2, 3, 4
PPV_SPECAUG_NPARAM = 16
PPV_PREP_NI, PPV_PREP_NF = 8, 4
PPV_HEAD_AAM, PPV_HEAD_AAM_EASY, PPV_HEAD_AM, PPV_HEAD_ARM, PPV_HEAD_CE = 0, 1, 2, 3, 4
PPV_HEAD_SUBCENTER = 16
PPV_HEAD_SPHEREFACE2 = 8


class SpectralCfg(C.Structure):
    _fields_ = [("method", C.c_int), ("sample_rate", C.c_int), ("n_fft", C.c_int), ("hop_length", C.c_int), ("win_length", C.c_int),
                ("power", C.c_float), ("center", C.c_int), ("n_mels", C.c_int), ("f_min", C.c_float), ("f_max", C.c_float),
                ("htk", C.c_int), ("norm_slaney", C.c_int), ("ref_value", C.c_float), ("amin", C.c_float), ("n_mfcc", C.c_int)]


class CamPPlusCfg(C.Structure):
    _fields_ = [("input_size", C.c_int), ("embd_dim", C.c_int), ("growth_rate", C.c_int), ("bn_size", C.c_int),
                ("init_channels", C.c_int), ("precision", C.c_int)]


_P = C.c_void_p
SIGNATURES = {
    "ppv_version": (C.c_int, []),
    "ppv_last_error": (C.c_int, [C.c_char_p, C.c_size_t]),
    "ppv_device_sm_count": (C.c_int, []),
    "ppv_fbank_default_cfg": (None, [C.POINTER(FbankCfg)]),
    "ppv_fbank_create": (C.c_int, [C.POINTER(FbankCfg), C.POINTER(_P)]),
    "ppv_fbank_destroy": (C.c_int, [_P]),
    "ppv_fbank_num_frames": (C.c_int, [_P, C.c_int]),
    "ppv_fbank_feature_dim": (C.c_int, [_P]),
    "ppv_fbank_forward": (C.c_int, [_P, _P, _P, C.c_int, C.c_int, _P, _P]),
    "ppv_spectral_default_cfg": (None, [C.POINTER(SpectralCfg), C.c_int]),
    "ppv_spectral_create": (C.c_int, [C.POINTER(SpectralCfg), C.POINTER(_P)]),
    "ppv_spectral_destroy": (C.c_int, [_P]),
    "ppv_spectral_num_frames": (C.c_int, [_P, C.c_int]),
    "ppv_spectral_feature_dim": (C.c_int, [_P]),
    "ppv_spectral_forward": (C.c_int, [_P, _P, _P, C.c_int, C.c_int, _P, _P]),
    "ppv_spec_augment": (C.c_int, [_P, _P, C.c_int, C.c_int, C.c_int, C.c_int, C.c_int, C.c_int, _P]),
    "ppv_ecapa_default_cfg": (None, [C.POINTER(EcapaCfg)]),
    "ppv_resnetse_default_cfg": (None, [C.POINTER(ResNetSECfg)]),
    "ppv_eres2net_default_cfg": (None, [C.POINTER(ERes2NetCfg)]),
    "ppv_campplus_default_cfg": (None, [C.POINTER(CamPPlusCfg)]),
    "ppv_model_create": (C.c_int, [C.c_int, _P, C.POINTER(_P)]),
    "ppv_model_destroy": (C.c_int, [_P]),
    "ppv_model_load_weight": (C.c_int, [_P, C.c_char_p, _P, C.POINTER(C.c_int64), C.c_int]),
    "ppv_model_finalize": (C.c_int, [_P]),
    "ppv_model_set_precision": (C.c_int, [_P, C.c_int]),
    "ppv_model_embd_dim": (C.c_int, [_P]),
    "ppv_model_workspace_bytes": (C.c_size_t, [_P, C.c_int, C.c_int]),
    "ppv_model_forward": (C.c_int, [_P, _P, C.c_int, C.c_int, _P, _P, C.c_size_t, _P]),
    "ppv_model_forward_lengths": (C.c_int, [_P, _P, _P, C.c_int, C.c_int, _P, _P, C.c_size_t, _P]),
    "ppv_model_forward_wav": (C.c_int, [_P, _P, _P, _P, C.c_int, C.c_int, _P, _P, C.c_size_t, _P]),
    "ppv_model_read_tap": (C.c_int, [_P, C.c_char_p, _P, C.c_size_t, _P]),
    "ppv_model_profile": (C.c_int, [_P, C.c_int]),
    "ppv_model_profile_read": (C.c_int, [_P, C.POINTER(C.c_double), C.POINTER(C.c_double), C.POINTER(C.c_int64),
                                         C.POINTER(C.c_int64)]),
    "ppv_trainer_create": (C.c_int, [C.POINTER(EcapaCfg), C.c_int, C.POINTER(_P)]),
    "ppv_trainer_destroy": (C.c_int, [_P]),
    "ppv_trainer_param_count": (C.c_int64, [_P]),
    "ppv_trainer_stat_count": (C.c_int64, [_P]),
    "ppv_trainer_lookup": (C.c_int, [_P, C.c_char_p, C.POINTER(C.c_int64), C.POINTER(C.c_int64), C.POINTER(C.c_int)]),
    "ppv_trainer_bind": (C.c_int, [_P, _P, _P, _P]),
    "ppv_trainer_set_precision": (C.c_int, [_P, C.c_int]),
    "ppv_set_pdl": (C.c_int, [C.c_int]),
    "ppv_trainer_workspace_bytes": (C.c_size_t, [_P, C.c_int, C.c_int]),
    "ppv_trainer_forward_backward": (C.c_int, [_P, _P, _P, C.c_int, C.c_int, C.c_float, C.c_float, C.c_int, C.c_float, _P, _P, _P,
                                               C.c_size_t, _P]),
    "ppv_trainer_read_tap": (C.c_int, [_P, C.c_char_p, _P, C.c_size_t, _P]),
    "ppv_adam_step": (C.c_int, [_P, _P, _P, _P, C.c_int64, C.c_float, C.c_float, C.c_float, C.c_float, C.c_float, C.c_int64, C.c_float, _P]),
    "ppv_cosine_workspace_bytes": (C.c_size_t, [C.c_int, C.c_int, C.c_int]),
    "ppv_cosine_matrix": (C.c_int, [_P, _P, C.c_int, C.c_int, C.c_int, _P, _P, C.c_size_t, _P]),
    "ppv_cosine_pairlist": (C.c_int, [_P, _P, C.c_int64, C.c_int, C.c_int, _P, _P]),
    "ppv_fbank_forward_ragged": (C.c_int, [_P, _P, _P, C.c_int, C.c_int, _P, _P]),
    "ppv_audio_prep_workspace_bytes": (C.c_size_t, [C.c_int, C.c_int]),
    "ppv_audio_prep": (C.c_int, [_P, C.c_int64, _P, _P, _P, C.c_int, C.c_int, C.c_float, C.c_int, C.c_int, _P, _P, C.c_size_t, _P]),
    "ppv_eer_workspace_bytes": (C.c_size_t, [C.c_int64]),
    "ppv_eer_mindcf": (C.c_int, [_P, _P, C.c_int64, C.c_double, C.c_double, C.c_double, _P, _P, C.c_size_t, _P]),
    "ppv_eer_mindcf_matrix": (C.c_int, [_P, _P, _P, C.c_int, C.c_int, C.c_double, C.c_double, C.c_double, _P, _P, C.c_size_t, _P]),
    "ppv_row_argmax": (C.c_int, [_P, C.c_int, C.c_int, _P, _P, _P]),
    "ppv_aam_workspace_bytes": (C.c_size_t, [C.c_int, C.c_int, C.c_int]),
    "ppv_aam_forward": (C.c_int, [_P, _P, _P, C.c_int, C.c_int, C.c_int, C.c_float, C.c_float, C.c_int, C.c_float,
                                  _P, _P, _P, C.c_size_t, _P]),
    "ppv_aam_backward": (C.c_int, [_P, _P, _P, _P, C.c_int, C.c_int, C.c_int, C.c_float, C.c_float, C.c_int,
                                   C.c_float, _P, _P, _P, C.c_size_t, _P]),
    "ppv_gemm_test_workspace_bytes": (C.c_size_t, [C.c_int, C.c_int, C.c_int]),
    "ppv_gemm_bench": (C.c_int, [C.c_int, C.c_int, C.c_int, C.c_int, C.c_int, C.c_int, C.c_int, C.c_int, _P, C.c_size_t,
                                 C.POINTER(C.c_float), _P]),
    "ppv_gemm_test": (C.c_int, [_P, _P, _P, _P, _P, C.c_int, C.c_int, C.c_int, C.c_int, C.c_int, C.c_int, C.c_int, _P, _P,
                                C.c_size_t, _P]),
    "ppv_gemm_test_planes": (C.c_int, [_P, _P, _P, _P, _P, _P, C.c_int, C.c_int, C.c_int, C.c_int, C.c_int, C.c_int, C.c_int,
                                       C.c_int, C.c_int, _P, _P, C.c_size_t, _P]),
    "ppv_conv2d_test_workspace_bytes": (C.c_size_t, [C.c_int] * 7),
    "ppv_conv2d_test": (C.c_int, [_P, _P, _P] + [C.c_int] * 13 + [_P, _P, C.c_size_t, _P]),
}

_lib = None


def load(path: str = None):
    global _lib
    if _lib is not None and path is None:
        return _lib
    p = path or LIB_PATH
    if not os.path.exists(p):
        raise PPVError(f"{p} not found: build it with `python -c 'import __graft_entry__ as g; g.build()'` "
                       f"(there is no CPU fallback for the ppvector hot path)")
    lib = C.CDLL(p)
    for name, (res, args) in SIGNATURES.items():
        fn = getattr(lib, name)
        fn.restype = res
        fn.argtypes = args
    if path is None:
        _lib = lib
    return lib


def last_error(lib=None) -> str:
    lib = lib or load()
    buf = C.create_string_buffer(2048)
    lib.ppv_last_error(buf, 2048)
    return buf.value.decode("utf-8", "replace")


def check(rc: int, what: str = ""):
    if rc != 0:
        raise PPVError(f"{what} failed with status {rc}: {last_error()}")


def ptr(t):
    if t is None:
        return None
    assert t.is_contiguous(), "ppv: tensor must be contiguous"
    return C.c_void_p(t.data_ptr())


def require_cuda(t, name="tensor"):
    if not t.is_cuda:
        raise PPVError(f"ppv: {name} must be a CUDA tensor -- the ppvector hot path has no CPU fallback")


def current_stream():
    import torch
    return C.c_void_p(torch.cuda.current_stream().cuda_stream)
```

Baseline: 44940.

## Fuse per-utterance column statistics into GEMM epilogue and rework skinny kernel

The tdnn2 and MFA GEMM epilogues now accumulate per-utterance column sums (and sums of squares for ASP) in fixed-point int64 using warp reduce-scatter and atomics. A tiny finalize kernel replaces the separate colstats passes that re-read the full activation planes for SE squeeze and the ASP global statistics. The skinny linear kernel also moves to a 2x2 register tile with a split-K reduction through shared memory, a smaller K chunk, two blocks per SM, and no K limit. The trade-offs are added epilogue work and atomic traffic, plus small quantisation error from clamping values to ±4096 and the fixed-point scaling.

```diff
diff --git a/include/ppv_b200.h b/include/ppv_b200.h
--- a/include/ppv_b200.h
+++ b/include/ppv_b200.h
@@ -211,6 +211,11 @@
 int ppv_gemm_test_planes(const float* A, const float* W, const float* bias, const float* rowgrp_bias, const float* bn_scale,
                          const float* bn_shift, int relu, int tanh_, int Tp, int P, int M, int N, int K, int block_n,
                          int precision, void* out, void* ws, size_t ws_bytes, void* stream);
+int ppv_gemm_test_stats(const float* A, const float* W, const float* bias, const float* bn_scale, const float* bn_shift, int Tp, int P, int M,
+                        int N, int K, int block_n, int precision, const int* nvalid, void* out, int64_t* stat_sum, int64_t* stat_sq, int* shifts,
+                        void* ws, size_t ws_bytes, void* stream);
+int ppv_skinny_test(const float* A, const float* W, const float* bias, int M, int N, int K, float* out, void* ws, size_t ws_bytes,
+                    void* stream);
 
 size_t ppv_conv2d_test_workspace_bytes(int B, int H, int W, int Cin, int Cout, int k, int x_ld);
 int ppv_conv2d_test(const float* x, const float* w, const float* bias, int relu, int B, int H, int W, int Cin, int Cout, int k,
diff --git a/voiceprintrecognition-paddlepaddle_b200/csrc/capi.cu b/voiceprintrecognition-paddlepaddle_b200/csrc/capi.cu
--- a/voiceprintrecognition-paddlepaddle_b200/csrc/capi.cu
+++ b/voiceprintrecognition-paddlepaddle_b200/csrc/capi.cu
@@ -442,10 +442,10 @@
     PPV_GUARD_END
 }
 
-int ppv_gemm_test_planes(const float* A, const float* W, const float* bias, const float* rowgrp_bias, const float* bn_scale,
-                         const float* bn_shift, int relu, int tanh_, int Tp, int P, int M, int N, int K, int block_n, int precision,
-                         void* out, void* ws, size_t ws_bytes, void* stream) {
-    PPV_GUARD_BEGIN
+static int gemm_test_planes(const float* A, const float* W, const float* bias, const float* rowgrp_bias, const float* bn_scale,
+                            const float* bn_shift, int relu, int tanh_, int Tp, int P, int M, int N, int K, int block_n, int precision,
+                            void* out, void* ws, size_t ws_bytes, void* stream, const int* nvalid, long long* stat_sum, long long* stat_sq,
+                            int* shifts) {
     PPV_REQUIRE(A && W && out && ws, "ppv_gemm_test_planes: null argument");
     PPV_REQUIRE(ws_bytes >= ppv_gemm_test_workspace_bytes(M, N, K), "ppv_gemm_test_planes: workspace too small");
     PPV_REQUIRE(N % 32 == 0 && (Tp == 0 || (M % Tp == 0 && Tp > 2 * P)), "ppv_gemm_test_planes: bad shape");
@@ -484,10 +484,62 @@
         ep.P = P;
         ep.T = Tp - 2 * P;
     }
+    if (stat_sum) {
+        ep.stat_sum = stat_sum;
+        ep.stat_sq = stat_sq;
+        ep.stat_nvalid = nvalid;
+        epilogue_stat_shifts(ep.T, &ep.stat_shift, &ep.stat_sq_shift);
+        shifts[0] = ep.stat_shift;
+        shifts[1] = ep.stat_sq_shift;
+    }
     GemmParams gp;
     rc = gemm_build(&gp, &src, 1, pw, M, N, ep, block_n, 64);
     if (rc) return rc;
     return gemm_launch(gp, precision, device_sm_count(), st);
+}
+int ppv_gemm_test_planes(const float* A, const float* W, const float* bias, const float* rowgrp_bias, const float* bn_scale,
+                         const float* bn_shift, int relu, int tanh_, int Tp, int P, int M, int N, int K, int block_n, int precision,
+                         void* out, void* ws, size_t ws_bytes, void* stream) {
+    PPV_GUARD_BEGIN
+    return gemm_test_planes(A, W, bias, rowgrp_bias, bn_scale, bn_shift, relu, tanh_, Tp, P, M, N, K, block_n, precision, out, ws, ws_bytes, stream,
+                            nullptr, nullptr, nullptr, nullptr);
+    PPV_GUARD_END
+}
+int ppv_gemm_test_stats(const float* A, const float* W, const float* bias, const float* bn_scale, const float* bn_shift, int Tp, int P, int M,
+                        int N, int K, int block_n, int precision, const int* nvalid, void* out, int64_t* stat_sum, int64_t* stat_sq, int* shifts,
+                        void* ws, size_t ws_bytes, void* stream) {
+    PPV_GUARD_BEGIN
+    PPV_REQUIRE(Tp > 0 && stat_sum && shifts, "ppv_gemm_test_stats: needs the padded time layout and stat_sum");
+    return gemm_test_planes(A, W, bias, nullptr, bn_scale, bn_shift, 1, 0, Tp, P, M, N, K, block_n, precision, out, ws, ws_bytes, stream, nvalid,
+                            reinterpret_cast<long long*>(stat_sum), reinterpret_cast<long long*>(stat_sq), shifts);
+    PPV_GUARD_END
+}
+int ppv_skinny_test(const float* A, const float* W, const float* bias, int M, int N, int K, float* out, void* ws, size_t ws_bytes, void* stream) {
+    PPV_GUARD_BEGIN
+    PPV_REQUIRE(A && W && out && ws && K % 64 == 0, "ppv_skinny_test: null argument or K % 64 != 0");
+    PPV_REQUIRE(ws_bytes >= ppv_gemm_test_workspace_bytes(M, N, K), "ppv_skinny_test: workspace too small");
+    int rc = check_device();
+    if (rc) return rc;
+    cudaStream_t st = static_cast<cudaStream_t>(stream);
+    Planes pa, pw;
+    pa.rows = int64_t(au(size_t(M), 128));
+    pa.ld = K;
+    pa.plane_stride = pa.rows * K;
+    pa.base = static_cast<__nv_bfloat16*>(ws);
+    pw.rows = int64_t(au(size_t(N), 256));
+    pw.ld = K;
+    pw.plane_stride = pw.rows * K;
+    pw.base = reinterpret_cast<__nv_bfloat16*>(static_cast<uint8_t*>(ws) + au(size_t(pa.plane_stride) * 4, 256));
+    rc = launch_f32_to_planes(A, M, K, pa, st);
+    if (rc) return rc;
+    rc = launch_f32_to_planes(W, N, K, pw, st);
+    if (rc) return rc;
+    Epilogue ep;
+    ep.bias = bias;
+    ep.out_mode = OUT_F32;
+    ep.out = out;
+    ep.out_ld = N;
+    return skinny_linear_launch(pa, 0, pw, M, N, K, ep, st);
     PPV_GUARD_END
 }
 
@@ -587,7 +639,7 @@
                    float* ms_per_launch, void* stream) {
     PPV_GUARD_BEGIN
     PPV_REQUIRE(ws && ms_per_launch && iters > 0, "ppv_gemm_bench: bad argument");
-    PPV_REQUIRE(planes_out >= 0 && planes_out <= 3, "ppv_gemm_bench: planes_out must be 0-3");
+    PPV_REQUIRE(planes_out >= 0 && planes_out <= 5, "ppv_gemm_bench: planes_out must be 0-5");
     constexpr int kTp = 306, kP = 4;
     PPV_REQUIRE(planes_out < 2 || M % kTp == 0, "ppv_gemm_bench: model epilogues need M % 306 == 0");
     cudaStream_t st = static_cast<cudaStream_t>(stream);
@@ -595,7 +647,8 @@
     const size_t a_bytes = au(au(size_t(M), 128) * Kp * 4, 256), w_bytes = au(au(size_t(N), 256) * Kp * 4, 256);
     const size_t o_bytes = au(au(size_t(M), 128) * size_t(N) * 4, 256);
     const size_t v_bytes = au((3 + size_t(M / kTp)) * size_t(N) * 4, 256);
-    PPV_REQUIRE(ws_bytes >= a_bytes + w_bytes + o_bytes + v_bytes, "ppv_gemm_bench: workspace too small");
+    const size_t s_bytes = planes_out >= 4 ? 2 * size_t(M / kTp) * N * sizeof(long long) : 0;
+    PPV_REQUIRE(ws_bytes >= a_bytes + w_bytes + o_bytes + v_bytes + s_bytes, "ppv_gemm_bench: workspace too small");
     Planes pa, pw, po;
     pa.rows = int64_t(au(size_t(M), 128)); pa.ld = int(Kp); pa.plane_stride = pa.rows * pa.ld; pa.base = static_cast<__nv_bfloat16*>(ws);
     pw.rows = int64_t(au(size_t(N), 256)); pw.ld = int(Kp); pw.plane_stride = pw.rows * pw.ld;
@@ -615,6 +668,13 @@
             ep.bias = vec; ep.bn_scale = vec + N; ep.bn_shift = vec + 2 * N;
             if (planes_out == 3) { ep.rowgrp_bias = vec + 3 * N; ep.tanh_ = 1; }
         }
+        if (planes_out >= 4) {
+            long long* sums = reinterpret_cast<long long*>(static_cast<uint8_t*>(ws) + a_bytes + w_bytes + o_bytes + v_bytes);
+            PPV_CUDA_OK(cudaMemsetAsync(sums, 0, s_bytes, st));
+            ep.stat_sum = sums;
+            if (planes_out == 5) ep.stat_sq = sums + size_t(M / kTp) * N;
+            epilogue_stat_shifts(ep.T, &ep.stat_shift, &ep.stat_sq_shift);
+        }
     } else {
         ep.out_mode = OUT_F32; ep.out = po.base; ep.out_ld = N;
     }
diff --git a/voiceprintrecognition-paddlepaddle_b200/csrc/common.h b/voiceprintrecognition-paddlepaddle_b200/csrc/common.h
--- a/voiceprintrecognition-paddlepaddle_b200/csrc/common.h
+++ b/voiceprintrecognition-paddlepaddle_b200/csrc/common.h
@@ -121,7 +121,19 @@
     int f32_vec_ok = 0;
     int debug_nostore = 0;
     int lean = 0;
-};
+    long long* stat_sum = nullptr;
+    long long* stat_sq = nullptr;
+    const int* stat_nvalid = nullptr;
+    int stat_shift = 0, stat_sq_shift = 0;
+};
+
+constexpr int EPI_STAT_YLOG2 = 12;
+inline void epilogue_stat_shifts(int T, int* s, int* s2) {
+    int L = 0;
+    while ((int64_t(1) << L) < T) ++L;
+    *s = 62 - L - EPI_STAT_YLOG2;
+    *s2 = 62 - L - 2 * EPI_STAT_YLOG2;
+}
 
 constexpr int GEMM_TRACE_TILES = 16;
 
@@ -247,6 +259,8 @@
 int launch_colstats(const Planes& x, int col0, int C, int B, int T, int P, int Tp, int mode, float eps, float* out_f32,
                     const Planes& out_pl, cudaStream_t st, float inv_count = 0.f, const int* nvalid = nullptr);
 int launch_lengths_to_counts(const float* lengths, int B, int T, int* nvalid, cudaStream_t st);
+int launch_stat_finalize(long long* sum, long long* sq, int B, int C, int T, const int* nvalid, int shift, int sq_shift, float eps,
+                         const Planes& out, cudaStream_t st);
 int launch_se_scale_res(const Planes& z, const float* scale, const Planes& res, int rc0, const Planes& out, int oc0, int C,
                         int Tp, int64_t rows, int num_sms, cudaStream_t st, int relu = 0, float relu_max = 0.f);
 int launch_asp_pool(const float* logits, int64_t lg_ld, const Planes& x, int C, int B, int T, int P, int Tp, float eps,
diff --git a/voiceprintrecognition-paddlepaddle_b200/csrc/ecapa.cu b/voiceprintrecognition-paddlepaddle_b200/csrc/ecapa.cu
--- a/voiceprintrecognition-paddlepaddle_b200/csrc/ecapa.cu
+++ b/voiceprintrecognition-paddlepaddle_b200/csrc/ecapa.cu
@@ -37,6 +37,7 @@
     Planes bufs[B_COUNT];
     float *se_mean = nullptr, *se_scale = nullptr, *fold_out = nullptr, *pooled_raw = nullptr, *raw_logmel = nullptr;
     int* nvalid = nullptr;
+    long long *stat_sum = nullptr, *stat_sq = nullptr;
 };
 
 }
@@ -49,6 +50,7 @@
     std::vector<Step> steps;
     EcBuffers buf;
     int Tp = 0;
+    int stat_shift = 0, stat_sq_shift = 0;
     bool prof_on = false;
     std::vector<cudaEvent_t> prof_ev;
     std::vector<int> prof_kind;
@@ -275,6 +277,8 @@
     eb->raw_logmel = static_cast<float*>(cv.take(size_t(B) * T * m->cfg.input_size * 4));
     *emb_out = static_cast<float*>(cv.take(mc_align_up(B, 128) * m->cfg.embd_dim * 4));
     eb->nvalid = static_cast<int*>(cv.take(size_t(B) * sizeof(int)));
+    eb->stat_sum = static_cast<long long*>(cv.take(size_t(B) * C3 * sizeof(long long)));
+    eb->stat_sq = static_cast<long long*>(cv.take(size_t(B) * C3 * sizeof(long long)));
 }
 
 constexpr int ECAPA_MAX_BN = 128;
@@ -300,6 +304,7 @@
     cv.base = static_cast<uint8_t*>(ws);
     carve(m, cv, B, T, &m->buf, &m->emb_out);
     m->Tp = T + 2 * m->P;
+    epilogue_stat_shifts(T, &m->stat_shift, &m->stat_sq_shift);
     PPV_CUDA_OK(cudaMemsetAsync(ws, 0, need, st));
     m->steps.clear();
     const int Tp = m->Tp, P = m->P, C = m->C, C3 = m->C3, w = m->width;
@@ -412,9 +417,13 @@
                 if (rc) return rc;
             }
         }
-        rc = add_gemm(m->tdnn2[b - 1], {{B_H, 0, w, 0, 0, w, 0}, {B_Y, w, C - w, 0, w, C - w, 0}}, nullptr, 0, int(R),
-                      planes_out(m->buf.bufs[B_Z], 0, false));
-        if (rc) return rc;
+        {
+            Epilogue ep = planes_out(m->buf.bufs[B_Z], 0, false);
+            ep.stat_sum = m->buf.stat_sum;
+            ep.stat_shift = m->stat_shift;
+            rc = add_gemm(m->tdnn2[b - 1], {{B_H, 0, w, 0, 0, w, 0}, {B_Y, w, C - w, 0, w, C - w, 0}}, nullptr, 0, int(R), ep);
+            if (rc) return rc;
+        }
         Step s;
         s.blk = b;
         s.kind = Step::SE_SQUEEZE;
@@ -439,10 +448,20 @@
         s.kind = Step::SE_SCALE;
         m->steps.push_back(s);
     }
-    rc = add_gemm(m->mfa, {{B_CAT, 0, C3, 0, 0, C3, 0}}, nullptr, 0, int(R), planes_out(m->buf.bufs[B_MFA], 0, false));
-    if (rc) return rc;
     const int pooling = m->cfg.pooling;
-    if (pooling == PPV_POOL_TAP || pooling == PPV_POOL_TSP) {
+    const bool pool_stats = pooling == PPV_POOL_TAP || pooling == PPV_POOL_TSP;
+    {
+        Epilogue ep = planes_out(m->buf.bufs[B_MFA], 0, false);
+        if (!pool_stats) {
+            ep.stat_sum = m->buf.stat_sum;
+            ep.stat_sq = m->buf.stat_sq;
+            ep.stat_shift = m->stat_shift;
+            ep.stat_sq_shift = m->stat_sq_shift;
+        }
+        rc = add_gemm(m->mfa, {{B_CAT, 0, C3, 0, 0, C3, 0}}, nullptr, 0, int(R), ep);
+        if (rc) return rc;
+    }
+    if (pool_stats) {
         Step s;
         s.kind = Step::POOL_STATS;
         m->steps.push_back(s);
@@ -560,7 +579,15 @@
         prof_mark(tensor_step ? 0 : 1, true);
         if (tensor_step) m->launches_gemm += 1; else m->launches_other += 1;
         switch (s.kind) {
-            case Step::GEMM: rc = gemm_launch(s.gp, m->precision, m->num_sms, st); break;
+            case Step::GEMM:
+                if (nv && s.gp.epi.stat_sum) {
+                    GemmParams gp = s.gp;
+                    gp.epi.stat_nvalid = nv;
+                    rc = gemm_launch(gp, m->precision, m->num_sms, st);
+                } else {
+                    rc = gemm_launch(s.gp, m->precision, m->num_sms, st);
+                }
+                break;
             case Step::SKINNY: rc = skinny_linear_launch(s.sk_x, s.sk_col0, s.sk_w, s.sk_M, s.sk_N, s.sk_K, s.sk_ep, st); break;
             case Step::RES2: rc = res2conv_launch(s.rp, m->precision, m->num_sms, st); break;
             case Step::RES2CHAIN:
@@ -571,7 +598,7 @@
                 }
                 break;
             case Step::SE_SQUEEZE:
-                rc = launch_colstats(m->buf.bufs[B_Z], 0, C, B, T, P, Tp, 0, 0.f, nullptr, m->buf.bufs[B_SEM], st, 0.f, nv);
+                rc = launch_stat_finalize(m->buf.stat_sum, nullptr, B, C, T, nv, m->stat_shift, 0, 0.f, m->buf.bufs[B_SEM], st);
                 break;
             case Step::SE_SCALE: {
                 const Planes& X = (s.blk == 1) ? m->buf.bufs[B_X0] : m->buf.bufs[B_CAT];
@@ -580,7 +607,7 @@
                 break;
             }
             case Step::ASP_GLOBAL:
-                rc = launch_colstats(m->buf.bufs[B_MFA], 0, C3, B, T, P, Tp, 1, 1e-12f, nullptr, m->buf.bufs[B_GSTAT], st, 0.f, nv);
+                rc = launch_stat_finalize(m->buf.stat_sum, m->buf.stat_sq, B, C3, T, nv, m->stat_shift, m->stat_sq_shift, 1e-12f, m->buf.bufs[B_GSTAT], st);
                 break;
             case Step::ASP_FUSED: {
                 AspFusedParams ap = s.ap;
diff --git a/voiceprintrecognition-paddlepaddle_b200/csrc/elementwise.cu b/voiceprintrecognition-paddlepaddle_b200/csrc/elementwise.cu
--- a/voiceprintrecognition-paddlepaddle_b200/csrc/elementwise.cu
+++ b/voiceprintrecognition-paddlepaddle_b200/csrc/elementwise.cu
@@ -172,6 +172,37 @@
     return PPV_OK;
 }
 
+__global__ void __launch_bounds__(256) stat_finalize_kernel(long long* __restrict__ sum, long long* __restrict__ sq, int B, int C, int T,
+                                                            const int* __restrict__ nvalid, int shift, int sq_shift, float eps, Planes out) {
+    griddep_launch_dependents();
+    griddep_wait();
+    const int64_t i = int64_t(blockIdx.x) * blockDim.x + threadIdx.x;
+    if (i >= int64_t(B) * C) return;
+    const int b = int(i / C), c = int(i - int64_t(b) * C);
+    const double inv = 1.0 / double(nvalid ? max(1, min(T, nvalid[b])) : T);
+    const double mean = ldexp(double(sum[i]), -shift) * inv;
+    sum[i] = 0;
+    __nv_bfloat16 h, l;
+    split_bf16(float(mean), h, l);
+    out.hi()[int64_t(b) * out.ld + c] = h;
+    out.lo()[int64_t(b) * out.ld + c] = l;
+    if (sq) {
+        const double var = ldexp(double(sq[i]), -sq_shift) * inv - mean * mean;
+        sq[i] = 0;
+        split_bf16(float(sqrt(fmax(var, double(eps)))), h, l);
+        out.hi()[int64_t(b) * out.ld + C + c] = h;
+        out.lo()[int64_t(b) * out.ld + C + c] = l;
+    }
+}
+
+int launch_stat_finalize(long long* sum, long long* sq, int B, int C, int T, const int* nvalid, int shift, int sq_shift, float eps,
+                         const Planes& out, cudaStream_t st) {
+    const int64_t n = int64_t(B) * C;
+    PPV_PDL_OK(launch_pdl(stat_finalize_kernel, dim3(unsigned((n + 255) / 256)), dim3(256), 0, st, sum, sq, B, C, T, nvalid, shift, sq_shift, eps, out),
+               "stat_finalize_kernel");
+    return PPV_OK;
+}
+
 int launch_colstats(const Planes& x, int col0, int C, int B, int T, int P, int Tp, int mode, float eps, float* out_f32,
                     const Planes& out_pl, cudaStream_t st, float inv_count, const int* nvalid) {
     PPV_REQUIRE(C % 64 == 0 && col0 % 8 == 0 && x.ld % 8 == 0, "colstats: C % 64, col0 % 8, ld % 8 required");
diff --git a/voiceprintrecognition-paddlepaddle_b200/csrc/gemm_epilogue.cuh b/voiceprintrecognition-paddlepaddle_b200/csrc/gemm_epilogue.cuh
--- a/voiceprintrecognition-paddlepaddle_b200/csrc/gemm_epilogue.cuh
+++ b/voiceprintrecognition-paddlepaddle_b200/csrc/gemm_epilogue.cuh
@@ -137,6 +137,47 @@
     }
 }
 
+__device__ __forceinline__ long long stat_reduce_scatter8(long long (&v)[8], int l) {
+#pragma unroll
+    for (int stage = 0; stage < 3; ++stage) {
+        const int half = 4 >> stage;
+        const bool up = (l & (16 >> stage)) != 0;
+#pragma unroll
+        for (int i = 0; i < half; ++i) {
+            const long long r = __shfl_xor_sync(0xffffffffu, up ? v[i] : v[i + half], 16 >> stage);
+            v[i] = (up ? v[i + half] : v[i]) + r;
+        }
+    }
+    return v[0];
+}
+
+__device__ __forceinline__ float stat_clamp(float y) {
+    constexpr float lim = float(1 << EPI_STAT_YLOG2);
+    return fminf(fmaxf(y, -lim), lim);
+}
+
+__device__ __forceinline__ void epilogue_stats_trip(const Epilogue& ep, int N, int col0, const float (&a)[8], const float (&b)[8], bool ca,
+                                                    bool cb, int ga, int gb, int g_lo, int g_hi, bool whole, int l) {
+    const float s1 = __int_as_float((127 + ep.stat_shift) << 23), s2 = __int_as_float((127 + ep.stat_sq_shift) << 23);
+    const int col = col0 + (l >> 2);
+    for (int g = g_lo; g <= g_hi; ++g) {
+        const bool ia = whole || (ca && ga == g), ib = whole || (cb && gb == g);
+        long long v[8];
+#pragma unroll
+        for (int k = 0; k < 8; ++k)
+            v[k] = (ia ? __float2ll_rn(stat_clamp(a[k]) * s1) : 0ll) + (ib ? __float2ll_rn(stat_clamp(b[k]) * s1) : 0ll);
+        atomicAdd(reinterpret_cast<unsigned long long*>(ep.stat_sum + int64_t(g) * N + col), (unsigned long long)stat_reduce_scatter8(v, l));
+        if (ep.stat_sq) {
+#pragma unroll
+            for (int k = 0; k < 8; ++k) {
+                const float ya = stat_clamp(a[k]), yb = stat_clamp(b[k]);
+                v[k] = (ia ? __float2ll_rn(ya * ya * s2) : 0ll) + (ib ? __float2ll_rn(yb * yb * s2) : 0ll);
+            }
+            atomicAdd(reinterpret_cast<unsigned long long*>(ep.stat_sq + int64_t(g) * N + col), (unsigned long long)stat_reduce_scatter8(v, l));
+        }
+    }
+}
+
 template <int BN, typename RowOf>
 __device__ __forceinline__ void epilogue_frag_lean(const Epilogue& ep, int N, int n0, float (&acc)[BN / 2], RowOf&& row_of, int t) {
     static_assert(BN % 32 == 0, "lean epilogue: whole 32-column trips");
@@ -151,6 +192,17 @@
     const int64_t lo_off = ep.out_plane_stride;
     const float* const ga = ep.rowgrp_bias ? ep.rowgrp_bias + ra.grp * N + cq : nullptr;
     const float* const gb = ep.rowgrp_bias ? ep.rowgrp_bias + rb.grp * N + cq : nullptr;
+    bool ca = false, cb = false, whole = false;
+    int g_lo = 0, g_hi = -1;
+    if (ep.stat_sum) {
+        auto counts = [&](const EpiRow& r) {
+            return r.valid && (!ep.stat_nvalid || int(r.out_row - r.grp * ep.Tp) - ep.P < max(1, __ldg(ep.stat_nvalid + r.grp)));
+        };
+        ca = counts(ra), cb = counts(rb);
+        g_lo = __reduce_min_sync(0xffffffffu, ca ? int(ra.grp) : cb ? int(rb.grp) : 0x7fffffff);
+        g_hi = __reduce_max_sync(0xffffffffu, cb ? int(rb.grp) : ca ? int(ra.grp) : -1);
+        whole = __all_sync(0xffffffffu, ca && cb) && g_lo == g_hi;
+    }
 #pragma unroll 1
     for (int c = 0; c < BN / 8; c += 4) {
         float a[8], b[8];
@@ -189,6 +241,7 @@
             *reinterpret_cast<uint4*>(pb + j0) = hb;
             *reinterpret_cast<uint4*>(pb + j0 + lo_off) = lb;
         }
+        if (g_hi >= 0) epilogue_stats_trip(ep, N, cq + j0, a, b, ca, cb, int(ra.grp), int(rb.grp), g_lo, g_hi, whole, l);
     }
 }
 
diff --git a/voiceprintrecognition-paddlepaddle_b200/csrc/gemm_wgmma.cu b/voiceprintrecognition-paddlepaddle_b200/csrc/gemm_wgmma.cu
--- a/voiceprintrecognition-paddlepaddle_b200/csrc/gemm_wgmma.cu
+++ b/voiceprintrecognition-paddlepaddle_b200/csrc/gemm_wgmma.cu
@@ -409,6 +409,8 @@
     } else {
         gp->epi.f32_vec_ok = ((epi.out_ld % 2) == 0 && (epi.out_col0 % 2) == 0 && (reinterpret_cast<uintptr_t>(epi.out) & 7) == 0) ? 1 : 0;
     }
+    PPV_REQUIRE(!epi.stat_sum || (gp->epi.lean && epi.Tp > 0), "gemm_build: epilogue statistics need the lean epilogue over the padded time layout");
+    PPV_REQUIRE(!epi.stat_sq || epi.stat_sum, "gemm_build: stat_sq needs stat_sum");
     return PPV_OK;
 }
 
diff --git a/voiceprintrecognition-paddlepaddle_b200/csrc/skinny.cu b/voiceprintrecognition-paddlepaddle_b200/csrc/skinny.cu
--- a/voiceprintrecognition-paddlepaddle_b200/csrc/skinny.cu
+++ b/voiceprintrecognition-paddlepaddle_b200/csrc/skinny.cu
@@ -6,12 +6,12 @@
 namespace {
 
 constexpr int SK_R = 16, SK_C = 16;
-constexpr int SK_KC = 512;
+constexpr int SK_KC = 256;
 constexpr int SK_LD = SK_KC + 4;
 constexpr int SK_ITERS = (SK_R + SK_C) * (SK_KC / 8) / 256;
 constexpr int SK_SMEM = (SK_R + SK_C) * SK_LD * 4;
 
-__global__ void __launch_bounds__(256) skinny_linear_kernel(Planes x, int x_col0, Planes W, int M, int N, int K, Epilogue ep) {
+__global__ void __launch_bounds__(256, 2) skinny_linear_kernel(Planes x, int x_col0, Planes W, int M, int N, int K, Epilogue ep) {
     extern __shared__ __align__(16) float sk_smem[];
     float(*sx)[SK_LD] = reinterpret_cast<float(*)[SK_LD]>(sk_smem);
     float(*sw)[SK_LD] = reinterpret_cast<float(*)[SK_LD]>(sk_smem + SK_R * SK_LD);
@@ -56,29 +56,40 @@
             *reinterpret_cast<float4*>(dst + 4) = make_float4(v[4], v[5], v[6], v[7]);
         }
     };
-    float acc0 = 0.f, acc1 = 0.f, acc2 = 0.f, acc3 = 0.f;
+    const int kg = tid >> 6, mr = tid & 7, mc = (tid >> 3) & 7;
+    float acc[2][2] = {{0.f, 0.f}, {0.f, 0.f}};
     fetch(0);
     for (int k0 = 0; k0 < K; k0 += SK_KC) {
         const int kc = min(SK_KC, K - k0);
         stash();
         __syncthreads();
         if (k0 + SK_KC < K) fetch(k0 + SK_KC);
-        const float* px = sx[lr];
-        const float* pw = sw[lc];
-#pragma unroll 4
-        for (int k = 0; k < kc; k += 4) {
-            const float4 a = *reinterpret_cast<const float4*>(px + k);
-            const float4 b = *reinterpret_cast<const float4*>(pw + k);
-            acc0 = fmaf(a.x, b.x, acc0);
-            acc1 = fmaf(a.y, b.y, acc1);
-            acc2 = fmaf(a.z, b.z, acc2);
-            acc3 = fmaf(a.w, b.w, acc3);
+#pragma unroll 2
+        for (int k = 4 * kg; k < kc; k += 16) {
+            const float4 a0 = *reinterpret_cast<const float4*>(&sx[mr][k]), a1 = *reinterpret_cast<const float4*>(&sx[mr + 8][k]);
+            const float4 b0 = *reinterpret_cast<const float4*>(&sw[mc][k]), b1 = *reinterpret_cast<const float4*>(&sw[mc + 8][k]);
+            const float4 av[2] = {a0, a1}, bv[2] = {b0, b1};
+#pragma unroll
+            for (int i = 0; i < 2; ++i)
+#pragma unroll
+                for (int j = 0; j < 2; ++j) {
+                    acc[i][j] = fmaf(av[i].x, bv[j].x, acc[i][j]);
+                    acc[i][j] = fmaf(av[i].y, bv[j].y, acc[i][j]);
+                    acc[i][j] = fmaf(av[i].z, bv[j].z, acc[i][j]);
+                    acc[i][j] = fmaf(av[i].w, bv[j].w, acc[i][j]);
+                }
         }
         __syncthreads();
     }
+    float(*part)[SK_R][SK_C] = reinterpret_cast<float(*)[SK_R][SK_C]>(sk_smem);
+#pragma unroll
+    for (int i = 0; i < 2; ++i)
+#pragma unroll
+        for (int j = 0; j < 2; ++j) part[kg][mr + 8 * i][mc + 8 * j] = acc[i][j];
+    __syncthreads();
     const int r = r0 + lr, c = c0 + lc;
     if (r >= M || c >= N) return;
-    float y = (acc0 + acc1) + (acc2 + acc3);
+    float y = ((part[0][lr][lc] + part[1][lr][lc]) + part[2][lr][lc]) + part[3][lr][lc];
     if (ep.bias) y += ep.bias[c];
     if (ep.relu) y = fmaxf(y, 0.f);
     if (ep.sigmoid_) y = 1.f / (1.f + expf(-y));
@@ -96,7 +107,7 @@
 }
 
 bool skinny_linear_supported(int M, int N, int K, const Epilogue& ep) {
-    return M <= 4096 && K % 8 == 0 && K <= 1024 && !ep.rowgrp_bias && !ep.seg_scale && !ep.bn_scale && !ep.tanh_ && !ep.silu_ && ep.Tp == 0 && ep.img_Wp == 0 &&
+    return M <= 4096 && K % 8 == 0 && !ep.rowgrp_bias && !ep.seg_scale && !ep.bn_scale && !ep.tanh_ && !ep.silu_ && ep.Tp == 0 && ep.img_Wp == 0 &&
            ep.relu_max == 0.f;
 }
 
diff --git a/voiceprintrecognition-paddlepaddle_b200/ppvector/_lib.py b/voiceprintrecognition-paddlepaddle_b200/ppvector/_lib.py
--- a/voiceprintrecognition-paddlepaddle_b200/ppvector/_lib.py
+++ b/voiceprintrecognition-paddlepaddle_b200/ppvector/_lib.py
@@ -132,6 +132,8 @@
                                 C.c_size_t, _P]),
     "ppv_gemm_test_planes": (C.c_int, [_P, _P, _P, _P, _P, _P, C.c_int, C.c_int, C.c_int, C.c_int, C.c_int, C.c_int, C.c_int,
                                        C.c_int, C.c_int, _P, _P, C.c_size_t, _P]),
+    "ppv_gemm_test_stats": (C.c_int, [_P, _P, _P, _P, _P] + [C.c_int] * 7 + [_P, _P, _P, _P, _P, _P, C.c_size_t, _P]),
+    "ppv_skinny_test": (C.c_int, [_P, _P, _P, C.c_int, C.c_int, C.c_int, _P, _P, C.c_size_t, _P]),
     "ppv_conv2d_test_workspace_bytes": (C.c_size_t, [C.c_int] * 7),
     "ppv_conv2d_test": (C.c_int, [_P, _P, _P] + [C.c_int] * 13 + [_P, _P, C.c_size_t, _P]),
 }
```

New measurement: 46290 (median of 6 runs). 1.03x the previous value.
